# nekopanda/Amatsukaze

Hardware: NVIDIA H100
Metric: 1920x1080i YV12 frames/sec (logo-eval + combing) (higher is better)
Workload: dtype u8+f32

## Files before the change

__graft_entry__.py:

```python
import os
import sys

ROOT = os.path.dirname(os.path.abspath(__file__))
if ROOT not in sys.path:
    sys.path.insert(0, ROOT)


def build():
    from amatsukaze_b200 import _build
    _build.build()
    _build.build_host_test()
    _build.build_pipeline_test()
    _build.build_host_only_test()
    _build.build_tnr_filter_test()
    _build.build_tnr_widen_test()
    _build.build_tnr_filter_stream_test()
    from oracle import pyoracle
    pyoracle.build_oracle()
    pyoracle.build_ref()
    from oracle import pytnr
    pytnr.build_oracle()
    pytnr.build_ref()
    from oracle import pytnr_stream
    pytnr_stream.build_ref()
    import amatsukaze_b200 as ab
    ab.lib()


def smoke():
    import numpy as np
    import torch
    import amatsukaze_b200 as ab
    from amatsukaze_b200 import synth
    from oracle import pyoracle as po

    assert torch.cuda.is_available(), "smoke() needs a GPU: there is no CPU fallback"
    torch.cuda.set_device(0)
    W, H, n, imgx, imgy = 512, 256, 12, 400, 40
    lg = synth.make_logo(64, 64)
    frames = synth.make_frames(45, n, W, H, device="cuda:0", logo=lg, imgx=imgx, imgy=imgy, logo_period=20)
    ctx = ab.Context(0, torch.cuda.current_stream().cuda_stream)
    logo = ab.Logo.create(lg["data"], 64, 64, W, H, imgx, imgy).deint().create_mask(0.35)
    prm = ab.default_comb_params()
    scores, counts = ctx.scan_comb_frames(ab.yv12_clip(frames, W, H, n, True), [logo], prm)
    torch.cuda.synchronize()
    scores, counts = scores.cpu().numpy(), counts.cpu().numpy()
    Y, U, V = synth.split_planes(frames, W, H)
    if po.ref_available():
        rlog = po.RefLogo.create(lg["data"], 64, 64, W, H, imgx, imgy).deint().create_mask(0.35)
        ref_s = np.stack([po.ref_scan_frame(rlog, Y[i]) for i in range(n)])
        checker = "reference code (oracle/_ref)"
    else:
        olog = po.OracleLogo.create(lg["data"], 64, 64, W, H, imgx, imgy).deint().create_mask(0.35)
        ref_s = np.stack([olog.scan_frame(Y[i]) for i in range(n)])
        checker = "C port (oracle/amtk_oracle.c)"
    ref_c = po.or_comb_clip(Y, U, V, prm.as_list())
    assert np.array_equal(scores[:, 0].view(np.uint32), ref_s.view(np.uint32)), "logo scores differ from the oracle"
    assert np.array_equal(counts, ref_c), "combing counters differ from the oracle"
    launches = ctx.launches
    assert launches >= 2
    ctx.close()
    del logo
    print("smoke ok: %d frames bit-exact vs %s, corr0 range [%.3f, %.3f], launches=%d"
          % (n, checker, ref_s[:, 0].min(), ref_s[:, 0].max(), launches))


if __name__ == "__main__":
    build()
    print("build ok")
```

amatsukaze_b200/csrc/amtk_b200.cu:

```cuda
#include "amtk_internal.h"
#include "logo_kernels.cuh"
#include "comb_kernels.cuh"
#include "comb_stream.cuh"
#include "comb_mma.cuh"
#include "scan_kernels.cuh"
#include "tnr_kernels.cuh"
#include <algorithm>
#include <cfloat>
#include <cmath>
#include <cstdlib>
#include <cstring>
#include <deque>
#include <mutex>

extern "C" { static int logo_ensure_device(const amtk_logo* cl, amtk_ctx* ctx, bool need_tables); }

namespace amtk {

static thread_local std::string g_error;
static constexpr size_t kEvalSmemLimit = 226 * 1024;
void set_error(const std::string& msg) { g_error = msg; }
bool cuda_ok(cudaError_t e, const char* what) {
  if (e == cudaSuccess) return true;
  set_error(std::string("CUDA error: ") + cudaGetErrorString(e) + " in " + what);
// ... 52 lines not shown
  if (ctx->stage_bytes < need) {
    for (int b = 0; b < 2; ++b) { if (ctx->stage[b]) cudaFree(ctx->stage[b]); ctx->stage[b] = nullptr; }
    ctx->stage_bytes = 0;
    for (int b = 0; b < 2; ++b) AMTK_CUDA(cudaMalloc(&ctx->stage[b], need));
    ctx->stage_bytes = need;
  }
  int chunk = 0;
  long long h2d = 0;
  for (int lo = frame0; lo < frame0 + nframes; lo += per, ++chunk) {
    const int hi = std::min(frame0 + nframes, lo + per);
    const int b = chunk & 1;
    const int first = (need_prev && lo > 0) ? lo - 1 : lo;
    AMTK_CUDA(cudaStreamWaitEvent(ctx->copy_stream, ctx->ev_done[b], 0));
    AMTK_CUDA(cudaMemcpyAsync(ctx->stage[b], reinterpret_cast<const uint8_t*>(clip->base) + (size_t)first * fs,
                              (size_t)(hi - first) * fs, cudaMemcpyHostToDevice, ctx->copy_stream));
    AMTK_CUDA(cudaEventRecord(ctx->ev_copy[b], ctx->copy_stream));
    AMTK_CUDA(cudaStreamWaitEvent(ctx->stream, ctx->ev_copy[b], 0));
    Window w{ reinterpret_cast<const uint8_t*>(ctx->stage[b]), first, hi - first };
    if (!fn(w, lo, hi)) return 0;
    AMTK_CUDA(cudaEventRecord(ctx->ev_done[b], ctx->stream));
    h2d += (long long)(hi - first) * (long long)fs;
  }
  ctx->h2d_bytes_last = h2d;
  return 1;
}

template <typename Fn>
static int for_each_roi_window(amtk_ctx* ctx, const amtk_clip* clip, int frame0, int nframes, int rx, int ry, int rw, int rh,
                               bool with_chroma, bool write_back, Fn fn) {
  if (frame0 < 0 || nframes < 0 || frame0 + nframes > clip->num_frames) AMTK_FAIL("frame range outside the clip");
  if (nframes == 0) return 1;
  if (clip->on_device) {
    Window w{ reinterpret_cast<const uint8_t*>(clip->base), 0, clip->num_frames };
    return fn(*clip, w, frame0, frame0 + nframes, 0, 0);
  }
  const int bps = clip->bytes_per_sample, lx = clip->log_uvx, ly = clip->log_uvy;
  const int A = 16 << lx;
  const int xb0 = ((rx * bps) / A) * A;
  const int xb1 = std::min(clip->pitch_y, (((rx + rw) * bps + A - 1) / A) * A);
  const int cp = ((xb1 - xb0 + A - 1) / A) * A;
  const int dy = ry & ~((1 << ly) - 1);
  const int y1 = std::min(clip->height, (ry + rh + (1 << ly) - 1) & ~((1 << ly) - 1));
  const int rowsY = y1 - dy, rowsC = with_chroma ? (rowsY >> ly) : 0;
  const int cpc = cp >> lx, spanY = xb1 - xb0;
  const int xc0 = xb0 >> lx, spanC = std::min(clip->pitch_uv - xc0, spanY >> lx);
  const int rows_u = rowsY, rows_c_as_y = (int)(((long long)cpc * rowsC + cp - 1) / cp);
  const long long offU = (long long)cp * rows_u, offV = offU + (long long)cp * rows_c_as_y;
  const long long fs = with_chroma ? offV + (long long)cp * rows_c_as_y : (long long)cp * rowsY;
  if (cp <= 0 || rowsY <= 0 || (with_chroma && spanC <= 0)) AMTK_FAIL("ROI staging: empty rectangle");
  size_t budget = (size_t)256 << 20;
  if (const char* e = getenv("AMTK_STAGE_MB")) budget = (size_t)std::max(1, atoi(e)) << 20;
  const int per = (int)std::max<size_t>(1, std::min<size_t>((size_t)nframes, budget / (size_t)fs));
  const size_t need = (size_t)per * (size_t)fs;
  if (ctx->stage_bytes < need) {
    for (int b = 0; b < 2; ++b) { if (ctx->stage[b]) cudaFree(ctx->stage[b]); ctx->stage[b] = nullptr; }
    ctx->stage_bytes = 0;
    for (int b = 0; b < 2; ++b) AMTK_CUDA(cudaMalloc(&ctx->stage[b], std::max(need, (size_t)1 << 20)));
    ctx->stage_bytes = std::max(need, (size_t)1 << 20);
  }
  amtk_clip v = *clip;
  v.frame_stride = fs; v.off_u = offU; v.off_v = offV;
  v.width = cp / bps; v.height = rowsY; v.pitch_y = cp; v.pitch_uv = cpc; v.on_device = 1;
  const uint8_t* hbase = reinterpret_cast<const uint8_t*>(clip->base);
  auto copy_plane = [&](int pl, uint8_t* dev, int first, int count, bool to_host, cudaStream_t st) -> bool {
    const long long hoff = pl == 0 ? 0 : (pl == 1 ? clip->off_u : clip->off_v);
    const int hp = pl ? clip->pitch_uv : clip->pitch_y, dp = pl ? cpc : cp;
    const int span = pl ? spanC : spanY, rows = pl ? rowsC : rowsY;
    const long long doff = pl == 0 ? 0 : (pl == 1 ? offU : offV);
    uint8_t* h = const_cast<uint8_t*>(hbase) + (long long)first * clip->frame_stride + hoff + (long long)(pl ? (dy >> ly) : dy) * hp + (pl ? xc0 : xb0);
    uint8_t* d = dev + doff;
    if (clip->frame_stride % hp == 0 && fs % dp == 0) {
      cudaMemcpy3DParms p3; memset(&p3, 0, sizeof(p3));
      const cudaPitchedPtr hptr = make_cudaPitchedPtr(h, (size_t)hp, (size_t)hp, (size_t)(clip->frame_stride / hp));
      const cudaPitchedPtr dptr = make_cudaPitchedPtr(d, (size_t)dp, (size_t)dp, (size_t)(fs / dp));
      p3.srcPtr = to_host ? dptr : hptr; p3.dstPtr = to_host ? hptr : dptr;
      p3.extent = make_cudaExtent((size_t)span, (size_t)rows, (size_t)count);
      p3.kind = to_host ? cudaMemcpyDeviceToHost : cudaMemcpyHostToDevice;
      return cuda_ok(cudaMemcpy3DAsync(&p3, st), "cudaMemcpy3DAsync(roi)");
    }
    for (int f = 0; f < count; ++f) {
      uint8_t* hf = h + (long long)f * clip->frame_stride; uint8_t* df = d + (long long)f * fs;
      if (!cuda_ok(to_host ? cudaMemcpy2DAsync(hf, hp, df, dp, span, rows, cudaMemcpyDeviceToHost, st)
                           : cudaMemcpy2DAsync(df, dp, hf, hp, span, rows, cudaMemcpyHostToDevice, st), "cudaMemcpy2DAsync(roi)")) return false;
    }
    return true;
  };
  int chunk = 0;
  for (int lo = frame0; lo < frame0 + nframes; lo += per, ++chunk) {
    const int hi = std::min(frame0 + nframes, lo + per);
    const int b = chunk & 1;
    uint8_t* dev = reinterpret_cast<uint8_t*>(ctx->stage[b]);
    AMTK_CUDA(cudaStreamWaitEvent(ctx->copy_stream, ctx->ev_done[b], 0));
    for (int pl = 0; pl < (with_chroma ? 3 : 1); ++pl) if (!copy_plane(pl, dev, lo, hi - lo, false, ctx->copy_stream)) return 0;
    AMTK_CUDA(cudaEventRecord(ctx->ev_copy[b], ctx->copy_stream));
    AMTK_CUDA(cudaStreamWaitEvent(ctx->stream, ctx->ev_copy[b], 0));
    v.base = dev; v.num_frames = hi - lo;
    Window w{ dev, lo, hi - lo };
    if (!fn(v, w, lo, hi, xb0 / bps, dy)) return 0;
    if (write_back)
      for (int pl = 0; pl < (with_chroma ? 3 : 1); ++pl) if (!copy_plane(pl, dev, lo, hi - lo, true, ctx->stream)) return 0;
    AMTK_CUDA(cudaEventRecord(ctx->ev_done[b], ctx->stream));
  }
  ctx->h2d_bytes_last = (long long)nframes * ((long long)spanY * rowsY + (with_chroma ? 2LL * spanC * rowsC : 0));
  return 1;
}

struct EvalSpec {
  const amtk_logo* logo;
  int roi_x, roi_y;
  int roi_w, roi_h;
  int src_mode, src_off, src_stride;
  int nfades; const float* fades;
  int take_abs;
  int out_off, out_fade_stride;
};

static bool want_smem(amtk_ctx* ctx, const void* fn, int bytes) {
  static std::mutex mu;
  static std::vector<std::pair<std::pair<int, const void*>, int>> table;
  std::lock_guard<std::mutex> lock(mu);
  for (auto& e : table) if (e.first.first == ctx->device && e.first.second == fn) {
    if (e.second >= bytes) return true;
    if (!cuda_ok(cudaFuncSetAttribute(fn, cudaFuncAttributeMaxDynamicSharedMemorySize, bytes), "cudaFuncSetAttribute")) return false;
    e.second = bytes; return true;
  }
  if (!cuda_ok(cudaFuncSetAttribute(fn, cudaFuncAttributeMaxDynamicSharedMemorySize, bytes), "cudaFuncSetAttribute")) return false;
  table.emplace_back(std::make_pair(ctx->device, fn), bytes);
  return true;
}

static int launch_eval(amtk_ctx* ctx, const amtk_clip* clip, const Window& win, int lo, int hi, int pitch_elems,
                       const EvalSpec& sp, float* dout, int out_frame_stride, int out_row0) {
  const amtk::HostLogo& hl = sp.logo->host;
  if (!logo_ensure_device(sp.logo, ctx, true)) return 0;
  if (sp.nfades < 1 || sp.nfades > kMaxFades) AMTK_FAIL("too many fade levels");
  const int count = hl.count();
  const int bits = clip->bits_per_sample;
  const float maxv = (float)((1 << bits) - 1);
  if (count == 0) {
    AMTK_FAIL("logo has no feature pixels");
  }
  const int countPad = sp.logo->countPad;
  const int bps = clip->bytes_per_sample;
  const int box_x = ((sp.roi_x * bps) & ~15) / bps;
  const int box_w = ((((sp.roi_x - box_x) + sp.roi_w) * bps + 15) & ~15) / bps;
  const long long pitch_bytes = (long long)pitch_elems * bps;
  const long long plane_rows = ((long long)clip->pitch_y * clip->height) / pitch_bytes;
  const bool tma_ok = ctx->encode_tiled && box_w <= 256 && sp.roi_h <= 256 && (pitch_bytes & 15) == 0 &&
                      (clip->frame_stride & 15) == 0 && (reinterpret_cast<uintptr_t>(win.dev_base) & 15) == 0;
  int ab_smem = 1, pair_fades = 1;
  size_t smem = logo_scores_smem_bytes(sp.roi_w * sp.roi_h, hl.w * hl.h, box_w * sp.roi_h * bps, ab_smem, pair_fades);
  if (smem > kEvalSmemLimit) { ab_smem = 0; smem = logo_scores_smem_bytes(sp.roi_w * sp.roi_h, hl.w * hl.h, box_w * sp.roi_h * bps, ab_smem, pair_fades); }
  if (smem > kEvalSmemLimit) { pair_fades = 0; smem = logo_scores_smem_bytes(sp.roi_w * sp.roi_h, hl.w * hl.h, box_w * sp.roi_h * bps, ab_smem, pair_fades); }
  if (smem > kEvalSmemLimit) AMTK_FAIL("logo too large for the shared-memory evaluation path (more than ~24k pixels)");
  CUtensorMap roi_map;
  memset(&roi_map, 0, sizeof(roi_map));
  if (tma_ok) {
    cuuint64_t gdim[3] = { (cuuint64_t)pitch_elems, (cuuint64_t)plane_rows, (cuuint64_t)win.count };
    cuuint64_t gstr[2] = { (cuuint64_t)pitch_bytes, (cuuint64_t)clip->frame_stride };
    cuuint32_t box[3] = { (cuuint32_t)box_w, (cuuint32_t)sp.roi_h, 1u };
    cuuint32_t estr[3] = { 1u, 1u, 1u };
    CUresult r = ctx->encode_tiled(&roi_map, bps == 1 ? CU_TENSOR_MAP_DATA_TYPE_UINT8 : CU_TENSOR_MAP_DATA_TYPE_UINT16, 3,
                                   const_cast<uint8_t*>(win.dev_base), gdim, gstr, box, estr, CU_TENSOR_MAP_INTERLEAVE_NONE,
                                   CU_TENSOR_MAP_SWIZZLE_NONE, CU_TENSOR_MAP_L2_PROMOTION_NONE, CU_TENSOR_MAP_FLOAT_OOB_FILL_NONE);
    if (r != CUDA_SUCCESS) AMTK_FAIL("cuTensorMapEncodeTiled(roi) failed (" + std::to_string((int)r) + ")");
  }
  const size_t per_frame = (size_t)sp.nfades * countPad * sizeof(float);
  const int batch = (int)std::max<size_t>(1, std::min<size_t>((size_t)(hi - lo), ((size_t)96 << 20) / per_frame));
  if (!ensure(&ctx->scratch, &ctx->scratch_bytes, ctx->scratch_off + per_frame * batch)) return 0;
  for (int f0 = lo; f0 < hi; f0 += batch) {
    const int n = std::min(batch, hi - f0);
    EvalJob job;
    job.ybase = win.dev_base; job.frame_stride = clip->frame_stride; job.pitch = pitch_elems;
    job.frame0 = f0 - win.first; job.nframes = n;
    job.imgx = sp.roi_x; job.imgy = sp.roi_y;
    job.roi_w = sp.roi_w; job.roi_h = sp.roi_h;
    job.src_mode = sp.src_mode; job.src_off = sp.src_off; job.src_stride = sp.src_stride;
    job.logo = logo_dev(sp.logo); job.maxv = maxv; job.nfades = sp.nfades;
    for (int i = 0; i < sp.nfades; ++i) job.fades[i] = sp.fades[i];
    job.scores = reinterpret_cast<float*>(reinterpret_cast<uint8_t*>(ctx->scratch) + ctx->scratch_off);
    job.use_tma = tma_ok ? 1 : 0; job.roi_box_w = box_w; job.roi_box_x = box_x; job.roi_map = roi_map;
    job.ab_smem = ab_smem; job.pair_fades = pair_fades;
    const int slices3 = (count + kEvalThreads * 3 - 1) / (kEvalThreads * 3);
    int pxt = 3, slices = slices3;
    if (count <= kEvalThreads) { pxt = 1; slices = 1; }
    else if (count <= kEvalThreads * 2) { pxt = 2; slices = 1; }
    const int lanes = std::max(1, std::min(n, (ctx->sm_count * ctx->knobs.eval_waves) / slices));
    dim3 grid(slices, lanes);
    const bool u16 = clip->bytes_per_sample == 2;
    const bool w64 = hl.w == 64 && sp.roi_w == 64 && ctx->knobs.eval_cw;
    const bool wh64 = w64 && hl.h == 64 && sp.roi_h == 64;
#define AMTK_LAUNCH_SCORES(T, P)                                                                              \
  do {                                                                                                        \
    void (*kfn)(const EvalJob) = wh64 ? logo_scores_kernel<T, P, 64, 64> : w64 ? logo_scores_kernel<T, P, 64, 0> : logo_scores_kernel<T, P, 0, 0>; \
    if (!want_smem(ctx, (const void*)kfn, (int)smem)) return 0;                                                \
    kfn<<<grid, kEvalThreads, smem, ctx->stream>>>(job);                                                      \
  } while (0)
    if (!u16) { if (pxt == 1) AMTK_LAUNCH_SCORES(uint8_t, 1); else if (pxt == 2) AMTK_LAUNCH_SCORES(uint8_t, 2); else AMTK_LAUNCH_SCORES(uint8_t, 3); }
    else      { if (pxt == 1) AMTK_LAUNCH_SCORES(uint16_t, 1); else if (pxt == 2) AMTK_LAUNCH_SCORES(uint16_t, 2); else AMTK_LAUNCH_SCORES(uint16_t, 3); }
#undef AMTK_LAUNCH_SCORES
    AMTK_CUDA(cudaGetLastError());
    const int total = n * sp.nfades;
    float* sum_out = dout + (size_t)(f0 - out_row0) * out_frame_stride;
    const size_t sum_smem = (size_t)32 * (countPad + 4) * sizeof(float);
    if (sum_smem <= 200 * 1024) {
      if (!want_smem(ctx, (const void*)logo_sum_bulk_kernel, (int)sum_smem)) return 0;
      logo_sum_bulk_kernel<<<(total + 31) / 32, 32, sum_smem, ctx->stream>>>(
          job.scores, count, countPad, n, sp.nfades, hl.blackScore, sp.take_abs, sum_out, out_frame_stride, sp.out_off, sp.out_fade_stride);
    } else {
      logo_sum_kernel<<<(total + kSumThreads - 1) / kSumThreads, kSumThreads, 0, ctx->stream>>>(
          job.scores, count, countPad, n, sp.nfades, hl.blackScore, sp.take_abs, sum_out, out_frame_stride, sp.out_off, sp.out_fade_stride);
    }
    AMTK_CUDA(cudaGetLastError());
    ctx->launches += 2;
  }
  return 1;
}

static bool roi_inside(const amtk::HostLogo& full, const amtk_clip* clip, int pitch_elems) {
  if (full.imgx < 0 || full.imgy < 0) return false;
  const long long last = (long long)full.imgx + full.w - 1 + (long long)(full.imgy + full.h - 1) * pitch_elems;
  const long long plane_elems = (long long)clip->pitch_y / clip->bytes_per_sample * clip->height;
  return full.imgx + full.w <= pitch_elems && last < plane_elems;
}

static int comb_thresholds_ok(const amtk_comb_params* p, int bytes_per_sample) {
  if (bytes_per_sample == 2) {
    const int all[6] = { p->th_move_y, p->th_shima_y, p->th_lshima_y, p->th_move_c, p->th_shima_c, p->th_lshima_c };
    for (int v : all) if (v < 1) { set_error("comb: thresholds must be >= 1"); return 0; }
    if (p->th_move_y > 32768 || p->th_move_c > 32768) { set_error("comb: th_move must be in [1,32768] for 16-bit samples"); return 0; }
    return 1;
  }
  const int m[2] = { p->th_move_y, p->th_move_c };
  const int s[4] = { p->th_shima_y, p->th_lshima_y, p->th_shima_c, p->th_lshima_c };
  for (int v : m) if (v < 1 || v > 128) { set_error("comb: th_move must be in [1,128]"); return 0; }
  for (int v : s) if (v < 1 || v > 2047) { set_error("comb: th_shima/th_lshima must be in [1,2047]"); return 0; }
  return 1;
}

struct CombVariant {
  int R, strip, stages, sync, TH, boxH, threads, smem;
  void (*kernel)(const CombArgs);
  void (*kernel16)(const CombArgs);
};
template <typename Cfg> static CombVariant make_variant() {
  return CombVariant{ Cfg::R, Cfg::STRIP, Cfg::STAGES, Cfg::SYNC, Cfg::TH, Cfg::BOXH, Cfg::THREADS, Cfg::SMEM, comb_tma_kernel<Cfg, 1>, nullptr };
}
template <typename Cfg> static CombVariant make_variant16() {
  return CombVariant{ Cfg::R, Cfg::STRIP, Cfg::STAGES, Cfg::SYNC, Cfg::TH, Cfg::BOXH, Cfg::THREADS, Cfg::SMEM, comb_tma_kernel<Cfg, 1>, comb_tma_kernel<Cfg, 2> };
}
static const CombVariant* comb_variants(int* n) {
  static const CombVariant v[] = {
    make_variant16<CombCfg<15, 8, 3, 0>>(), make_variant16<CombCfg<16, 8, 3, 0>>(), make_variant16<CombCfg<17, 8, 3, 0>>(),
    make_variant<CombCfg<17, 8, 2, 0>>(), make_variant<CombCfg<17, 8, 4, 0>>(), make_variant<CombCfg<17, 8, 3, 1>>(),
  };
  *n = (int)(sizeof(v) / sizeof(v[0]));
  return v;
}

static int pick_comb_R(int hY, int hC) {
  int best = 16; long long best_waste = -1;
  for (int R = 17; R >= 15; --R) {
    const int th = 8 * R;
    const long long waste = (long long)((hY + th - 1) / th) * th - hY + 2LL * (((hC + th - 1) / th) * th - hC) / 2;
    if (best_waste < 0 || waste < best_waste) { best_waste = waste; best = R; }
  }
  return best;
}

struct WsVariant { int R, stages, warps, bps, TH, boxH, smem; bool band; void (*kernel)(const WsArgs); };
template <typename Cfg> static WsVariant make_ws() { return WsVariant{ Cfg::R, Cfg::STAGES, Cfg::WARPS, Cfg::BPS, Cfg::TH, Cfg::BOXH, Cfg::SMEM, Cfg::BAND, comb_ws_kernel<Cfg> }; }
static const WsVariant* ws_variants(int* n) {
  static const WsVariant v[] = { make_ws<WsCfg<17, 2>>(), make_ws<WsCfg<15, 2>>(), make_ws<WsCfg<16, 2>>(), make_ws<WsCfg<9, 2>>(), make_ws<WsCfg<15, 3>>(), make_ws<WsCfg<12, 2>>(), make_ws<WsCfg<10, 2>>(),
                                 make_ws<WsCfg<15, 2, 7>>(), make_ws<WsCfg<13, 2, 5>>(), make_ws<WsCfg<15, 2, 2>>(), make_ws<WsCfg<15, 3, 3>>(),
                                 make_ws<WsCfg<15, 2, 4, 2>>(), make_ws<WsCfg<16, 2, 4, 2>>(), make_ws<WsCfg<17, 2, 4, 2>>(),
                                 make_ws<WbCfg<15, 2>>(), make_ws<WbCfg<16, 2>>(), make_ws<WbCfg<17, 2>>(), make_ws<WbCfg<15, 3>>() };
  *n = (int)(sizeof(v) / sizeof(v[0]));
  return v;
}
static int pick_ws_R(int hY, int hC) {
  int best = 17; long long best_waste = -1;
  for (int R : { 17, 16, 15 }) {
    const int th = 4 * R;
    const long long waste = 2LL * ((long long)((hY + th - 1) / th) * th - hY) + 2LL * ((long long)((hC + th - 1) / th) * th - hC);
    if (best_waste < 0 || waste < best_waste) { best_waste = waste; best = R; }
  }
  return best;
}

static int ws_watchdog_ok(amtk_ctx* ctx) {
  if (!ctx->watch_pending) return 1;
  AMTK_CUDA(cudaEventSynchronize(ctx->ev_watch));
  ctx->watch_pending = false;
  const int* d = ctx->ws_watch;
  if (d[0]) {
    char msg[256];
    snprintf(msg, sizeof(msg), "comb_ws (band form): a device-side wait of the previous launch timed out (wait %d, step %d, CTA %d, thread %d, parity %d); its counters are not valid",
             d[1], d[2], d[3], d[4], d[5]);
    AMTK_FAIL(msg);
  }
  return 1;
}

static int launch_comb_ws(amtk_ctx* ctx, const amtk_clip* clip, const Window& win, int lo, int hi,
                          const amtk_comb_params* prm, int* dcounts, int out_row0) {
  const int hY = clip->height, hC = clip->height >> clip->log_uvy;
  const int wY = clip->width, wC = clip->width >> clip->log_uvx;
  const int R = ctx->knobs.comb_R ? ctx->knobs.comb_R : pick_ws_R(hY, hC);
  int nvar = 0; const WsVariant* vars = ws_variants(&nvar); const WsVariant* V = nullptr;
  const int bps = clip->bytes_per_sample;
  const bool band = bps == 1 && ctx->knobs.comb_ws_band && ctx->knobs.comb_ws_warps == kWsWarps;
  for (int i = 0; i < nvar; ++i)
    if (vars[i].R == R && vars[i].stages == ctx->knobs.comb_ws_stages && vars[i].warps == ctx->knobs.comb_ws_warps && vars[i].bps == bps && vars[i].band == band) V = &vars[i];
  if (!V) AMTK_FAIL("comb: no warp-stream kernel variant for the requested AMTK_COMB_* settings");
  const int WW = V->warps;
  if (!ws_watchdog_ok(ctx)) return 0;
  WsArgs args;
  memset(&args, 0, sizeof(args));
  const CUtensorMapL2promotion promo = ctx->knobs.comb_l2 == 0 ? CU_TENSOR_MAP_L2_PROMOTION_NONE : ctx->knobs.comb_l2 == 64 ? CU_TENSOR_MAP_L2_PROMOTION_L2_64B :
                                       ctx->knobs.comb_l2 == 256 ? CU_TENSOR_MAP_L2_PROMOTION_L2_256B : CU_TENSOR_MAP_L2_PROMOTION_L2_128B;
  for (int pl = 0; pl < 3; ++pl) {
    const long long off = pl == 0 ? 0 : (pl == 1 ? clip->off_u : clip->off_v);
    cuuint64_t gdim[3] = { (cuuint64_t)(pl ? wC : wY) * bps, (cuuint64_t)(pl ? hC : hY), (cuuint64_t)win.count };
    cuuint64_t gstr[2] = { (cuuint64_t)(pl ? clip->pitch_uv : clip->pitch_y), (cuuint64_t)clip->frame_stride };
    cuuint32_t box[3] = { (cuuint32_t)(band ? kWbHalf : kWsTW), (cuuint32_t)V->boxH, 1u };
    cuuint32_t estr[3] = { 1u, 1u, 1u };
    if (ctx->encode_tiled(&args.map[pl], CU_TENSOR_MAP_DATA_TYPE_UINT8, 3, const_cast<uint8_t*>(win.dev_base) + off, gdim, gstr, box, estr,
                          CU_TENSOR_MAP_INTERLEAVE_NONE, CU_TENSOR_MAP_SWIZZLE_NONE, promo, CU_TENSOR_MAP_FLOAT_OOB_FILL_NONE) != CUDA_SUCCESS)
      AMTK_FAIL("cuTensorMapEncodeTiled failed");
  }
  const int remC = (wC * bps) % kWsTW;
  const long long uv_dist = clip->off_v - clip->off_u;
  const bool pair_uv = !band && ctx->knobs.comb_merge_uv && remC > 0 && remC <= kWsTW / 2 && uv_dist > 0 && (uv_dist & 15) == 0;
  if (pair_uv) {
    cuuint64_t gdim[4] = { (cuuint64_t)wC * bps, 2u, (cuuint64_t)hC, (cuuint64_t)win.count };
    cuuint64_t gstr[3] = { (cuuint64_t)uv_dist, (cuuint64_t)clip->pitch_uv, (cuuint64_t)clip->frame_stride };
    cuuint32_t box[4] = { (cuuint32_t)(kWsTW / 2), 2u, (cuuint32_t)V->boxH, 1u };
    cuuint32_t estr[4] = { 1u, 1u, 1u, 1u };
    if (ctx->encode_tiled(&args.map_uv, CU_TENSOR_MAP_DATA_TYPE_UINT8, 4, const_cast<uint8_t*>(win.dev_base) + clip->off_u, gdim, gstr, box, estr,
                          CU_TENSOR_MAP_INTERLEAVE_NONE, CU_TENSOR_MAP_SWIZZLE_NONE, promo, CU_TENSOR_MAP_FLOAT_OOB_FILL_NONE) != CUDA_SUCCESS)
      AMTK_FAIL("cuTensorMapEncodeTiled(uv pair) failed");
  }
  const int tyY = (hY + V->TH - 1) / V->TH, tyC = (hC + V->TH - 1) / V->TH;
  int tile0 = 0, nc = 0;
  auto thresholds = [&](WsClass& C, bool chroma) {
    C.cls = chroma ? 1 : 0; C.H = chroma ? hC : hY;
    const int tM = chroma ? prm->th_move_c : prm->th_move_y, tS = chroma ? prm->th_shima_c : prm->th_shima_y, tL = chroma ? prm->th_lshima_c : prm->th_lshima_y;
    if (bps == 1) {
      C.thM = (unsigned)(0x80 - tM) * 0x01010101u;
      C.thS = (unsigned)tS * 0x00010001u;
      C.thL = (unsigned)tL * 0x00010001u;
    } else {
      C.thM = (unsigned)std::min(tM, 2047) * 0x00010001u;
      C.thS = (unsigned)(8192 + std::min(tS, 8191)) * 0x00010001u;
      C.thL = (unsigned)(8192 + std::min(tL, 8191)) * 0x00010001u;
    }
  };
  for (int pl = 0; pl < 3; ++pl) {
    WsClass& C = args.cl[nc];
    const int w = (pl ? wC : wY) * bps;
    C.kind = 0; C.map = pl; C.W = w; thresholds(C, pl != 0);
    C.tilesX = band ? (w + kWbW - 1) / kWbW : (pl && pair_uv) ? w / kWsTW : (w + kWsTW - 1) / kWsTW;
    C.tile0 = tile0; C.ntiles = C.tilesX * (pl ? tyC : tyY);
    if (C.ntiles == 0) continue;
    tile0 += C.ntiles; ++nc;
  }
  if (pair_uv) {
    WsClass& C = args.cl[nc];
    C.kind = 1; C.x0 = wC * bps - remC; C.tilesX = 1; thresholds(C, true);
    C.tile0 = tile0; C.ntiles = tyC; tile0 += C.ntiles; ++nc;
  }
  args.nclasses = nc;
  const int ntiles = tile0, nf = hi - lo;
  amtk_ctx::CombPlan& plan = ctx->plan;
  if (plan.occ_kernel != (const void*)V->kernel) {
    int occ = 0;
    AMTK_CUDA(cudaFuncSetAttribute(V->kernel, cudaFuncAttributeMaxDynamicSharedMemorySize, V->smem));
    AMTK_CUDA(cudaOccupancyMaxActiveBlocksPerMultiprocessor(&occ, V->kernel, 32 * WW, V->smem));
    if (occ < 1) AMTK_FAIL("comb kernel does not fit on an SM");
    plan.occ = occ; plan.occ_kernel = (const void*)V->kernel; plan.valid = false;
  }
  int occ = plan.occ;
  if (ctx->knobs.comb_ctas > 0) occ = std::min(occ, ctx->knobs.comb_ctas);
  const long long total = (long long)ntiles * nf;
  const int per_cta = band ? 1 : WW;
  const int nwarps = ctx->sm_count * occ * per_cta;
  const int grid = (int)std::min<long long>((long long)ctx->sm_count * occ, (total + per_cta - 1) / per_cta);
  const int f0 = lo - win.first;
  if (!(plan.valid && plan.wY == wY && plan.hY == hY && plan.wC == wC && plan.hC == hC && plan.ntiles == ntiles && plan.nf == nf && plan.f0 == f0 &&
        plan.R == V->R + 100 * bps + 1000 * band && plan.item == ctx->knobs.comb_item + 1000 * ctx->knobs.comb_tail && plan.ctas == occ * WW)) {
    int big = ctx->knobs.comb_item > 0 ? ctx->knobs.comb_item : 64, small = std::max(4, big / 4);
    while (big > 8 && (long long)ntiles * (nf / big) < 6LL * nwarps) { big /= 2; small = std::max(4, big / 4); }
    const int tail_frames = std::min(nf, std::max(small, (int)(nf * 0.15)));
    const int head_frames = nf - tail_frames;
    const int tiny = ctx->knobs.comb_tail;
    const int end_frames = (tiny > 0 && tiny < small) ? std::min(tail_frames, std::max(tiny, (int)(nf * 0.04))) : 0;
    const int mid_end = nf - end_frames;
    std::vector<CombSegment> segs;
    segs.reserve((size_t)ntiles * (head_frames / big + tail_frames / small + (tiny > 0 ? end_frames / tiny : 0) + 3));
    auto tier = [&](int fa, int fz, int step) {
      if (band) {
        for (int f = fa; f < fz; f += step)
          for (int t = 0; t < ntiles; ++t) segs.push_back(CombSegment{ t, f0 + f, f0 + std::min(fz, f + step) });
      } else {
        for (int t = 0; t < ntiles; ++t)
          for (int f = fa; f < fz; f += step) segs.push_back(CombSegment{ t, f0 + f, f0 + std::min(fz, f + step) });
      }
    };
    tier(0, head_frames, big);
    tier(head_frames, mid_end, small);
    if (tiny > 0) tier(mid_end, nf, tiny);
    const size_t seg_bytes = segs.size() * sizeof(CombSegment);
    plan.q_off = (seg_bytes + 255) & ~(size_t)255;
    plan.valid = false;
    if (!ensure(&plan.dev, &plan.cap, plan.q_off + 256)) return 0;
    AMTK_CUDA(cudaMemcpyAsync(plan.dev, segs.data(), seg_bytes, cudaMemcpyHostToDevice, ctx->stream));
    AMTK_CUDA(cudaStreamSynchronize(ctx->stream));
    plan.nitems = (int)segs.size();
    plan.wY = wY; plan.hY = hY; plan.wC = wC; plan.hC = hC; plan.ntiles = ntiles; plan.nf = nf; plan.f0 = f0; plan.R = V->R + 100 * bps + 1000 * band;
    plan.item = ctx->knobs.comb_item + 1000 * ctx->knobs.comb_tail; plan.ctas = occ * WW; plan.valid = true;
  }
  AMTK_CUDA(cudaMemsetAsync(reinterpret_cast<uint8_t*>(plan.dev) + plan.q_off, 0, 256, ctx->stream));
  args.segs = reinterpret_cast<const CombSegment*>(plan.dev);
  args.nitems = plan.nitems;
  args.queue = reinterpret_cast<int*>(reinterpret_cast<uint8_t*>(plan.dev) + plan.q_off);
  args.counts = dcounts;
  args.out_frame0 = out_row0 - win.first;
  AMTK_CUDA(cudaMemsetAsync(dcounts + (size_t)(lo - out_row0) * 12, 0, (size_t)nf * 12 * sizeof(int), ctx->stream));
  std::pair<cudaEvent_t, cudaEvent_t> ev{ nullptr, nullptr };
  if (ctx->timing) {
    if (!ctx->timing_pool.empty()) { ev = ctx->timing_pool.back(); ctx->timing_pool.pop_back(); }
    else { AMTK_CUDA(cudaEventCreate(&ev.first)); AMTK_CUDA(cudaEventCreate(&ev.second)); }
    AMTK_CUDA(cudaEventRecord(ev.first, ctx->stream));
  }
  args.prefetch = ctx->knobs.comb_ws_prefetch;
  if (ctx->want_side_mark) {
    AMTK_CUDA(cudaEventRecord(ctx->ev_side, ctx->stream));
    ctx->want_side_mark = false;
  }
  V->kernel<<<grid, 32 * WW, V->smem, ctx->stream>>>(args);
  AMTK_CUDA(cudaGetLastError());
  if (ctx->timing) { AMTK_CUDA(cudaEventRecord(ev.second, ctx->stream)); ctx->timing_events.push_back(ev); }
  ctx->launches += 1;
  if (band) {
    if (!ctx->ws_watch) {
      AMTK_CUDA(cudaHostAlloc(&ctx->ws_watch, 8 * sizeof(int), cudaHostAllocDefault));
      AMTK_CUDA(cudaEventCreateWithFlags(&ctx->ev_watch, cudaEventDisableTiming));
    }
    AMTK_CUDA(cudaMemcpyAsync(ctx->ws_watch, args.queue + 16, 8 * sizeof(int), cudaMemcpyDeviceToHost, ctx->stream));
    AMTK_CUDA(cudaEventRecord(ctx->ev_watch, ctx->stream));
    ctx->watch_pending = true;
  }
  return 1;
}

static int launch_comb_mma(amtk_ctx* ctx, const amtk_clip* clip, const Window& win, int lo, int hi,
                           const amtk_comb_params* prm, int* dcounts, int out_row0) {
  const int hY = clip->height, hC = clip->height >> clip->log_uvy;
  const int wY = clip->width, wC = clip->width >> clip->log_uvx;
  WsArgs args;
  memset(&args, 0, sizeof(args));
  const CUtensorMapL2promotion promo = ctx->knobs.comb_l2 == 0 ? CU_TENSOR_MAP_L2_PROMOTION_NONE : ctx->knobs.comb_l2 == 64 ? CU_TENSOR_MAP_L2_PROMOTION_L2_64B :
                                       ctx->knobs.comb_l2 == 256 ? CU_TENSOR_MAP_L2_PROMOTION_L2_256B : CU_TENSOR_MAP_L2_PROMOTION_L2_128B;
  for (int pl = 0; pl < 3; ++pl) {
    const long long off = pl == 0 ? 0 : (pl == 1 ? clip->off_u : clip->off_v);
    cuuint64_t gdim[3] = { (cuuint64_t)(pl ? wC : wY), (cuuint64_t)(pl ? hC : hY), (cuuint64_t)win.count };
    cuuint64_t gstr[2] = { (cuuint64_t)(pl ? clip->pitch_uv : clip->pitch_y), (cuuint64_t)clip->frame_stride };
    cuuint32_t box[3] = { (cuuint32_t)kMmTW, (cuuint32_t)kMmBoxH, 1u };
    cuuint32_t estr[3] = { 1u, 1u, 1u };
    if (ctx->encode_tiled(&args.map[pl], CU_TENSOR_MAP_DATA_TYPE_UINT8, 3, const_cast<uint8_t*>(win.dev_base) + off, gdim, gstr, box, estr,
                          CU_TENSOR_MAP_INTERLEAVE_NONE, CU_TENSOR_MAP_SWIZZLE_128B, promo, CU_TENSOR_MAP_FLOAT_OOB_FILL_NONE) != CUDA_SUCCESS)
      AMTK_FAIL("cuTensorMapEncodeTiled failed");
  }
  const int tyY = (hY + kMmTH - 1) / kMmTH, tyC = (hC + kMmTH - 1) / kMmTH;
  int tile0 = 0, nc = 0;
  for (int pl = 0; pl < 3; ++pl) {
    WsClass& C = args.cl[nc];
    const bool chroma = pl != 0;
    C.kind = 0; C.map = pl; C.cls = chroma ? 1 : 0; C.H = chroma ? hC : hY;
    C.thM = (unsigned)(0x80 - (chroma ? prm->th_move_c : prm->th_move_y)) * 0x01010101u;
    C.thS = (unsigned)(chroma ? prm->th_shima_c : prm->th_shima_y) * 0x00010001u;
    C.thL = (unsigned)(chroma ? prm->th_lshima_c : prm->th_lshima_y) * 0x00010001u;
    C.tilesX = ((chroma ? wC : wY) + kMmTW - 1) / kMmTW;
    C.tile0 = tile0; C.ntiles = C.tilesX * (chroma ? tyC : tyY);
    if (C.ntiles == 0) continue;
    tile0 += C.ntiles; ++nc;
  }
  args.nclasses = nc;
  const int ntiles = tile0, nf = hi - lo;
  amtk_ctx::CombPlan& plan = ctx->plan;
  const int NS = ctx->knobs.comb_mma == 2 ? 2 : 1;
  void (*kern)(const WsArgs) = NS == 2 ? comb_mma_kernel<2> : comb_mma_kernel<1>;
  const int smem = NS * kMmSmemPerStream + kMmBandBytes + 1024;
  if (plan.occ_kernel != (const void*)kern) {
    AMTK_CUDA(cudaFuncSetAttribute(kern, cudaFuncAttributeMaxDynamicSharedMemorySize, smem));
    int occ_q = 0;
    AMTK_CUDA(cudaOccupancyMaxActiveBlocksPerMultiprocessor(&occ_q, kern, kMmThreads, smem));
    if (occ_q < 1) AMTK_FAIL("comb_mma: kernel does not fit on an SM");
    plan.occ = occ_q; plan.occ_kernel = (const void*)kern; plan.valid = false;
  }
  int occ = plan.occ;
  if (ctx->knobs.comb_ctas > 0) occ = std::min(occ, ctx->knobs.comb_ctas);
  const int npairs_t = (ntiles + NS - 1) / NS;
  const long long total = (long long)npairs_t * nf;
  const int nstreams = ctx->sm_count * occ;
  const int grid = (int)std::min<long long>(nstreams, total);
  const int f0 = lo - win.first;
  if (!(plan.valid && plan.wY == wY && plan.hY == hY && plan.wC == wC && plan.hC == hC && plan.ntiles == ntiles && plan.nf == nf && plan.f0 == f0 &&
        plan.R == 1000 * NS + kMmTH && plan.item == ctx->knobs.comb_item && plan.ctas == occ)) {
    int big = ctx->knobs.comb_item > 0 ? ctx->knobs.comb_item : 64, small = std::max(4, big / 4);
    while (big > 8 && (long long)npairs_t * (nf / big) < 6LL * nstreams) { big /= 2; small = std::max(4, big / 4); }
    const int tail_frames = std::min(nf, std::max(small, (int)(nf * 0.15)));
    const int head_frames = nf - tail_frames;
    std::vector<CombSegment> segs;
    segs.reserve((size_t)NS * npairs_t * (head_frames / big + tail_frames / small + 2));
    auto push_block = [&](int fa, int fz) {
      for (int t = 0; t < ntiles; t += NS) {
        segs.push_back(CombSegment{ t, fa, fz });
        if (NS == 2) segs.push_back(CombSegment{ t + 1 < ntiles ? t + 1 : ~t, fa, fz });
      }
    };
    for (int f = 0; f < head_frames; f += big) push_block(f0 + f, f0 + std::min(head_frames, f + big));
    for (int f = head_frames; f < nf; f += small) push_block(f0 + f, f0 + std::min(nf, f + small));
    const size_t seg_bytes = segs.size() * sizeof(CombSegment);
    plan.q_off = (seg_bytes + 255) & ~(size_t)255;
    plan.valid = false;
    if (!ensure(&plan.dev, &plan.cap, plan.q_off + 256)) return 0;
    AMTK_CUDA(cudaMemcpyAsync(plan.dev, segs.data(), seg_bytes, cudaMemcpyHostToDevice, ctx->stream));
    AMTK_CUDA(cudaStreamSynchronize(ctx->stream));
    plan.nitems = (int)segs.size();
    plan.wY = wY; plan.hY = hY; plan.wC = wC; plan.hC = hC; plan.ntiles = ntiles; plan.nf = nf; plan.f0 = f0; plan.R = 1000 * NS + kMmTH;
    plan.item = ctx->knobs.comb_item; plan.ctas = occ; plan.valid = true;
  }
  AMTK_CUDA(cudaMemsetAsync(reinterpret_cast<uint8_t*>(plan.dev) + plan.q_off, 0, 256, ctx->stream));
  args.segs = reinterpret_cast<const CombSegment*>(plan.dev);
  args.nitems = plan.nitems;
  args.queue = reinterpret_cast<int*>(reinterpret_cast<uint8_t*>(plan.dev) + plan.q_off);
  args.counts = dcounts;
  args.out_frame0 = out_row0 - win.first;
  AMTK_CUDA(cudaMemsetAsync(dcounts + (size_t)(lo - out_row0) * 12, 0, (size_t)nf * 12 * sizeof(int), ctx->stream));
  std::pair<cudaEvent_t, cudaEvent_t> ev{ nullptr, nullptr };
  if (ctx->timing) {
    if (!ctx->timing_pool.empty()) { ev = ctx->timing_pool.back(); ctx->timing_pool.pop_back(); }
    else { AMTK_CUDA(cudaEventCreate(&ev.first)); AMTK_CUDA(cudaEventCreate(&ev.second)); }
    AMTK_CUDA(cudaEventRecord(ev.first, ctx->stream));
  }
  kern<<<grid, kMmThreads, smem, ctx->stream>>>(args);
  AMTK_CUDA(cudaGetLastError());
  if (ctx->timing) { AMTK_CUDA(cudaEventRecord(ev.second, ctx->stream)); ctx->timing_events.push_back(ev); }
  ctx->launches += 1;
  int dbg[8] = { 0, 0, 0, 0, 0, 0, 0, 0 };
  AMTK_CUDA(cudaMemcpyAsync(dbg, args.queue + 16, sizeof(dbg), cudaMemcpyDeviceToHost, ctx->stream));
  AMTK_CUDA(cudaStreamSynchronize(ctx->stream));
  if (dbg[0]) {
    char msg[256];
    snprintf(msg, sizeof(msg), "comb_mma<%d>: a device-side wait timed out (wait %d, step %d, CTA %d, thread %d, parity %d); results discarded",
             NS, dbg[1], dbg[2], dbg[3], dbg[4], dbg[5]);
    AMTK_FAIL(msg);
  }
  return 1;
}

static int launch_comb(amtk_ctx* ctx, const amtk_clip* clip, const Window& win, int lo, int hi,
                       const amtk_comb_params* prm, int* dcounts, int out_row0) {
  const bool tma_layout = !((clip->frame_stride & 15) || (clip->pitch_y & 15) || (clip->pitch_uv & 15) || (clip->off_u & 15) ||
                            (clip->off_v & 15) || (reinterpret_cast<uintptr_t>(win.dev_base) & 15));
  if (!tma_layout || !ctx->encode_tiled || ctx->knobs.comb_generic) {
    CombGenericArgs g;
    g.base = win.dev_base; g.frame_stride = clip->frame_stride;
    g.off[0] = 0; g.off[1] = clip->off_u; g.off[2] = clip->off_v;
    const int bps = clip->bytes_per_sample;
    for (int pl = 0; pl < 3; ++pl) {
      g.pitch[pl] = (pl ? clip->pitch_uv : clip->pitch_y) / bps;
      g.W[pl] = pl ? (clip->width >> clip->log_uvx) : clip->width;
      g.H[pl] = pl ? (clip->height >> clip->log_uvy) : clip->height;
      g.thM[pl] = pl ? prm->th_move_c : prm->th_move_y;
      g.thS[pl] = pl ? prm->th_shima_c : prm->th_shima_y;
      g.thL[pl] = pl ? prm->th_lshima_c : prm->th_lshima_y;
    }
    g.first_frame = lo - win.first; g.prev_of_first = lo > 0 ? lo - 1 - win.first : lo - win.first;
    g.nframes = hi - lo; g.counts = dcounts + (size_t)(lo - out_row0) * 12;
    AMTK_CUDA(cudaMemsetAsync(g.counts, 0, (size_t)(hi - lo) * 12 * sizeof(int), ctx->stream));
    for (int f0 = 0; f0 < hi - lo; f0 += 16384) {
      CombGenericArgs gg = g;
      gg.first_frame = g.first_frame + f0; gg.prev_of_first = f0 ? gg.first_frame - 1 : g.prev_of_first;
      gg.nframes = std::min(16384, hi - lo - f0); gg.counts = g.counts + (size_t)f0 * 12;
      dim3 grid((g.W[0] + kGenTW - 1) / kGenTW, (g.H[0] + kGenTH - 1) / kGenTH, gg.nframes * 3);
      if (bps == 1) comb_generic_kernel<uint8_t><<<grid, 256, 0, ctx->stream>>>(gg);
      else comb_generic_kernel<uint16_t><<<grid, 256, 0, ctx->stream>>>(gg);
      AMTK_CUDA(cudaGetLastError());
      ctx->launches += 1;
    }
    return 1;
  }
  if (clip->bytes_per_sample == 1 && ctx->knobs.comb_mma) return launch_comb_mma(ctx, clip, win, lo, hi, prm, dcounts, out_row0);
  if (ctx->knobs.comb_ws && (clip->bytes_per_sample == 1 || (clip->bits_per_sample <= 10 && ctx->knobs.comb_ws10)))
    return launch_comb_ws(ctx, clip, win, lo, hi, prm, dcounts, out_row0);
  const int hY = clip->height, hC = clip->height >> clip->log_uvy;
  const int R = ctx->knobs.comb_R ? ctx->knobs.comb_R : pick_comb_R(hY, hC);
  int nvar = 0; const CombVariant* vars = comb_variants(&nvar); const CombVariant* V = nullptr;
  for (int i = 0; i < nvar; ++i) if (vars[i].R == R && vars[i].strip == ctx->knobs.comb_strip && vars[i].stages == ctx->knobs.comb_stages && vars[i].sync == ctx->knobs.comb_sync) V = &vars[i];
  if (!V) AMTK_FAIL("comb: no kernel variant for the requested AMTK_COMB_* settings");
  const int bps = clip->bytes_per_sample;
  if (bps == 2 && !V->kernel16) AMTK_FAIL("comb: the selected AMTK_COMB_* variant has no 16-bit kernel");
  const int twe = kCombTW / bps;
  CombArgs args;
  memset(&args, 0, sizeof(args));
  const int wC = clip->width >> clip->log_uvx;
  const int rem = wC % twe;
  const bool merge_uv = ctx->knobs.comb_merge_uv && rem > 0 && rem <= twe / 2 && (V->boxH * (kCombTW / 2)) % 128 == 0;
  int tile0 = 0;
  for (int pl = 0; pl < 4; ++pl) {
    CombPlane& P = args.plane[pl];
    const bool chroma = pl != 0;
    P.W = chroma ? wC : clip->width;
    P.H = chroma ? hC : hY;
    P.tilesX = (P.W + twe - 1) / twe; P.tilesY = (P.H + V->TH - 1) / V->TH;
    if (merge_uv && (pl == 1 || pl == 2)) P.tilesX -= 1;
    if (pl == 3) { P.tilesX = merge_uv ? 1 : 0; if (!merge_uv) P.tilesY = 0; }
    P.tile0 = tile0; tile0 += P.tilesX * P.tilesY;
    P.cls = chroma ? 1 : 0;
    const int thM = chroma ? prm->th_move_c : prm->th_move_y;
    const int thS = chroma ? prm->th_shima_c : prm->th_shima_y, thL = chroma ? prm->th_lshima_c : prm->th_lshima_y;
    if (bps == 1) {
      P.thM = (unsigned)(0x80 - thM) * 0x01010101u;
      P.thS = (unsigned)thS * 0x00010001u;
      P.thL = (unsigned)thL * 0x00010001u;
    } else {
      P.thM = (unsigned)(0x8000 - thM) * 0x00010001u;
      const float fs = (float)thS, fl = (float)thL;
      memcpy(&P.thS, &fs, 4); memcpy(&P.thL, &fl, 4);
    }
    if (pl == 3) break;
    const long long off = pl == 0 ? 0 : (pl == 1 ? clip->off_u : clip->off_v);
    const int pitch = pl ? clip->pitch_uv : clip->pitch_y;
    cuuint64_t gdim[3] = { (cuuint64_t)P.W, (cuuint64_t)P.H, (cuuint64_t)win.count };
    cuuint64_t gstr[2] = { (cuuint64_t)pitch, (cuuint64_t)clip->frame_stride };
    cuuint32_t estr[3] = { 1u, 1u, 1u };
    const CUtensorMapL2promotion promo = ctx->knobs.comb_l2 == 0 ? CU_TENSOR_MAP_L2_PROMOTION_NONE : ctx->knobs.comb_l2 == 64 ? CU_TENSOR_MAP_L2_PROMOTION_L2_64B :
                                         ctx->knobs.comb_l2 == 256 ? CU_TENSOR_MAP_L2_PROMOTION_L2_256B : CU_TENSOR_MAP_L2_PROMOTION_L2_128B;
    for (int half = 0; half < (pl && merge_uv ? 2 : 1); ++half) {
      cuuint32_t box[3] = { (cuuint32_t)(half ? twe / 2 : twe), (cuuint32_t)V->boxH, 1u };
      CUtensorMap* m = half ? &args.map_half[pl - 1] : &args.map[pl];
      CUresult r = ctx->encode_tiled(m, bps == 1 ? CU_TENSOR_MAP_DATA_TYPE_UINT8 : CU_TENSOR_MAP_DATA_TYPE_UINT16, 3, const_cast<uint8_t*>(win.dev_base) + off, gdim, gstr, box, estr,
                                     CU_TENSOR_MAP_INTERLEAVE_NONE, CU_TENSOR_MAP_SWIZZLE_NONE, promo, CU_TENSOR_MAP_FLOAT_OOB_FILL_NONE);
      if (r != CUDA_SUCCESS) AMTK_FAIL("cuTensorMapEncodeTiled failed (" + std::to_string((int)r) + ")");
    }
  }
  args.half_x = wC - rem;
  const int ntiles = tile0;
  const int nf = hi - lo;
  int occ = 0;
  void (*kern)(const CombArgs) = bps == 1 ? V->kernel : V->kernel16;
  AMTK_CUDA(cudaFuncSetAttribute(kern, cudaFuncAttributeMaxDynamicSharedMemorySize, V->smem));
  AMTK_CUDA(cudaOccupancyMaxActiveBlocksPerMultiprocessor(&occ, kern, V->threads, V->smem));
  if (occ < 1) AMTK_FAIL("comb kernel does not fit on an SM");
  if (ctx->knobs.comb_ctas > 0) occ = std::min(occ, ctx->knobs.comb_ctas);
  const long long total = (long long)ntiles * nf;
  int grid = (int)std::min<long long>((long long)ctx->sm_count * occ, total);
  std::vector<CombSegment> segs;
  const int chunks = std::max(1, std::min(nf, grid / std::max(1, ntiles)));
  const bool lockstep = ctx->knobs.comb_part == 1;
  if (lockstep) grid = chunks * ntiles;
  std::vector<int> seg_start((size_t)grid + 1, 0);
  if (lockstep) {
    for (int b = 0; b < grid; ++b) {
      const int c = b / ntiles, t = b % ntiles;
      const int f0 = (int)((long long)nf * c / chunks), f1 = (int)((long long)nf * (c + 1) / chunks);
      seg_start[b] = (int)segs.size();
      if (f1 > f0) segs.push_back(CombSegment{ t, lo - win.first + f0, lo - win.first + f1 });
    }
  } else
  for (int b = 0; b < grid; ++b) {
    const long long lo_i = total * b / grid, hi_i = total * (b + 1) / grid;
    seg_start[b] = (int)segs.size();
    long long i = lo_i;
    while (i < hi_i) {
      const int t = (int)(i / nf), f = (int)(i % nf);
      const int take = (int)std::min<long long>(nf - f, hi_i - i);
      segs.push_back(CombSegment{ t, lo - win.first + f, lo - win.first + f + take });
      i += take;
    }
  }
  seg_start[grid] = (int)segs.size();
  const size_t seg_bytes = segs.size() * sizeof(CombSegment), st_bytes = seg_start.size() * sizeof(int);
  const size_t st_off = (seg_bytes + 255) & ~(size_t)255;
  if (!ensure(&ctx->small, &ctx->small_bytes, st_off + st_bytes)) return 0;
  AMTK_CUDA(cudaMemcpyAsync(ctx->small, segs.data(), seg_bytes, cudaMemcpyHostToDevice, ctx->stream));
  AMTK_CUDA(cudaMemcpyAsync(reinterpret_cast<uint8_t*>(ctx->small) + st_off, seg_start.data(), st_bytes, cudaMemcpyHostToDevice, ctx->stream));
  args.segs = reinterpret_cast<const CombSegment*>(ctx->small);
  args.seg_start = reinterpret_cast<const int*>(reinterpret_cast<uint8_t*>(ctx->small) + st_off);
  args.counts = dcounts;
  args.out_frame0 = out_row0 - win.first;
  AMTK_CUDA(cudaMemsetAsync(dcounts + (size_t)(lo - out_row0) * 12, 0, (size_t)nf * 12 * sizeof(int), ctx->stream));
  std::pair<cudaEvent_t, cudaEvent_t> ev{ nullptr, nullptr };
  if (ctx->timing) {
    if (!ctx->timing_pool.empty()) { ev = ctx->timing_pool.back(); ctx->timing_pool.pop_back(); }
    else { AMTK_CUDA(cudaEventCreate(&ev.first)); AMTK_CUDA(cudaEventCreate(&ev.second)); }
    AMTK_CUDA(cudaEventRecord(ev.first, ctx->stream));
  }
  kern<<<grid, V->threads, V->smem, ctx->stream>>>(args);
  AMTK_CUDA(cudaGetLastError());
  if (ctx->timing) { AMTK_CUDA(cudaEventRecord(ev.second, ctx->stream)); ctx->timing_events.push_back(ev); }
  ctx->launches += 1;
  return 1;
}

static void clip_span(const amtk_clip* c, uintptr_t* lo, uintptr_t* hi) {
  const int hc = c->height >> c->log_uvy, rowc = (c->width >> c->log_uvx) * c->bytes_per_sample;
  const long long ends[3] = { (long long)c->pitch_y * (c->height - 1) + (long long)c->width * c->bytes_per_sample,
                              c->off_u + (long long)c->pitch_uv * (hc - 1) + rowc, c->off_v + (long long)c->pitch_uv * (hc - 1) + rowc };
  const long long first = std::min<long long>(0, std::min(c->off_u, c->off_v));
  const long long last = std::max(ends[0], std::max(ends[1], ends[2])) + (long long)(c->num_frames - 1) * c->frame_stride;
  *lo = reinterpret_cast<uintptr_t>(c->base) + first; *hi = reinterpret_cast<uintptr_t>(c->base) + last;
}

static int launch_tnr(amtk_ctx* ctx, const amtk_clip* src, const Window& win, const amtk_clip* dl, uint8_t* dbase,
                      int lo, int hi, const amtk_tnr_params* p, bool ring = false) {
  TnrArgs a;
  a.src = win.dev_base; a.src_stride = src->frame_stride; a.s_offu = src->off_u; a.s_offv = src->off_v;
  a.s_pitchY = src->pitch_y; a.s_pitchUV = src->pitch_uv; a.src_first = win.first; a.src_count = win.count;
  a.dst = dbase; a.dst_stride = dl->frame_stride; a.d_offu = dl->off_u; a.d_offv = dl->off_v;
  a.d_pitchY = dl->pitch_y; a.d_pitchUV = dl->pitch_uv;
  a.W = src->width; a.H = src->height; a.N = src->num_frames;
  a.lo = lo; a.hi = hi;
  a.thresh = p->threshold << (src->bits_per_sample - 8);
  a.interlaced = p->interlaced;
  const int bps = src->bytes_per_sample, obps = dl->bytes_per_sample, nl = 16 / obps;
  const int shift = dl->bits_per_sample - src->bits_per_sample;
  const TnrWiden wd{ ldexpf(0.5f, -shift), ldexpf(1.0f, shift) };
  const int sa = 16 * bps / obps;
  auto al = [](long long v, int m) { return (v & (m - 1)) == 0; };
  a.vec = al((long long)reinterpret_cast<uintptr_t>(win.dev_base), sa) && al(a.src_stride, sa) && al(a.s_pitchY, sa) &&
          al(a.s_offu, sa / 2) && al(a.s_offv, sa / 2) && al(a.s_pitchUV, sa / 2) &&
          al((long long)reinterpret_cast<uintptr_t>(dbase), 16) && al(a.dst_stride, 16) && al(a.d_pitchY, 16) &&
          al(a.d_offu, 8) && al(a.d_offv, 8) && al(a.d_pitchUV, 8);
  const long long groups = (long long)((a.W + nl - 1) / nl) * (a.H >> 1);
  const long long want = (long long)ctx->sm_count * 2048 * 2;
  const int n = hi - lo;
  int nruns = (int)std::max<long long>(1, std::min<long long>({ (long long)n, (want + groups - 1) / groups, 65535LL }));
  a.run = (n + nruns - 1) / nruns;
  nruns = (n + a.run - 1) / a.run;
  const dim3 grid((unsigned)((groups + kTnrThreads - 1) / kTnrThreads), (unsigned)nruns);
  const int d = p->temporal_distance;
#define AMTK_TNR_CASE(TI, TO, RING, WIDEN)                                                                    \
  switch (d) {                                                                                                \
    case 0: tnr_kernel<TI, TO, 0, RING, WIDEN><<<grid, kTnrThreads, 0, ctx->stream>>>(a, wd); break;         \
    case 1: tnr_kernel<TI, TO, 1, RING, WIDEN><<<grid, kTnrThreads, 0, ctx->stream>>>(a, wd); break;         \
    case 2: tnr_kernel<TI, TO, 2, RING, WIDEN><<<grid, kTnrThreads, 0, ctx->stream>>>(a, wd); break;         \
    case 3: tnr_kernel<TI, TO, 3, RING, WIDEN><<<grid, kTnrThreads, 0, ctx->stream>>>(a, wd); break;         \
    case 4: tnr_kernel<TI, TO, 4, RING, WIDEN><<<grid, kTnrThreads, 0, ctx->stream>>>(a, wd); break;         \
    case 5: tnr_kernel<TI, TO, 5, RING, WIDEN><<<grid, kTnrThreads, 0, ctx->stream>>>(a, wd); break;         \
    case 6: tnr_kernel<TI, TO, 6, RING, WIDEN><<<grid, kTnrThreads, 0, ctx->stream>>>(a, wd); break;         \
    case 7: tnr_kernel<TI, TO, 7, RING, WIDEN><<<grid, kTnrThreads, 0, ctx->stream>>>(a, wd); break;         \
    default: tnr_general_kernel<TI, TO, RING, WIDEN><<<grid, kTnrThreads, 0, ctx->stream>>>(a, d, wd); break;     \
  }
  static_assert(kTnrMaxTemplD == 7, "the switch above lists every register-window kernel");
  if (shift == 0) {
    if (bps == 1) { if (ring) { AMTK_TNR_CASE(uint8_t, uint8_t, true, false) } else { AMTK_TNR_CASE(uint8_t, uint8_t, false, false) } }
    else { if (ring) { AMTK_TNR_CASE(uint16_t, uint16_t, true, false) } else { AMTK_TNR_CASE(uint16_t, uint16_t, false, false) } }
  } else {
    if (bps == 1) { if (ring) { AMTK_TNR_CASE(uint8_t, uint16_t, true, true) } else { AMTK_TNR_CASE(uint8_t, uint16_t, false, true) } }
    else { if (ring) { AMTK_TNR_CASE(uint16_t, uint16_t, true, true) } else { AMTK_TNR_CASE(uint16_t, uint16_t, false, true) } }
  }
#undef AMTK_TNR_CASE
  AMTK_CUDA(cudaGetLastError());
  ctx->launches += 1;
  return 1;
}

static std::once_flag g_driver_once;
static amtk_encode_tiled_fn g_encode = nullptr;

}

using namespace amtk;

extern "C" {

const char* amtk_last_error(void) { return g_error.c_str(); }
int amtk_version(void) { return 100; }

int amtk_device_count(void) {
  int n = 0;
  if (cudaGetDeviceCount(&n) != cudaSuccess) { cudaGetLastError(); return 0; }
  return n;
}

int amtk_ctx_create(int device, void* cuda_stream, amtk_ctx** out) {
  if (!out) AMTK_FAIL("amtk_ctx_create: out is null");
  *out = nullptr;
  int n = 0;
  if (cudaGetDeviceCount(&n) != cudaSuccess || n == 0) { cudaGetLastError(); AMTK_FAIL("no CUDA device: this library has no CPU fallback"); }
  if (device < 0 || device >= n) AMTK_FAIL("amtk_ctx_create: bad device ordinal");
  int prev = 0; AMTK_CUDA(cudaGetDevice(&prev));
  AMTK_CUDA(cudaSetDevice(device));
  cudaDeviceProp prop; AMTK_CUDA(cudaGetDeviceProperties(&prop, device));
  if (prop.major != 9 || prop.minor != 0) { cudaSetDevice(prev); AMTK_FAIL("this build targets sm_90a (Hopper H100) only"); }
  amtk_ctx* c = new amtk_ctx();
  c->device = device; c->sm_count = prop.multiProcessorCount;
  c->stream = reinterpret_cast<cudaStream_t>(cuda_stream); c->own_stream = false;
  bool ok = cuda_ok(cudaStreamCreateWithFlags(&c->copy_stream, cudaStreamNonBlocking), "cudaStreamCreate(copy)") &&
            cuda_ok(cudaStreamCreateWithFlags(&c->side_stream, cudaStreamNonBlocking), "cudaStreamCreate(side)") &&
            cuda_ok(cudaEventCreateWithFlags(&c->ev_side, cudaEventDisableTiming), "cudaEventCreate") &&
            cuda_ok(cudaEventCreateWithFlags(&c->ev_side_done, cudaEventDisableTiming), "cudaEventCreate") &&
            cuda_ok(cudaStreamCreateWithFlags(&c->side_stream2, cudaStreamNonBlocking), "cudaStreamCreate(side2)") &&
            cuda_ok(cudaEventCreateWithFlags(&c->ev_fork, cudaEventDisableTiming), "cudaEventCreate") &&
            cuda_ok(cudaEventCreateWithFlags(&c->ev_join1, cudaEventDisableTiming), "cudaEventCreate") &&
            cuda_ok(cudaEventCreateWithFlags(&c->ev_join2, cudaEventDisableTiming), "cudaEventCreate");
  for (int b = 0; b < 2 && ok; ++b) {
    ok = cuda_ok(cudaEventCreateWithFlags(&c->ev_copy[b], cudaEventDisableTiming), "cudaEventCreate") &&
         cuda_ok(cudaEventCreateWithFlags(&c->ev_done[b], cudaEventDisableTiming), "cudaEventCreate");
  }
  std::call_once(g_driver_once, [] {
    void* fn = nullptr; cudaDriverEntryPointQueryResult q;
    if (cudaGetDriverEntryPoint("cuTensorMapEncodeTiled", &fn, cudaEnableDefault, &q) == cudaSuccess && q == cudaDriverEntryPointSuccess)
      g_encode = reinterpret_cast<amtk_encode_tiled_fn>(fn);
    else cudaGetLastError();
  });
  c->encode_tiled = g_encode;
  if (const char* e = getenv("AMTK_COMB_STRIP")) c->knobs.comb_strip = atoi(e);
  if (const char* e = getenv("AMTK_COMB_STAGES")) c->knobs.comb_stages = atoi(e);
  if (const char* e = getenv("AMTK_COMB_R")) c->knobs.comb_R = atoi(e);
  if (const char* e = getenv("AMTK_COMB_CTAS")) c->knobs.comb_ctas = atoi(e);
  if (const char* e = getenv("AMTK_COMB_SYNC")) c->knobs.comb_sync = atoi(e);
  if (const char* e = getenv("AMTK_COMB_GENERIC")) c->knobs.comb_generic = atoi(e);
  if (const char* e = getenv("AMTK_COMB_MERGE_UV")) c->knobs.comb_merge_uv = atoi(e);
  if (const char* e = getenv("AMTK_COMB_PART")) c->knobs.comb_part = atoi(e);
  if (const char* e = getenv("AMTK_EVAL_WAVES")) c->knobs.eval_waves = std::max(1, atoi(e));
  if (const char* e = getenv("AMTK_COMB_L2")) c->knobs.comb_l2 = atoi(e);
  if (const char* e = getenv("AMTK_COMB_WS")) c->knobs.comb_ws = atoi(e);
  if (const char* e = getenv("AMTK_SCAN_LITE")) c->knobs.scan_lite = atoi(e);
  if (const char* e = getenv("AMTK_LITE_CTAS")) c->knobs.lite_ctas = std::max(1, atoi(e));
  if (const char* e = getenv("AMTK_COMB_WS_STAGES")) c->knobs.comb_ws_stages = atoi(e);
  if (const char* e = getenv("AMTK_COMB_ITEM")) c->knobs.comb_item = atoi(e);
  if (const char* e = getenv("AMTK_COMB_TAIL")) c->knobs.comb_tail = atoi(e);
  if (const char* e = getenv("AMTK_COMB_MMA")) c->knobs.comb_mma = atoi(e);
  if (const char* e = getenv("AMTK_COMB_WS10")) c->knobs.comb_ws10 = atoi(e);
  if (const char* e = getenv("AMTK_EVAL_CW")) c->knobs.eval_cw = atoi(e);
  if (const char* e = getenv("AMTK_EVAL_PAR")) c->knobs.eval_par = atoi(e);
  if (const char* e = getenv("AMTK_SCAN_OVERLAP")) c->knobs.scan_overlap = atoi(e);
  if (const char* e = getenv("AMTK_COMB_WS_WARPS")) c->knobs.comb_ws_warps = atoi(e);
  if (const char* e = getenv("AMTK_COMB_WS_PF")) c->knobs.comb_ws_prefetch = atoi(e);
  if (const char* e = getenv("AMTK_COMB_WS_BAND")) c->knobs.comb_ws_band = atoi(e);
  cudaSetDevice(prev);
  if (!ok) { amtk_ctx_destroy(c); return 0; }
  *out = c;
  return 1;
}

void amtk_ctx_destroy(amtk_ctx* c) {
  if (!c) return;
  int prev = 0; cudaGetDevice(&prev); cudaSetDevice(c->device);
  if (c->stream) cudaStreamSynchronize(c->stream);
  if (c->copy_stream) { cudaStreamSynchronize(c->copy_stream); cudaStreamDestroy(c->copy_stream); }
  if (c->side_stream) { cudaStreamSynchronize(c->side_stream); cudaStreamDestroy(c->side_stream); }
  if (c->ev_side) cudaEventDestroy(c->ev_side);
  if (c->ev_side_done) cudaEventDestroy(c->ev_side_done);
  if (c->side_stream2) { cudaStreamSynchronize(c->side_stream2); cudaStreamDestroy(c->side_stream2); }
  for (cudaEvent_t e : { c->ev_fork, c->ev_join1, c->ev_join2 }) if (e) cudaEventDestroy(e);
  for (int b = 0; b < 2; ++b) { if (c->ev_copy[b]) cudaEventDestroy(c->ev_copy[b]); if (c->ev_done[b]) cudaEventDestroy(c->ev_done[b]); if (c->stage[b]) cudaFree(c->stage[b]); }
  if (c->scratch) cudaFree(c->scratch);
  if (c->small) cudaFree(c->small);
  if (c->dout) cudaFree(c->dout);
  if (c->dout2) cudaFree(c->dout2);
  if (c->hout) cudaFreeHost(c->hout);
  if (c->ws_watch) cudaFreeHost(c->ws_watch);
  if (c->ev_watch) cudaEventDestroy(c->ev_watch);
  if (c->plan.dev) cudaFree(c->plan.dev);
  for (auto* v : { &c->timing_events, &c->timing_pool }) for (auto& ev : *v) { cudaEventDestroy(ev.first); cudaEventDestroy(ev.second); }
  if (c->own_stream && c->stream) cudaStreamDestroy(c->stream);
  cudaSetDevice(prev);
  delete c;
}

int amtk_ctx_synchronize(amtk_ctx* c) {
  if (!c) AMTK_FAIL("null context");
  DevSelect ds(c); if (!ds.ok) return 0;
  AMTK_CUDA(cudaStreamSynchronize(c->stream));
  return 1;
}
int64_t amtk_ctx_launch_count(const amtk_ctx* c) { return c ? c->launches : 0; }
int64_t amtk_ctx_last_h2d_bytes(const amtk_ctx* c) { return c ? c->h2d_bytes_last : 0; }

int amtk_ctx_set_kernel_timing(amtk_ctx* c, int enable) {
  if (!c) AMTK_FAIL("null context");
  c->timing = enable != 0;
  return 1;
}

int amtk_ctx_get_kernel_timing(amtk_ctx* c, double* ms_total, int64_t* launches, int reset) {
  if (!c) AMTK_FAIL("null context");
  DevSelect ds(c); if (!ds.ok) return 0;
  AMTK_CUDA(cudaStreamSynchronize(c->stream));
  for (auto& ev : c->timing_events) {
    float ms = 0.0f;
    AMTK_CUDA(cudaEventElapsedTime(&ms, ev.first, ev.second));
    c->timing_ms += ms; c->timing_count += 1;
    c->timing_pool.push_back(ev);
  }
  c->timing_events.clear();
  if (ms_total) *ms_total = c->timing_ms;
  if (launches) *launches = c->timing_count;
  if (reset) { c->timing_ms = 0.0; c->timing_count = 0; }
  return 1;
}

int amtk_probe_read_ms(amtk_ctx* c, const void* ptr, size_t bytes, int reps, double* ms_out) {
  if (!c || !ptr || !ms_out || reps < 1) AMTK_FAIL("amtk_probe_read_ms: bad argument");
  if (reinterpret_cast<uintptr_t>(ptr) & 15) AMTK_FAIL("amtk_probe_read_ms: pointer must be 16-byte aligned");
  DevSelect ds(c); if (!ds.ok) return 0;
  if (!ensure(&c->small, &c->small_bytes, 256)) return 0;
  cudaEvent_t e0, e1;
  AMTK_CUDA(cudaEventCreate(&e0)); AMTK_CUDA(cudaEventCreate(&e1));
  const int grid = c->sm_count * 8;
  unsigned* sink = reinterpret_cast<unsigned*>(c->small);
  read_probe_kernel<<<grid, 256, 0, c->stream>>>(reinterpret_cast<const uint4*>(ptr), bytes / 16, sink);
  AMTK_CUDA(cudaEventRecord(e0, c->stream));
  for (int i = 0; i < reps; ++i) read_probe_kernel<<<grid, 256, 0, c->stream>>>(reinterpret_cast<const uint4*>(ptr), bytes / 16, sink);
  AMTK_CUDA(cudaEventRecord(e1, c->stream));
  AMTK_CUDA(cudaEventSynchronize(e1));
  float ms = 0; AMTK_CUDA(cudaEventElapsedTime(&ms, e0, e1));
  cudaEventDestroy(e0); cudaEventDestroy(e1);
  AMTK_CUDA(cudaGetLastError());
  *ms_out = ms / reps;
  return 1;
}

int amtk_host_alloc(size_t bytes, void** out) {
  if (!out) AMTK_FAIL("amtk_host_alloc: out is null");
  AMTK_CUDA(cudaHostAlloc(out, bytes, cudaHostAllocDefault));
  return 1;
}
void amtk_host_free(void* p) { if (p) cudaFreeHost(p); }

int amtk_device_alloc(amtk_ctx* c, size_t bytes, void** out) {
  if (!c || !out) AMTK_FAIL("amtk_device_alloc: null argument");
  DevSelect ds(c); if (!ds.ok) return 0;
  AMTK_CUDA(cudaMalloc(out, bytes));
  return 1;
}
void amtk_device_free(amtk_ctx* c, void* p) {
  if (!c || !p) return;
  DevSelect ds(c);
  cudaStreamSynchronize(c->stream);
  cudaFree(p);
}
int amtk_memcpy_h2d(amtk_ctx* c, void* dst, const void* src, size_t bytes) {
  if (!c || !dst || !src) AMTK_FAIL("amtk_memcpy_h2d: null argument");
  DevSelect ds(c); if (!ds.ok) return 0;
  AMTK_CUDA(cudaMemcpyAsync(dst, src, bytes, cudaMemcpyHostToDevice, c->stream));
  AMTK_CUDA(cudaStreamSynchronize(c->stream));
  return 1;
}
int amtk_memcpy_d2d(amtk_ctx* c, void* dst, const void* src, size_t bytes) {
  if (!c || !dst || !src) AMTK_FAIL("amtk_memcpy_d2d: null argument");
  DevSelect ds(c); if (!ds.ok) return 0;
  AMTK_CUDA(cudaMemcpyAsync(dst, src, bytes, cudaMemcpyDeviceToDevice, c->stream));
  AMTK_CUDA(cudaStreamSynchronize(c->stream));
  return 1;
}
int amtk_memcpy_d2h(amtk_ctx* c, void* dst, const void* src, size_t bytes) {
  if (!c || !dst || !src) AMTK_FAIL("amtk_memcpy_d2h: null argument");
  DevSelect ds(c); if (!ds.ok) return 0;
  AMTK_CUDA(cudaMemcpyAsync(dst, src, bytes, cudaMemcpyDeviceToHost, c->stream));
  AMTK_CUDA(cudaStreamSynchronize(c->stream));
  return 1;
}

static void logo_free_device(amtk_logo* l) {
  float* fp[] = { l->dA, l->dB, l->dAU, l->dBU, l->dAV, l->dBV, l->dTapsT };
  for (float* p : fp) if (p) cudaFree(p);
  if (l->dPix) cudaFree(l->dPix);
  if (l->dScales) cudaFree(l->dScales);
  l->dA = l->dB = l->dAU = l->dBU = l->dAV = l->dBV = l->dTapsT = nullptr; l->dPix = nullptr; l->dScales = nullptr;
}

static int logo_upload_planes(amtk_logo* l) {
  amtk::HostLogo& h = l->host;
  const size_t ny = h.ySize() * sizeof(float), nc = h.cSize() * sizeof(float);
  float** dst[6] = { &l->dA, &l->dB, &l->dAU, &l->dBU, &l->dAV, &l->dBV };
  const float* src[6] = { h.aY(), h.bY(), h.aU(), h.bU(), h.aV(), h.bV() };
  for (int i = 0; i < 6; ++i) {
    const size_t n = i < 2 ? ny : nc;
    AMTK_CUDA(cudaMalloc(dst[i], std::max<size_t>(n, 16)));
    AMTK_CUDA(cudaMemcpy(*dst[i], src[i], n, cudaMemcpyHostToDevice));
  }
  return 1;
}

static int logo_upload_tables(amtk_logo* l) {
  amtk::HostLogo& h = l->host;
  if (l->dPix) { cudaFree(l->dPix); l->dPix = nullptr; }
  if (l->dTapsT) { cudaFree(l->dTapsT); l->dTapsT = nullptr; }
  if (l->dScales) { cudaFree(l->dScales); l->dScales = nullptr; }
  const int count = h.count();
  if (count > 0) {
    std::vector<float> tapsT((size_t)25 * l->countPad, 0.0f);
    for (int c = 0; c < count; ++c) for (int t = 0; t < 25; ++t) tapsT[(size_t)t * l->countPad + c] = h.kernels[(size_t)c * 25 + t];
    AMTK_CUDA(cudaMalloc(&l->dPix, (size_t)count * sizeof(uint32_t)));
    AMTK_CUDA(cudaMalloc(&l->dTapsT, tapsT.size() * sizeof(float)));
    AMTK_CUDA(cudaMalloc(&l->dScales, (size_t)count * 32 * sizeof(float2)));
    AMTK_CUDA(cudaMemcpy(l->dPix, h.pix.data(), (size_t)count * sizeof(uint32_t), cudaMemcpyHostToDevice));
    AMTK_CUDA(cudaMemcpy(l->dTapsT, tapsT.data(), tapsT.size() * sizeof(float), cudaMemcpyHostToDevice));
    AMTK_CUDA(cudaMemcpy(l->dScales, h.scales.data(), (size_t)count * 32 * sizeof(float2), cudaMemcpyHostToDevice));
  }
  l->tables_uploaded = true;
  return 1;
}

static int logo_ensure_device(const amtk_logo* cl, amtk_ctx* ctx, bool need_tables) {
  amtk_logo* l = const_cast<amtk_logo*>(cl);
  std::lock_guard<std::mutex> lock(l->mu);
  if (l->device >= 0 && l->dA && l->device != ctx->device) AMTK_FAIL("logo already resident on another device");
  l->device = ctx->device;
  if (!l->dA && !logo_upload_planes(l)) return 0;
  if (need_tables) {
    if (!l->has_mask) AMTK_FAIL("logo has no mask: call amtk_logo_create_mask first");
    if (!l->tables_uploaded && !logo_upload_tables(l)) return 0;
  }
  return 1;
}

static int logo_adopt(amtk_ctx* , amtk::HostLogo&& h, amtk_logo** out) {
  amtk_logo* l = new amtk_logo();
  l->host = std::move(h);
  *out = l;
  return 1;
}

int amtk_logo_create(amtk_ctx* ctx, const float* data, int w, int h, int lx, int ly, int imgw, int imgh, int imgx, int imgy, amtk_logo** out) {
  if (!data || !out) AMTK_FAIL("amtk_logo_create: null argument");
  if (w < 5 || h < 5 || w > 4096 || h > 4096 || lx < 0 || lx > 2 || ly < 0 || ly > 2) AMTK_FAIL("amtk_logo_create: bad logo geometry");
  amtk::HostLogo hl; hl.init(w, h, lx, ly, imgw, imgh, imgx, imgy);
  memcpy(hl.data.data(), data, hl.dataSize() * sizeof(float));
  return logo_adopt(ctx, std::move(hl), out);
}

int amtk_logo_load(amtk_ctx* ctx, const char* path, amtk_logo** out, void* header540) {
  if (!path || !out) AMTK_FAIL("amtk_logo_load: null argument");
  amtk::HostLogo hl; amtk::LgdHeader hdr; std::string err;
  if (!amtk::lgd_load(path, hl, &hdr, err)) AMTK_FAIL(err);
  if (header540) memcpy(header540, &hdr, sizeof(hdr));
  return logo_adopt(ctx, std::move(hl), out);
}

int amtk_logo_save(const amtk_logo* l, const char* path, const char* name, int service_id) {
  if (!l || !path) AMTK_FAIL("amtk_logo_save: null argument");
  std::string err;
  if (!amtk::lgd_save(l->host, path, name ? name : "No Name", service_id, err)) AMTK_FAIL(err);
  return 1;
}

void amtk_logo_destroy(amtk_logo* l) {
  if (!l) return;
  if (l->device >= 0 && l->dA) { DevSelect ds(l->device); logo_free_device(l); }
  delete l;
}

int amtk_logo_deint(const amtk_logo* src, amtk_logo** out) {
  if (!src || !out) AMTK_FAIL("amtk_logo_deint: null argument");
  amtk::HostLogo d; amtk::logo_deint(src->host, d);
  return logo_adopt(nullptr, std::move(d), out);
}

int amtk_logo_field(const amtk_logo* src, int bottom, amtk_logo** out) {
  if (!src || !out) AMTK_FAIL("amtk_logo_field: null argument");
  if (src->host.h / 2 < 5) AMTK_FAIL("amtk_logo_field: logo too small");
  amtk::HostLogo f; amtk::logo_field(src->host, bottom != 0, f);
  return logo_adopt(nullptr, std::move(f), out);
}

int amtk_logo_create_mask(amtk_logo* l, float maskratio) {
  if (!l) AMTK_FAIL("amtk_logo_create_mask: null logo");
  if (!(maskratio > 0.0f) || maskratio > 1.0f) AMTK_FAIL("amtk_logo_create_mask: maskratio must be in (0,1]");
  std::lock_guard<std::mutex> lock(l->mu);
  amtk::logo_create_mask(l->host, maskratio);
  l->countPad = std::max(32, (l->host.count() + 31) & ~31);
  l->has_mask = true;
  l->tables_uploaded = false;
  return 1;
}

int amtk_logo_get_info(const amtk_logo* l, amtk_logo_info* o) {
  if (!l || !o) AMTK_FAIL("amtk_logo_get_info: null argument");
  const amtk::HostLogo& h = l->host;
  o->w = h.w; o->h = h.h; o->log_uvx = h.logUVx; o->log_uvy = h.logUVy;
  o->imgw = h.imgw; o->imgh = h.imgh; o->imgx = h.imgx; o->imgy = h.imgy;
  o->maskpixels = h.maskpixels; o->count = h.count(); o->black_score = h.blackScore;
  return 1;
}

int amtk_logo_get_tables(const amtk_logo* l, float* data, uint8_t* mask, float* kernels, float* scales) {
  if (!l) AMTK_FAIL("amtk_logo_get_tables: null logo");
  const amtk::HostLogo& h = l->host;
  if (data) memcpy(data, h.data.data(), h.dataSize() * sizeof(float));
  if ((mask || kernels || scales) && !l->has_mask) AMTK_FAIL("logo has no mask");
  if (mask) memcpy(mask, h.mask.data(), h.mask.size());
  if (kernels) memcpy(kernels, h.kernels.data(), h.kernels.size() * sizeof(float));
  if (scales) memcpy(scales, h.scales.data(), h.scales.size() * sizeof(float));
  return 1;
}

constexpr size_t kHostOutBytes = 64 << 10;
static float* host_out_alias(amtk_ctx* ctx, size_t bytes) {
  if (bytes > kHostOutBytes) return nullptr;
  if (!ctx->hout) {
    if (cudaHostAlloc(&ctx->hout, kHostOutBytes, cudaHostAllocMapped) != cudaSuccess) { cudaGetLastError(); ctx->hout = nullptr; return nullptr; }
    if (cudaHostGetDevicePointer(&ctx->hout_dev, ctx->hout, 0) != cudaSuccess) { cudaGetLastError(); cudaFreeHost(ctx->hout); ctx->hout = nullptr; return nullptr; }
  }
  return reinterpret_cast<float*>(ctx->hout_dev);
}
static float* host_out_buffer(amtk_ctx* ctx, size_t bytes) {
  if (float* a = host_out_alias(ctx, bytes)) return a;
  if (!ensure(&ctx->dout, &ctx->dout_bytes, bytes)) return nullptr;
  return reinterpret_cast<float*>(ctx->dout);
}

static int finish_output(amtk_ctx* ctx, void* host_dst, const void* dev_src, size_t bytes, int out_on_device) {
  if (out_on_device) return 1;
  if (ctx->hout && dev_src == ctx->hout_dev) {
    AMTK_CUDA(cudaStreamSynchronize(ctx->stream));
    memcpy(host_dst, ctx->hout, bytes);
    return 1;
  }
  AMTK_CUDA(cudaMemcpyAsync(host_dst, dev_src, bytes, cudaMemcpyDeviceToHost, ctx->stream));
  AMTK_CUDA(cudaStreamSynchronize(ctx->stream));
  return 1;
}

static int scan_frames_impl(amtk_ctx* ctx, const amtk_clip* real, const amtk_clip* clip, int dx, int dy, amtk_logo* const* logos, int nlogos,
                            const Window& win, int lo, int hi, int pitch_override, float* dscores, int row0) {
  static const float kFades01[2] = { 0.0f, 1.0f };
  const int pitch = pitch_override > 0 ? pitch_override : clip->pitch_y / clip->bytes_per_sample;
  const int real_pitch = pitch_override > 0 ? pitch_override : real->pitch_y / real->bytes_per_sample;
  for (int i = 0; i < nlogos; ++i) {
    const amtk_logo* lg = logos[i];
    float* o = dscores + (size_t)(lo - row0) * nlogos * 2;
    if (!lg || lg->host.imgw != real->width || lg->host.imgh != real->height) {
      fill_pairs_kernel<<<(hi - lo + 127) / 128, 128, 0, ctx->stream>>>(o, hi - lo, nlogos * 2, i * 2, 0.0f, -1.0f);
      AMTK_CUDA(cudaGetLastError()); ctx->launches += 1;
      continue;
    }
    if (!roi_inside(lg->host, real, real_pitch)) AMTK_FAIL("logo rectangle lies outside the frame");
    EvalSpec sp{ lg, lg->host.imgx - dx, lg->host.imgy - dy, lg->host.w, lg->host.h, 0, 0, lg->host.w, 2, kFades01, 0, i * 2, 1 };
    if (!launch_eval(ctx, clip, win, lo, hi, pitch, sp, dscores, nlogos * 2, row0)) return 0;
  }
  return 1;
}

static bool logos_bbox(const amtk_clip* clip, amtk_logo* const* logos, int nlogos, int* rx, int* ry, int* rw, int* rh) {
  int x0 = 1 << 30, y0 = 1 << 30, x1 = -1, y1 = -1;
  for (int i = 0; i < nlogos; ++i) {
    const amtk_logo* lg = logos[i];
    if (!lg || lg->host.imgw != clip->width || lg->host.imgh != clip->height) continue;
    x0 = std::min(x0, lg->host.imgx); y0 = std::min(y0, lg->host.imgy);
    x1 = std::max(x1, lg->host.imgx + lg->host.w); y1 = std::max(y1, lg->host.imgy + lg->host.h);
  }
  if (x1 < 0 || x0 < 0 || y0 < 0 || x1 > clip->width || y1 > clip->height) return false;
  *rx = x0; *ry = y0; *rw = x1 - x0; *rh = y1 - y0;
  return true;
}

int amtk_logo_scan_frames(amtk_ctx* ctx, const amtk_clip* clip, amtk_logo* const* logos, int nlogos,
                          int frame0, int nframes, int pitch_override, float* out, int out_on_device) {
  if (ctx && nframes == 0) return 1;
  if (!ctx || !logos || !out || nlogos < 1) AMTK_FAIL("amtk_logo_scan_frames: bad argument");
  if (!validate_clip(clip, false)) return 0;
  DevSelect ds(ctx); if (!ds.ok) return 0;
  const size_t bytes = (size_t)nframes * nlogos * 2 * sizeof(float);
  float* d = out;
  if (!out_on_device) { d = host_out_buffer(ctx, bytes); if (!d) return 0; }
  int rx, ry, rw, rh;
  if (!clip->on_device && pitch_override <= 0 && logos_bbox(clip, logos, nlogos, &rx, &ry, &rw, &rh)) {
    if (!for_each_roi_window(ctx, clip, frame0, nframes, rx, ry, rw, rh, false, false,
                             [&](const amtk_clip& v, const Window& w, int lo, int hi, int dx, int dy) {
          return scan_frames_impl(ctx, clip, &v, dx, dy, logos, nlogos, w, lo, hi, 0, d, frame0); }))
      return 0;
  } else if (!for_each_window(ctx, clip, frame0, nframes, false, [&](const Window& w, int lo, int hi) {
        return scan_frames_impl(ctx, clip, clip, 0, 0, logos, nlogos, w, lo, hi, pitch_override, d, frame0); }))
    return 0;
  return finish_output(ctx, out, d, bytes, out_on_device);
}

static int analyze_impl(amtk_ctx* ctx, const amtk_clip* clip, int dx, int dy, const amtk_logo* dl, const amtk_logo* ft, const amtk_logo* fb,
                        const Window& win, int lo, int hi, float* dout, int row0) {
  float fades[11];
  for (int f = 0; f <= 10; ++f) fades[f] = (float)f / 10.0f;
  const int pitch = clip->pitch_y / clip->bytes_per_sample;
  const int w = dl->host.w, h = dl->host.h;
  const int rx = dl->host.imgx - dx, ry = dl->host.imgy - dy;
  EvalSpec sp{ dl, rx, ry, w, h, 0, 0, w, 11, fades, 1, 0, 1 };
  EvalSpec st{ ft, rx, ry, w, h, 1, 0, 2 * w, 11, fades, 1, 11, 1 };
  EvalSpec sb{ fb, rx, ry, w, h, 1, w, 2 * w, 11, fades, 1, 22, 1 };
  const int n = hi - lo;
  if (!(ctx->knobs.eval_par && n <= 16 && ctx->side_stream && ctx->side_stream2))
    return launch_eval(ctx, clip, win, lo, hi, pitch, sp, dout, 33, row0) &&
           launch_eval(ctx, clip, win, lo, hi, pitch, st, dout, 33, row0) &&
           launch_eval(ctx, clip, win, lo, hi, pitch, sb, dout, 33, row0);
  const EvalSpec* specs[3] = { &sp, &st, &sb };
  size_t off[3], total = 0;
  for (int i = 0; i < 3; ++i) {
    if (!logo_ensure_device(specs[i]->logo, ctx, true)) return 0;
    off[i] = total;
    total += (((size_t)n * 11 * specs[i]->logo->countPad * sizeof(float)) + 255) & ~(size_t)255;
  }
  if (!ensure(&ctx->scratch, &ctx->scratch_bytes, total)) return 0;
  cudaStream_t main_stream = ctx->stream, streams[3] = { ctx->stream, ctx->side_stream, ctx->side_stream2 };
  cudaEvent_t joins[3] = { nullptr, ctx->ev_join1, ctx->ev_join2 };
  AMTK_CUDA(cudaEventRecord(ctx->ev_fork, main_stream));
  int ok = 1;
  for (int i = 0; i < 3 && ok; ++i) {
    if (i) ok = cuda_ok(cudaStreamWaitEvent(streams[i], ctx->ev_fork, 0), "cudaStreamWaitEvent");
    ctx->stream = streams[i]; ctx->scratch_off = off[i];
    ok = ok && launch_eval(ctx, clip, win, lo, hi, pitch, *specs[i], dout, 33, row0);
    ctx->stream = main_stream; ctx->scratch_off = 0;
    if (i && ok) ok = cuda_ok(cudaEventRecord(joins[i], streams[i]), "cudaEventRecord") &&
                      cuda_ok(cudaStreamWaitEvent(main_stream, joins[i], 0), "cudaStreamWaitEvent");
  }
  if (!ok) { cudaStreamSynchronize(ctx->side_stream); cudaStreamSynchronize(ctx->side_stream2); }
  return ok;
}

int amtk_logo_analyze_frames(amtk_ctx* ctx, const amtk_clip* clip, const amtk_logo* dl, const amtk_logo* ft, const amtk_logo* fb,
                             int frame0, int nframes, float* out, int out_on_device) {
  if (ctx && nframes == 0) return 1;
  if (!ctx || !dl || !ft || !fb || !out) AMTK_FAIL("amtk_logo_analyze_frames: bad argument");
  if (!validate_clip(clip, false)) return 0;
  if (ft->host.w != dl->host.w || fb->host.w != dl->host.w || ft->host.h != dl->host.h / 2 || fb->host.h != dl->host.h / 2)
    AMTK_FAIL("field logos do not match the deint logo");
  DevSelect ds(ctx); if (!ds.ok) return 0;
  const size_t bytes = (size_t)nframes * 33 * sizeof(float);
  float* d = out;
  if (!out_on_device) { d = host_out_buffer(ctx, bytes); if (!d) return 0; }
  if (!roi_inside(dl->host, clip, clip->pitch_y / clip->bytes_per_sample)) AMTK_FAIL("logo rectangle lies outside the frame");
  if (!for_each_roi_window(ctx, clip, frame0, nframes, dl->host.imgx, dl->host.imgy, dl->host.w, dl->host.h, false, false,
                           [&](const amtk_clip& v, const Window& w, int lo, int hi, int dx, int dy) {
        return analyze_impl(ctx, &v, dx, dy, dl, ft, fb, w, lo, hi, d, frame0); }))
    return 0;
  return finish_output(ctx, out, d, bytes, out_on_device);
}

int amtk_logo_eval_fades(amtk_ctx* ctx, const amtk_clip* clip, const amtk_logo* dl, const float* fades, int nfades,
                         int frame0, int nframes, float* out, int out_on_device) {
  if (ctx && nframes == 0) return 1;
  if (!ctx || !dl || !fades || !out) AMTK_FAIL("amtk_logo_eval_fades: bad argument");
  if (nfades < 1 || nfades > kMaxFades) AMTK_FAIL("amtk_logo_eval_fades: 1..24 fade levels");
  if (!validate_clip(clip, false)) return 0;
  DevSelect ds(ctx); if (!ds.ok) return 0;
  const size_t bytes = (size_t)nframes * nfades * sizeof(float);
  float* d = out;
  if (!out_on_device) { d = host_out_buffer(ctx, bytes); if (!d) return 0; }
  const int pitch = clip->pitch_y / clip->bytes_per_sample;
  if (!roi_inside(dl->host, clip, pitch)) AMTK_FAIL("logo rectangle lies outside the frame");
  if (!for_each_roi_window(ctx, clip, frame0, nframes, dl->host.imgx, dl->host.imgy, dl->host.w, dl->host.h, false, false,
                           [&](const amtk_clip& v, const Window& w, int lo, int hi, int dx, int dy) {
        EvalSpec sp{ dl, dl->host.imgx - dx, dl->host.imgy - dy, dl->host.w, dl->host.h, 0, 0, dl->host.w, nfades, fades, 0, 0, 1 };
        return launch_eval(ctx, &v, w, lo, hi, v.pitch_y / v.bytes_per_sample, sp, d, nfades, frame0); }))
    return 0;
  return finish_output(ctx, out, d, bytes, out_on_device);
}

void amtk_comb_default_params(amtk_comb_params* p) {
  if (!p) return;
  p->th_move_y = 20; p->th_shima_y = 12; p->th_lshima_y = 36;
  p->th_move_c = 24; p->th_shima_c = 16; p->th_lshima_c = 48;
}

int amtk_comb_frames(amtk_ctx* ctx, const amtk_clip* clip, const amtk_comb_params* prm, int frame0, int nframes,
                     int32_t* counts, int out_on_device) {
  if (ctx && nframes == 0) return 1;
  if (!ctx || !prm || !counts) AMTK_FAIL("amtk_comb_frames: bad argument");
  if (!validate_clip(clip, true) || !comb_thresholds_ok(prm, clip->bytes_per_sample)) return 0;
  DevSelect ds(ctx); if (!ds.ok) return 0;
  const size_t bytes = (size_t)nframes * 12 * sizeof(int32_t);
  int* d = counts;
  if (!out_on_device) { if (!ensure(&ctx->dout2, &ctx->dout2_bytes, bytes)) return 0; d = reinterpret_cast<int*>(ctx->dout2); }
  if (!for_each_window(ctx, clip, frame0, nframes, true, [&](const Window& w, int lo, int hi) {
        return launch_comb(ctx, clip, w, lo, hi, prm, d, frame0); }))
    return 0;
  return finish_output(ctx, counts, d, bytes, out_on_device);
}

static int launch_scan_lite(amtk_ctx* ctx, const amtk_clip* clip, const Window& win, int lo, int hi, const amtk_logo* lg,
                            float* dscores, int nlogos, int logo_index, int row0, bool side) {
  cudaStream_t st = side ? ctx->side_stream : ctx->stream;
  if (!logo_ensure_device(lg, ctx, true)) return 0;
  const amtk::HostLogo& hl = lg->host;
  const int count = hl.count(), countPad = lg->countPad, n = hi - lo;
  if (!ensure(&ctx->scratch, &ctx->scratch_bytes, (size_t)n * 2 * countPad * sizeof(float))) return 0;
  LiteJob job;
  job.ybase = win.dev_base; job.frame_stride = clip->frame_stride; job.pitch = clip->pitch_y / clip->bytes_per_sample;
  job.frame0 = lo - win.first; job.nframes = n; job.imgx = hl.imgx; job.imgy = hl.imgy;
  job.logo = logo_dev(lg); job.maxv = (float)((1 << clip->bits_per_sample) - 1);
  job.nfades = 2; job.fades[0] = 0.0f; job.fades[1] = 1.0f;
  job.scores = reinterpret_cast<float*>(ctx->scratch);
  const size_t smem = logo_lite_smem_bytes(hl.w, hl.h, clip->bytes_per_sample);
  if (side) AMTK_CUDA(cudaStreamWaitEvent(ctx->side_stream, ctx->ev_side, 0));
  const int grid = side ? std::min(n, ctx->sm_count) : std::min(n, ctx->sm_count * ctx->knobs.lite_ctas);
  static bool carveout_set = false;
  if (!carveout_set) {
    AMTK_CUDA(cudaFuncSetAttribute(logo_lite_kernel<uint8_t>, cudaFuncAttributePreferredSharedMemoryCarveout, cudaSharedmemCarveoutMaxShared));
    AMTK_CUDA(cudaFuncSetAttribute(logo_lite_kernel<uint16_t>, cudaFuncAttributePreferredSharedMemoryCarveout, cudaSharedmemCarveoutMaxShared));
    AMTK_CUDA(cudaFuncSetAttribute(logo_sum_bulk_kernel, cudaFuncAttributePreferredSharedMemoryCarveout, cudaSharedmemCarveoutMaxShared));
    carveout_set = true;
  }
  if (clip->bytes_per_sample == 1) logo_lite_kernel<uint8_t><<<grid, kLiteThreads, smem, st>>>(job);
  else logo_lite_kernel<uint16_t><<<grid, kLiteThreads, smem, st>>>(job);
  AMTK_CUDA(cudaGetLastError());
  const int total = n * 2;
  float* sum_out = dscores + (size_t)(lo - row0) * nlogos * 2;
  const size_t sum_smem = (size_t)32 * (countPad + 4) * sizeof(float);
  if (sum_smem <= 200 * 1024) {
    if (!want_smem(ctx, (const void*)logo_sum_bulk_kernel, (int)sum_smem)) return 0;
    logo_sum_bulk_kernel<<<(total + 31) / 32, 32, sum_smem, st>>>(job.scores, count, countPad, n, 2, hl.blackScore, 0, sum_out, nlogos * 2, logo_index * 2, 1);
  } else {
    logo_sum_kernel<<<(total + kSumThreads - 1) / kSumThreads, kSumThreads, 0, st>>>(job.scores, count, countPad, n, 2, hl.blackScore, 0, sum_out, nlogos * 2, logo_index * 2, 1);
  }
  AMTK_CUDA(cudaGetLastError());
  if (side) AMTK_CUDA(cudaEventRecord(ctx->ev_side_done, ctx->side_stream));
  ctx->launches += 2;
  return 1;
}

int amtk_scan_comb_frames(amtk_ctx* ctx, const amtk_clip* clip, amtk_logo* const* logos, int nlogos,
                          const amtk_comb_params* prm, int frame0, int nframes, float* scores, int32_t* counts, int out_on_device) {
  if (ctx && nframes == 0) return 1;
  if (!ctx || !prm || !counts || !scores || !logos || nlogos < 1) AMTK_FAIL("amtk_scan_comb_frames: bad argument");
  if (!validate_clip(clip, true) || !comb_thresholds_ok(prm, clip->bytes_per_sample)) return 0;
  DevSelect ds(ctx); if (!ds.ok) return 0;
  const size_t sbytes = (size_t)nframes * nlogos * 2 * sizeof(float), cbytes = (size_t)nframes * 12 * sizeof(int32_t);
  float* ds_ = scores; int* dc = counts;
  if (!out_on_device) {
    if (!ensure(&ctx->dout, &ctx->dout_bytes, sbytes) || !ensure(&ctx->dout2, &ctx->dout2_bytes, cbytes)) return 0;
    ds_ = reinterpret_cast<float*>(ctx->dout); dc = reinterpret_cast<int*>(ctx->dout2);
  }
  const amtk_logo* lg0 = logos[0];
  const bool lite = ctx->knobs.scan_lite && nlogos == 1 && lg0 && lg0->has_mask && lg0->host.count() > 0 &&
                    lg0->host.imgw == clip->width && lg0->host.imgh == clip->height &&
                    roi_inside(lg0->host, clip, clip->pitch_y / clip->bytes_per_sample) &&
                    logo_lite_smem_bytes(lg0->host.w, lg0->host.h, clip->bytes_per_sample) <= 29 * 1024;
  if (!for_each_window(ctx, clip, frame0, nframes, true, [&](const Window& w, int lo, int hi) -> int {
        if (lite && ctx->knobs.scan_lite == 2) {
          return launch_comb(ctx, clip, w, lo, hi, prm, dc, frame0) && launch_scan_lite(ctx, clip, w, lo, hi, lg0, ds_, nlogos, 0, frame0, false);
        }
        if (lite) {
          AMTK_CUDA(cudaEventRecord(ctx->ev_side, ctx->stream));
          if (!launch_comb(ctx, clip, w, lo, hi, prm, dc, frame0)) return 0;
          if (!launch_scan_lite(ctx, clip, w, lo, hi, lg0, ds_, nlogos, 0, frame0, true)) return 0;
          return cuda_ok(cudaStreamWaitEvent(ctx->stream, ctx->ev_side_done, 0), "cudaStreamWaitEvent") ? 1 : 0;
        }
        if (ctx->knobs.scan_overlap && clip->on_device) {
          ctx->want_side_mark = true;
          if (!launch_comb(ctx, clip, w, lo, hi, prm, dc, frame0)) { ctx->want_side_mark = false; return 0; }
          const bool marked = !ctx->want_side_mark;
          ctx->want_side_mark = false;
          if (marked) {
            AMTK_CUDA(cudaStreamWaitEvent(ctx->side_stream, ctx->ev_side, 0));
            cudaStream_t main_stream = ctx->stream;
            ctx->stream = ctx->side_stream;
            const int ok = scan_frames_impl(ctx, clip, clip, 0, 0, logos, nlogos, w, lo, hi, 0, ds_, frame0);
            ctx->stream = main_stream;
            if (!ok) return 0;
            AMTK_CUDA(cudaEventRecord(ctx->ev_side_done, ctx->side_stream));
            return cuda_ok(cudaStreamWaitEvent(ctx->stream, ctx->ev_side_done, 0), "cudaStreamWaitEvent") ? 1 : 0;
          }
          return scan_frames_impl(ctx, clip, clip, 0, 0, logos, nlogos, w, lo, hi, 0, ds_, frame0);
        }
        return launch_comb(ctx, clip, w, lo, hi, prm, dc, frame0) &&
               scan_frames_impl(ctx, clip, clip, 0, 0, logos, nlogos, w, lo, hi, 0, ds_, frame0); }))
    return 0;
  if (out_on_device) return 1;
  AMTK_CUDA(cudaMemcpyAsync(scores, ds_, sbytes, cudaMemcpyDeviceToHost, ctx->stream));
  AMTK_CUDA(cudaMemcpyAsync(counts, dc, cbytes, cudaMemcpyDeviceToHost, ctx->stream));
  AMTK_CUDA(cudaStreamSynchronize(ctx->stream));
  return 1;
}

int amtk_scan_create(amtk_ctx* ctx, int scanw, int scanh, int lx, int ly, int thy, amtk_scan** out) {
  if (!ctx || !out) AMTK_FAIL("amtk_scan_create: null argument");
  if (scanw < 4 || scanh < 4 || scanw > 4096 || scanh > 4096 || lx < 0 || lx > 2 || ly < 0 || ly > 2) AMTK_FAIL("amtk_scan_create: bad geometry");
  DevSelect ds(ctx); if (!ds.ok) return 0;
  amtk_scan* s = new amtk_scan();
  s->ctx = ctx; s->device = ctx->device; s->scanw = scanw; s->scanh = scanh; s->logUVx = lx; s->logUVy = ly; s->thy = thy;
  s->npix = (size_t)scanw * scanh + 2 * (size_t)(scanw >> lx) * (scanh >> ly);
  if (!cuda_ok(cudaMalloc(&s->dSums, s->npix * 3 * sizeof(unsigned long long)), "cudaMalloc") ||
      !cuda_ok(cudaMalloc(&s->dBg, 8 * sizeof(unsigned long long)), "cudaMalloc")) { amtk_scan_destroy(s); return 0; }
  cudaMemset(s->dSums, 0, s->npix * 3 * sizeof(unsigned long long));
  cudaMemset(s->dBg, 0, 8 * sizeof(unsigned long long));
  *out = s;
  return 1;
}

void amtk_scan_destroy(amtk_scan* s) {
  if (!s) return;
  { DevSelect ds(s->device); if (s->dSums) cudaFree(s->dSums); if (s->dBg) cudaFree(s->dBg); }
  delete s;
}

int amtk_scan_add_frames(amtk_scan* s, const amtk_clip* clip, int scanx, int scany, int frame0, int nframes,
                         const uint8_t* frame_select, uint8_t* valid_out) {
  if (!s) AMTK_FAIL("amtk_scan_add_frames: null scan");
  amtk_ctx* ctx = s->ctx;
  if (!validate_clip(clip, true)) return 0;
  if (clip->bytes_per_sample != 1) AMTK_FAIL("LogoScan supports 8-bit clips only (as the reference, LogoScan.hpp:812)");
  if (clip->log_uvx != s->logUVx || clip->log_uvy != s->logUVy) AMTK_FAIL("chroma subsampling mismatch");
  if (scanx < 0 || scany < 0 || scanx + s->scanw > clip->width || scany + s->scanh > clip->height) AMTK_FAIL("scan rectangle outside the frame");
  DevSelect ds(ctx); if (!ds.ok) return 0;
  const size_t bg_bytes = (size_t)nframes * sizeof(int4), off_sel = (bg_bytes + 255) & ~(size_t)255;
  const size_t off_val = off_sel + (((size_t)nframes + 255) & ~(size_t)255);
  if (!ensure(&ctx->dout, &ctx->dout_bytes, off_val + (size_t)nframes + 256)) return 0;
  uint8_t* base = reinterpret_cast<uint8_t*>(ctx->dout);
  int4* dbg = reinterpret_cast<int4*>(base); uint8_t* dsel = base + off_sel; uint8_t* dval = base + off_val;
  if (frame_select) AMTK_CUDA(cudaMemcpyAsync(dsel, frame_select, (size_t)nframes, cudaMemcpyHostToDevice, ctx->stream));
  const int ok = for_each_roi_window(ctx, clip, frame0, nframes, scanx, scany, s->scanw, s->scanh, true, false,
                                     [&](const amtk_clip& v, const Window& w, int lo, int hi, int dx, int dy) {
    ScanClip c;
    c.base = w.dev_base; c.frame_stride = v.frame_stride; c.offU = v.off_u; c.offV = v.off_v;
    c.pitchY = v.pitch_y; c.pitchUV = v.pitch_uv;
    c.scanx = scanx - dx; c.scany = scany - dy; c.scanw = s->scanw; c.scanh = s->scanh; c.logUVx = s->logUVx; c.logUVy = s->logUVy; c.thy = s->thy;
    c.frame0 = lo - w.first; c.nframes = hi - lo;
    const int rel = lo - frame0;
    scan_border_kernel<<<hi - lo, 256, 0, ctx->stream>>>(c, frame_select ? dsel + rel : nullptr, dbg + rel);
    AMTK_CUDA(cudaGetLastError());
    const int pixblocks = (int)((s->npix + 255) / 256);
    const int splits = std::max(1, std::min(hi - lo, (ctx->sm_count * 8) / pixblocks));
    scan_accumulate_kernel<<<dim3(pixblocks, splits), 256, 0, ctx->stream>>>(c, dbg + rel, s->dSums, s->dBg, dval + rel);
    AMTK_CUDA(cudaGetLastError());
    ctx->launches += 2;
    return 1;
  });
  if (!ok) return 0;
  std::vector<uint8_t> tmp;
  unsigned long long nv = 0;
  if (valid_out) AMTK_CUDA(cudaMemcpyAsync(valid_out, dval, (size_t)nframes, cudaMemcpyDeviceToHost, ctx->stream));
  AMTK_CUDA(cudaMemcpyAsync(&nv, s->dBg + 6, sizeof(nv), cudaMemcpyDeviceToHost, ctx->stream));
  AMTK_CUDA(cudaStreamSynchronize(ctx->stream));
  s->nvalid = (int)nv;
  return 1;
}

int amtk_scan_num_valid(const amtk_scan* s) { return s ? s->nvalid : 0; }

int amtk_scan_get_sums(amtk_scan* s, double* out) {
  if (!s || !out) AMTK_FAIL("amtk_scan_get_sums: null argument");
  DevSelect ds(s->ctx); if (!ds.ok) return 0;
  std::vector<unsigned long long> h(s->npix * 3), bg(8);
  AMTK_CUDA(cudaStreamSynchronize(s->ctx->stream));
  AMTK_CUDA(cudaMemcpy(h.data(), s->dSums, h.size() * sizeof(unsigned long long), cudaMemcpyDeviceToHost));
  AMTK_CUDA(cudaMemcpy(bg.data(), s->dBg, bg.size() * sizeof(unsigned long long), cudaMemcpyDeviceToHost));
  const size_t ny = (size_t)s->scanw * s->scanh, nc = (size_t)(s->scanw >> s->logUVx) * (s->scanh >> s->logUVy);
  for (size_t i = 0; i < s->npix; ++i) {
    const int pl = i < ny ? 0 : (i < ny + nc ? 1 : 2);
    out[i * 5 + 0] = (double)h[i * 3 + 0];
    out[i * 5 + 1] = (double)bg[pl * 2 + 0];
    out[i * 5 + 2] = (double)h[i * 3 + 1];
    out[i * 5 + 3] = (double)bg[pl * 2 + 1];
    out[i * 5 + 4] = (double)h[i * 3 + 2];
  }
  s->nvalid = (int)bg[6];
  return 1;
}

int amtk_scan_get_logo(amtk_scan* s, int maxv, int clean, float* data) {
  if (!s || !data) AMTK_FAIL("amtk_scan_get_logo: null argument");
  std::vector<double> sums(s->npix * 5);
  if (!amtk_scan_get_sums(s, sums.data())) return 0;
  if (!amtk::scan_finalize(sums.data(), s->nvalid, s->scanw, s->scanh, s->logUVx, s->logUVy, maxv, clean != 0, data))
    AMTK_FAIL("Insufficient logo frames");
  return 1;
}

namespace {
struct ScanGuard { amtk_scan* s = nullptr; ~ScanGuard() { if (s) amtk_scan_destroy(s); } };
struct LogoGuard { amtk_logo* l = nullptr; ~LogoGuard() { if (l) amtk_logo_destroy(l); } };
}

int amtk_scan_logo(amtk_ctx* ctx, const amtk_clip* clip, int service_id, const char* dstpath,
                   int imgx, int imgy, int w, int h, int thy, int max_frames, amtk_logo_analyze_cb cb) {
  if (!ctx || !dstpath) AMTK_FAIL("amtk_scan_logo: null argument");
  if (!validate_clip(clip, true)) return 0;
  if (clip->bytes_per_sample != 1) AMTK_FAIL("LogoScan supports 8-bit clips only (as the reference, LogoScan.hpp:812)");
  const int n = clip->num_frames;
  std::vector<uint8_t> valid((size_t)n), select((size_t)n, 0);
  int numFrames = 0, nread = 0;
  {
    ScanGuard probe;
    if (!amtk_scan_create(ctx, w, h, clip->log_uvx, clip->log_uvy, thy, &probe.s)) return 0;
    while (nread < n && numFrames < max_frames) {
      const int blk = std::min(200, n - nread);
      if (!amtk_scan_add_frames(probe.s, clip, imgx, imgy, nread, blk, nullptr, valid.data() + nread)) return 0;
      int i = nread;
      for (; i < nread + blk && numFrames < max_frames; ++i) if (valid[i]) { select[i] = 1; ++numFrames; }
      nread = (numFrames >= max_frames) ? i : nread + blk;
      if ((nread % 200) == 0 && cb && !cb(50.0f * (float)nread / (float)std::max(1, n), nread, 0, numFrames)) AMTK_FAIL("Cancel requested");
    }
  }
  const size_t ndata = ((size_t)w * h + 2 * (size_t)(w >> clip->log_uvx) * (h >> clip->log_uvy)) * 2;
  std::vector<float> logodata(ndata);
  {
    ScanGuard init;
    if (!amtk_scan_create(ctx, w, h, clip->log_uvx, clip->log_uvy, thy, &init.s)) return 0;
    if (!amtk_scan_add_frames(init.s, clip, imgx, imgy, 0, nread, select.data(), nullptr)) return 0;
    if (!amtk_scan_get_logo(init.s, 255, 0, logodata.data())) return 0;
  }
  float fades[20];
  for (int fi = 0; fi < 20; ++fi) fades[fi] = 0.1f * fi;
  const int kBlock = 128;
  std::vector<float> sweep((size_t)kBlock * 20);
  for (int round = 0; round < 2; ++round) {
    const float progressbase = 50.0f + 25.0f * round;
    LogoGuard raw, deint;
    if (!amtk_logo_create(ctx, logodata.data(), w, h, clip->log_uvx, clip->log_uvy, w, h, imgx, imgy, &raw.l)) return 0;
    if (!amtk_logo_deint(raw.l, &deint.l) || !amtk_logo_create_mask(deint.l, 0.1f)) return 0;
    std::vector<uint8_t> sel2((size_t)n, 0);
    int stored = 0;
    for (int f0 = 0; f0 < nread; f0 += kBlock) {
      const int blk = std::min(kBlock, nread - f0);
      bool any = false;
      for (int i = f0; i < f0 + blk; ++i) any = any || select[i];
      if (!any) continue;
      if (!amtk_logo_eval_fades(ctx, clip, deint.l, fades, 20, f0, blk, sweep.data(), 0)) return 0;
      for (int i = f0; i < f0 + blk; ++i) {
        if (!select[i]) continue;
        float best = FLT_MAX; int bi = 0;
        for (int fi = 0; fi < 20; ++fi) { const float r = std::fabs(sweep[(size_t)(i - f0) * 20 + fi]); if (r < best) { best = r; bi = fi; } }
        sel2[i] = bi > 8;
        if ((stored % 100) == 0 && cb && !cb((float)stored / (float)numFrames * 25.0f + progressbase, stored, numFrames, numFrames))
          AMTK_FAIL("Cancel requested");
        ++stored;
      }
    }
    ScanGuard acc;
    if (!amtk_scan_create(ctx, w, h, clip->log_uvx, clip->log_uvy, thy, &acc.s)) return 0;
    if (!amtk_scan_add_frames(acc.s, clip, imgx, imgy, 0, nread, sel2.data(), nullptr)) return 0;
    if (!amtk_scan_get_logo(acc.s, 255, 1, logodata.data())) return 0;
  }
  if (cb && !cb(1.0f, numFrames, numFrames, numFrames)) AMTK_FAIL("Cancel requested");
  LogoGuard fin;
  if (!amtk_logo_create(nullptr, logodata.data(), w, h, clip->log_uvx, clip->log_uvy, clip->width, clip->height, imgx, imgy, &fin.l)) return 0;
  return amtk_logo_save(fin.l, dstpath, "No Name", service_id);
}

int amtk_erase_logo_frames(amtk_ctx* ctx, const amtk_clip* clip, const amtk_logo* logo, int frame0, int nframes, const float* fades) {
  if (!ctx || !logo || !fades) AMTK_FAIL("amtk_erase_logo_frames: bad argument");
  if (!validate_clip(clip, true)) return 0;
  const amtk::HostLogo& h = logo->host;
  if (h.imgx < 0 || h.imgy < 0 || h.imgx + h.w > clip->width || h.imgy + h.h > clip->height) AMTK_FAIL("logo rectangle lies outside the frame");
  if (frame0 < 0 || nframes < 0 || frame0 + nframes > clip->num_frames) AMTK_FAIL("frame range outside the clip");
  if (nframes == 0) return 1;
  DevSelect ds(ctx); if (!ds.ok) return 0;
  if (!logo_ensure_device(logo, ctx, false)) return 0;
  if (!ensure(&ctx->dout, &ctx->dout_bytes, (size_t)nframes * 2 * sizeof(float))) return 0;
  AMTK_CUDA(cudaMemcpyAsync(ctx->dout, fades, (size_t)nframes * 2 * sizeof(float), cudaMemcpyHostToDevice, ctx->stream));
  const int ok = for_each_roi_window(ctx, clip, frame0, nframes, h.imgx, h.imgy, h.w, h.h, true, true,
                                     [&](const amtk_clip& v, const Window& w, int lo, int hi, int dx, int dy) {
    EraseJob j;
    j.base = const_cast<uint8_t*>(w.dev_base); j.frame_stride = v.frame_stride;
    j.offU = v.off_u; j.offV = v.off_v;
    j.pitchY = v.pitch_y / v.bytes_per_sample; j.pitchUV = v.pitch_uv / v.bytes_per_sample;
    j.frame0 = lo - w.first; j.nframes = hi - lo;
    j.w = h.w; j.h = h.h; j.logUVx = h.logUVx; j.logUVy = h.logUVy; j.imgx = h.imgx - dx; j.imgy = h.imgy - dy;
    j.uvparity = (h.imgy / 2) % 2;
    j.aY = logo->dA; j.bY = logo->dB; j.aU = logo->dAU; j.bU = logo->dBU; j.aV = logo->dAV; j.bV = logo->dBV;
    j.fades = reinterpret_cast<const float*>(ctx->dout) + (size_t)(lo - frame0) * 2;
    j.maxv = (float)((1 << v.bits_per_sample) - 1);
    if (v.bytes_per_sample == 1) erase_logo_kernel<uint8_t><<<hi - lo, 256, 0, ctx->stream>>>(j);
    else erase_logo_kernel<uint16_t><<<hi - lo, 256, 0, ctx->stream>>>(j);
    AMTK_CUDA(cudaGetLastError());
    ctx->launches += 1;
    return 1;
  });
  if (!ok) return 0;
  AMTK_CUDA(cudaStreamSynchronize(ctx->stream));
  return 1;
}

int amtk_weave_frames(amtk_ctx* ctx, const amtk_clip* src, const amtk_clip* dst, int dst_frame0,
                      const int32_t* top_idx, const int32_t* bottom_idx, int n, int src_is_nv12) {
  if (!ctx || !top_idx || !bottom_idx) AMTK_FAIL("amtk_weave_frames: null argument");
  if (!validate_clip(src, true) || !validate_clip(dst, true)) return 0;
  if (!src->on_device || !dst->on_device) AMTK_FAIL("amtk_weave_frames: clips must be device resident");
  if (src->width != dst->width || src->height != dst->height || src->bytes_per_sample != dst->bytes_per_sample ||
      src->log_uvx != dst->log_uvx || src->log_uvy != dst->log_uvy)
    AMTK_FAIL("amtk_weave_frames: source and destination formats differ");
  if (n < 0 || dst_frame0 < 0 || dst_frame0 + n > dst->num_frames) AMTK_FAIL("frame range outside the clip");
  for (int k = 0; k < n; ++k)
    if (top_idx[k] < 0 || top_idx[k] >= src->num_frames || bottom_idx[k] < 0 || bottom_idx[k] >= src->num_frames)
      AMTK_FAIL("amtk_weave_frames: source frame index outside the clip");
  if (n == 0) return 1;
  DevSelect ds(ctx); if (!ds.ok) return 0;
  if (!ensure(&ctx->dout, &ctx->dout_bytes, (size_t)n * 2 * sizeof(int))) return 0;
  int* didx = reinterpret_cast<int*>(ctx->dout);
  AMTK_CUDA(cudaMemcpyAsync(didx, top_idx, (size_t)n * sizeof(int), cudaMemcpyHostToDevice, ctx->stream));
  AMTK_CUDA(cudaMemcpyAsync(didx + n, bottom_idx, (size_t)n * sizeof(int), cudaMemcpyHostToDevice, ctx->stream));
  WeaveJob j;
  j.src = reinterpret_cast<const uint8_t*>(src->base); j.dst = const_cast<uint8_t*>(reinterpret_cast<const uint8_t*>(dst->base));
  j.sstride = src->frame_stride; j.dstride = dst->frame_stride;
  j.s_offu = src->off_u; j.s_offv = src->off_v; j.d_offu = dst->off_u; j.d_offv = dst->off_v;
  j.s_pitchY = src->pitch_y; j.s_pitchUV = src->pitch_uv; j.d_pitchY = dst->pitch_y; j.d_pitchUV = dst->pitch_uv;
  j.bps = src->bytes_per_sample; j.nv12 = src_is_nv12 ? 1 : 0;
  j.H = src->height; j.HC = src->height >> src->log_uvy;
  j.row_bytes_y = src->width * j.bps; j.row_bytes_c = (src->width >> src->log_uvx) * j.bps;
  j.top_idx = didx; j.bot_idx = didx + n; j.dst_frame0 = dst_frame0;
  for (int k0 = 0; k0 < n; k0 += 32768) {
    WeaveJob jj = j; jj.top_idx += k0; jj.bot_idx += k0; jj.dst_frame0 += k0;
    const int nn = std::min(32768, n - k0);
    const long long work = (long long)j.H * ((j.row_bytes_y + 15) / 16);
    dim3 grid((unsigned)std::min<long long>((work + 255) / 256, 4096), 3, nn);
    weave_kernel<<<grid, 256, 0, ctx->stream>>>(jj);
    AMTK_CUDA(cudaGetLastError());
    ctx->launches += 1;
  }
  AMTK_CUDA(cudaStreamSynchronize(ctx->stream));
  return 1;
}

void amtk_tnr_default_params(amtk_tnr_params* p) {
  if (!p) return;
  p->temporal_distance = 3; p->threshold = 1; p->interlaced = 0;
}

int amtk_tnr_frames(amtk_ctx* ctx, const amtk_clip* src, const amtk_clip* dst, int dst_frame0,
                    const amtk_tnr_params* p, int frame0, int nframes) {
  if (!ctx || !src || !dst || !p) AMTK_FAIL("amtk_tnr_frames: null argument");
  if (p->temporal_distance < 0 || p->temporal_distance > kTnrMaxD) AMTK_FAIL("tnr: temporal_distance must be in [0,63]");
  if (p->threshold < 0 || p->threshold > 65535) AMTK_FAIL("tnr: threshold must be in [0,65535]");
  if (p->interlaced != 0 && p->interlaced != 1) AMTK_FAIL("tnr: interlaced must be 0 or 1");
  if (!validate_clip(src, true) || !validate_clip(dst, true)) return 0;
  if (src->log_uvx != 1 || src->log_uvy != 1) AMTK_FAIL("tnr: only 4:2:0 clips are supported");
  const int bits = src->bits_per_sample;
  if (!(src->bytes_per_sample == 1 ? bits == 8 : (bits == 10 || bits == 12 || bits == 14 || bits == 16)))
    AMTK_FAIL("tnr: bits_per_sample must be 8 (1-byte samples) or 10, 12, 14, 16 (2-byte samples)");
  if ((src->width & 1) || (src->height & 1)) AMTK_FAIL("tnr: width and height must be even");
  if (p->interlaced && (src->height & 3)) AMTK_FAIL("tnr: interlaced clips need a height that is a multiple of 4");
  if (dst->width != src->width || dst->height != src->height || dst->log_uvx != 1 || dst->log_uvy != 1)
    AMTK_FAIL("tnr: source and destination formats differ");
  if (dst->bytes_per_sample != src->bytes_per_sample || dst->bits_per_sample != bits) {
    if (dst->bytes_per_sample == 1 && src->bytes_per_sample == 2)
      AMTK_FAIL("tnr: a 1-byte destination cannot hold a 2-byte source");
    if (dst->bytes_per_sample != 2 || dst->bits_per_sample == 8)
      AMTK_FAIL("tnr: source and destination formats differ (a 2-byte destination must be at 10, 12, 14 or 16 bits)");
    if (dst->bits_per_sample < bits)
      AMTK_FAIL("tnr: the destination has fewer bits than the source; only widening is provided (narrowing is dither arithmetic)");
    if (!(dst->bits_per_sample == 10 || dst->bits_per_sample == 12 || dst->bits_per_sample == 14 || dst->bits_per_sample == 16))
      AMTK_FAIL("tnr: bits_per_sample must be 8 (1-byte samples) or 10, 12, 14, 16 (2-byte samples)");
  }
  if (frame0 < 0 || nframes < 0 || frame0 + nframes > src->num_frames) AMTK_FAIL("frame range outside the clip");
  if (dst_frame0 < 0 || dst_frame0 + nframes > dst->num_frames) AMTK_FAIL("tnr: destination frame range outside the clip");
  if (src->on_device == dst->on_device) {
    uintptr_t s0, s1, d0, d1;
    clip_span(src, &s0, &s1); clip_span(dst, &d0, &d1);
    if (s0 < d1 && d0 < s1) AMTK_FAIL("tnr: source and destination overlap");
  }
  if (nframes == 0) return 1;
  DevSelect ds(ctx); if (!ds.ok) return 0;
  const int d = p->temporal_distance, N = src->num_frames;
  const size_t sfs = (size_t)src->frame_stride, dfs = (size_t)dst->frame_stride;
  size_t budget = (size_t)256 << 20;
  if (const char* e = getenv("AMTK_STAGE_MB")) budget = (size_t)std::max(1, atoi(e)) << 20;
  int per = nframes;
  if (!src->on_device) per = (int)std::max<long long>(1, std::min<long long>(per, (long long)(budget / sfs) - 2LL * d));
  if (!dst->on_device) per = (int)std::max<size_t>(1, std::min<size_t>((size_t)per, budget / dfs));
  if (!src->on_device) {
    const size_t need = (size_t)(per + 2 * d) * sfs;
    if (ctx->stage_bytes < need) {
      for (int b = 0; b < 2; ++b) { if (ctx->stage[b]) cudaFree(ctx->stage[b]); ctx->stage[b] = nullptr; }
      ctx->stage_bytes = 0;
      for (int b = 0; b < 2; ++b) AMTK_CUDA(cudaMalloc(&ctx->stage[b], need));
      ctx->stage_bytes = need;
// ... 275 lines not shown
```

amatsukaze_b200/csrc/amtk_internal.h:

```cpp
#pragma once
#include <cuda.h>
#include <cuda_runtime.h>
#include <cstdint>
#include <cstdio>
#include <mutex>
#include <string>
#include <vector>
#include "../../include/amtk_b200.h"
#include "logo_host.h"

typedef CUresult (*amtk_encode_tiled_fn)(CUtensorMap*, CUtensorMapDataType, cuuint32_t, void*, const cuuint64_t*,
                                         const cuuint64_t*, const cuuint32_t*, const cuuint32_t*, CUtensorMapInterleave,
                                         CUtensorMapSwizzle, CUtensorMapL2promotion, CUtensorMapFloatOOBfill);

namespace amtk {

void set_error(const std::string& msg);
bool cuda_ok(cudaError_t e, const char* what);

#define AMTK_CUDA(call)                                          \
  do {                                                           \
    if (!::amtk::cuda_ok((call), #call)) return 0;               \
  } while (0)
#define AMTK_FAIL(msg)                                           \
  do {                                                           \
    ::amtk::set_error(msg);                                      \
    return 0;                                                    \
  } while (0)

struct LogoDev {
  int w, h, count, countPad;
  float blackScore;
  const float* A;
  const float* B;
  const uint32_t* pix;
  const float* tapsT;
  const float2* scales;
};

}

struct amtk_ctx {
  mutable std::recursive_mutex mu;
  int device = 0;
  cudaStream_t stream = nullptr;
  bool own_stream = false;
  cudaStream_t copy_stream = nullptr;
  cudaStream_t side_stream = nullptr;
  cudaEvent_t ev_side = nullptr, ev_side_done = nullptr;
  cudaStream_t side_stream2 = nullptr;
  cudaEvent_t ev_fork = nullptr, ev_join1 = nullptr, ev_join2 = nullptr;
  size_t scratch_off = 0;
  cudaEvent_t ev_copy[2] = { nullptr, nullptr };
  cudaEvent_t ev_done[2] = { nullptr, nullptr };
  int sm_count = 0;
  int64_t launches = 0;
  long long h2d_bytes_last = 0;
  void* scratch = nullptr; size_t scratch_bytes = 0;
  void* stage[2] = { nullptr, nullptr }; size_t stage_bytes = 0;
  void* small = nullptr; size_t small_bytes = 0;
  void* dout = nullptr; size_t dout_bytes = 0;
  void* dout2 = nullptr; size_t dout2_bytes = 0;
  void* hout = nullptr; void* hout_dev = nullptr;
  amtk_encode_tiled_fn encode_tiled = nullptr;
  bool want_side_mark = false;
  struct Knobs {
    int eval_waves = 1;
    int eval_cw = 1;
    int eval_par = 1;
    int scan_overlap = 0;
    int comb_generic = 0;
    int comb_merge_uv = 1;
    int comb_part = -1;
    int comb_strip = 8, comb_stages = 3, comb_R = 0, comb_ctas = 0, comb_sync = 0, comb_l2 = 64;
    int comb_item = 0;
    int comb_tail = 4;
    int comb_ws_stages = 2;
    int comb_mma = 0;
    int comb_ws10 = 0;
    int comb_ws_warps = 4;
    int comb_ws_prefetch = 0;
    int comb_ws_band = 1;
    int lite_ctas = 5;
    int scan_lite = 0;
    int comb_ws = 1;
  } knobs;
  struct CombPlan {
    bool valid = false;
    int wY = 0, hY = 0, wC = 0, hC = 0, ntiles = 0, nf = 0, f0 = 0, R = 0, item = 0, ctas = 0;
    void* dev = nullptr; size_t cap = 0;
    int nitems = 0; size_t q_off = 0;
    int occ = 0; const void* occ_kernel = nullptr;
  } plan;
  int* ws_watch = nullptr;
  cudaEvent_t ev_watch = nullptr;
  bool watch_pending = false;
  bool timing = false;
  std::vector<std::pair<cudaEvent_t, cudaEvent_t>> timing_events;
  std::vector<std::pair<cudaEvent_t, cudaEvent_t>> timing_pool;
  double timing_ms = 0.0; int64_t timing_count = 0;
};

struct amtk_logo {
  int device = -1;
  amtk::HostLogo host;
  float* dA = nullptr; float* dB = nullptr;
  float* dAU = nullptr; float* dBU = nullptr; float* dAV = nullptr; float* dBV = nullptr;
  uint32_t* dPix = nullptr; float* dTapsT = nullptr; float2* dScales = nullptr;
  int countPad = 0;
  bool has_mask = false;
  bool tables_uploaded = false;
  std::mutex mu;
};

struct amtk_scan {
  amtk_ctx* ctx = nullptr;
  int device = 0;
  int scanw = 0, scanh = 0, logUVx = 1, logUVy = 1, thy = 0;
  int nvalid = 0;
  unsigned long long* dSums = nullptr;
  unsigned long long* dBg = nullptr;
  size_t npix = 0;
};
```

amatsukaze_b200/csrc/comb_stream.cuh:

```cuda
#pragma once
#include <cuda_fp16.h>
#include "amtk_internal.h"
#include "tma_utils.cuh"
#include "comb_kernels.cuh"

namespace amtk {

constexpr int kWsTW = 128;
constexpr int kWsRuns = 4;
constexpr int kWsWarps = 4;

template <int R_, int STAGES_, int WARPS_ = kWsWarps, int BPS_ = 1>
struct WsCfg {
  static constexpr int R = R_, STAGES = STAGES_, WARPS = WARPS_;
  static constexpr int BPS = BPS_;
  static constexpr int TH = kWsRuns * R;
  static constexpr int BOXH = TH + 4;
  static constexpr int STAGE_BYTES = kWsTW * BOXH;
  static constexpr int RING_BYTES = STAGES * STAGE_BYTES;
  static constexpr int SMEM = WARPS * RING_BYTES + 128;
  static constexpr int FIT = (227 * 1024) / (SMEM + 1024 + 8 * WARPS * STAGES + 8);
  static constexpr int MIN_CTAS = FIT >= 4 ? 4 : FIT >= 3 ? 3 : FIT >= 2 ? 2 : 1;
  static constexpr bool BAND = false;
};

constexpr int kWbW = 512;
constexpr int kWbHalf = 256;
template <int R_, int STAGES_>
struct WbCfg {
  static constexpr int R = R_, STAGES = STAGES_, WARPS = kWbW / kWsTW, BPS = 1;
  static constexpr int TH = kWsRuns * R;
  static constexpr int BOXH = TH + 4;
  static constexpr int HALF_BYTES = kWbHalf * BOXH;
  static constexpr int STAGE_BYTES = 2 * HALF_BYTES;
  static constexpr int SMEM = STAGES * STAGE_BYTES + 128;
  static constexpr int FIT = (227 * 1024) / (SMEM + 1024 + 12 * STAGES + 16);
  static constexpr int MIN_CTAS = FIT >= 4 ? 4 : FIT >= 3 ? 3 : FIT >= 2 ? 2 : 1;
  static constexpr bool BAND = true;
};

struct WsClass {
  int tile0, ntiles;
  int kind;
  int tilesX;
  int map;
  int x0;
  int W;
  int H;
  int cls;
  unsigned thM, thS, thL;
};
constexpr int kWsMaxClasses = 4;
struct WsArgs {
  CUtensorMap map[3];
  CUtensorMap map_uv;
  WsClass cl[kWsMaxClasses];
  int nclasses;
  const CombSegment* segs;
  int nitems;
  int* queue;
  int* counts;
  int out_frame0;
  int prefetch;
};

__device__ __forceinline__ void tma_load_4d(void* smem_dst, const CUtensorMap* map, uint64_t* bar, int c0, int c1, int c2, int c3) {
  asm volatile(
      "cp.async.bulk.tensor.4d.shared::cluster.global.mbarrier::complete_tx::bytes [%0], [%1, {%3, %4, %5, %6}], [%2];"
      ::"r"(smem_u32(smem_dst)), "l"(map), "r"(smem_u32(bar)), "r"(c0), "r"(c1), "r"(c2), "r"(c3)
      : "memory");
}

__device__ __forceinline__ void tma_prefetch_3d(const CUtensorMap* map, int c0, int c1, int c2) {
  asm volatile("cp.async.bulk.prefetch.tensor.3d.L2.global.tile [%0, {%1, %2, %3}];" ::"l"(map), "r"(c0), "r"(c1), "r"(c2) : "memory");
}
__device__ __forceinline__ void tma_prefetch_4d(const CUtensorMap* map, int c0, int c1, int c2, int c3) {
  asm volatile("cp.async.bulk.prefetch.tensor.4d.L2.global.tile [%0, {%1, %2, %3, %4}];" ::"l"(map), "r"(c0), "r"(c1), "r"(c2), "r"(c3) : "memory");
}

#ifndef AMTK_WS_RELOAD_PREV
#define AMTK_WS_RELOAD_PREV 1
#endif
constexpr bool kWsReloadPrev = AMTK_WS_RELOAD_PREV != 0;
#ifndef AMTK_WS_L_VIA_IDP
#define AMTK_WS_L_VIA_IDP 0
#endif
constexpr bool kWsLviaIdp = AMTK_WS_L_VIA_IDP != 0;
__device__ __forceinline__ uint4 lds128(const uint8_t* p) {
  uint4 v;
  asm("ld.shared.v4.u32 {%0, %1, %2, %3}, [%4];" : "=r"(v.x), "=r"(v.y), "=r"(v.z), "=r"(v.w) : "r"(smem_u32(p)));
  return v;
}

struct H8 { __half2 v[8]; };

__device__ __forceinline__ H8 bytes16_to_half(const uint4 raw) {
  H8 r;
  const uint32_t w[4] = { raw.x, raw.y, raw.z, raw.w };
#pragma unroll
  for (int i = 0; i < 4; ++i) {
    uint32_t a = __byte_perm(w[i], 0, 0x4140), b = __byte_perm(w[i], 0, 0x4342);
    r.v[2 * i] = *reinterpret_cast<__half2*>(&a); r.v[2 * i + 1] = *reinterpret_cast<__half2*>(&b);
  }
  return r;
}

struct WsCounts { uint32_t S[2], L[2], M[2]; };

__device__ __forceinline__ void ws_row_masks(const H8& h0, const H8& h1, const H8& h2, const H8& h3, const H8& h4,
                                             const __half2 thS, const __half2 thL, uint32_t& accS, uint32_t& accL) {
  const __half2 k4 = __float2half2_rn(4.0f), km3 = __float2half2_rn(-3.0f);
  uint32_t mS[8], mL[8];
#pragma unroll
  for (int q = 0; q < 8; ++q) {
    __half2 t = __hadd2(h0.v[q], h4.v[q]);
    t = __hfma2(k4, h2.v[q], t);
    const __half2 u = __hadd2(h1.v[q], h3.v[q]);
    const __half2 r = __habs2(__hfma2(km3, u, t));
    mS[q] = __hge2_mask(r, thS);
    mL[q] = __hge2_mask(r, thL);
  }
  accS = accS - (mS[0] + mS[1]) - (mS[2] + mS[3] + mS[4]) - (mS[5] + mS[6] + mS[7]);
  if (kWsLviaIdp) {
#pragma unroll
    for (int q = 0; q < 8; ++q) accL = __dp4a(mL[q], 0x01010101u, accL);
  } else {
    accL = accL - (mL[0] + mL[1]) - (mL[2] + mL[3] + mL[4]) - (mL[5] + mL[6] + mL[7]);
  }
}

template <int R, int PITCH>
__device__ __forceinline__ WsCounts ws_rows(const uint8_t* __restrict__ cur, uint4 (&P)[R],
                                            const uint32_t kM, const uint32_t thS_bits, const uint32_t thL_bits) {
  const __half2 thS = *reinterpret_cast<const __half2*>(&thS_bits);
  const __half2 thL = *reinterpret_cast<const __half2*>(&thL_bits);
  WsCounts c = { { 0u, 0u }, { 0u, 0u }, { 0u, 0u } };
  H8 h0 = bytes16_to_half(*reinterpret_cast<const uint4*>(cur));
  H8 h1 = bytes16_to_half(*reinterpret_cast<const uint4*>(cur + PITCH));
  uint4 raw_c = *reinterpret_cast<const uint4*>(cur + 2 * PITCH);
  uint4 raw_n = *reinterpret_cast<const uint4*>(cur + 3 * PITCH);
  H8 h2 = bytes16_to_half(raw_c);
  H8 h3 = bytes16_to_half(raw_n);
#pragma unroll
  for (int j = 0; j < R; ++j) {
    const uint4 raw_nn = *reinterpret_cast<const uint4*>(cur + (j + 4) * PITCH);
    const uint4 pv = P[j];
    const int f = j & 1;
    const H8 h4 = bytes16_to_half(raw_nn);
    c.M[f] = __dp4a(bytes_ge(__vabsdiffu4(raw_c.x, pv.x), kM), 0x01010101u, c.M[f]);
    c.M[f] = __dp4a(bytes_ge(__vabsdiffu4(raw_c.y, pv.y), kM), 0x01010101u, c.M[f]);
    c.M[f] = __dp4a(bytes_ge(__vabsdiffu4(raw_c.z, pv.z), kM), 0x01010101u, c.M[f]);
    c.M[f] = __dp4a(bytes_ge(__vabsdiffu4(raw_c.w, pv.w), kM), 0x01010101u, c.M[f]);
    if (kWsReloadPrev) P[j] = lds128(cur + (j + 2) * PITCH); else P[j] = raw_c;
    ws_row_masks(h0, h1, h2, h3, h4, thS, thL, c.S[f], c.L[f]);
    h0 = h1; h1 = h2; h2 = h3; h3 = h4; raw_c = raw_n; raw_n = raw_nn;
  }
  return c;
}


__device__ __forceinline__ void ws_masks_q(const __half2 r, const __half2 thS, const __half2 thL, uint32_t& mS, uint32_t& mL) {
  mS = __hge2_mask(__habs2(r), thS);
  mL = __hge2_mask(__habs2(r), thL);
}
template <int R, int PITCH>
__device__ __forceinline__ WsCounts ws_rows_sp(const uint8_t* __restrict__ cur, uint4 (&P)[R],
                                               const uint32_t kM, const uint32_t thS_bits, const uint32_t thL_bits) {
  const __half2 thS = *reinterpret_cast<const __half2*>(&thS_bits);
  const __half2 thL = *reinterpret_cast<const __half2*>(&thL_bits);
  const __half2 k4 = __float2half2_rn(4.0f), km3 = __float2half2_rn(-3.0f);
  WsCounts c = { { 0u, 0u }, { 0u, 0u }, { 0u, 0u } };
  H8 h0 = bytes16_to_half(*reinterpret_cast<const uint4*>(cur));
  H8 h1 = bytes16_to_half(*reinterpret_cast<const uint4*>(cur + PITCH));
  uint4 raw_c = *reinterpret_cast<const uint4*>(cur + 2 * PITCH);
  uint4 raw_n = *reinterpret_cast<const uint4*>(cur + 3 * PITCH);
  H8 h2 = bytes16_to_half(raw_c);
  H8 h3 = bytes16_to_half(raw_n);
  __half2 rp[8];
#pragma unroll
  for (int j = 0; j <= R; ++j) {
    uint4 raw_nn = make_uint4(0u, 0u, 0u, 0u);
    H8 h4;
    if (j < R) {
      raw_nn = *reinterpret_cast<const uint4*>(cur + (j + 4) * PITCH);
      const uint4 pv = P[j];
      const int f = j & 1;
      h4 = bytes16_to_half(raw_nn);
      c.M[f] = __dp4a(bytes_ge(__vabsdiffu4(raw_c.x, pv.x), kM), 0x01010101u, c.M[f]);
      c.M[f] = __dp4a(bytes_ge(__vabsdiffu4(raw_c.y, pv.y), kM), 0x01010101u, c.M[f]);
      c.M[f] = __dp4a(bytes_ge(__vabsdiffu4(raw_c.z, pv.z), kM), 0x01010101u, c.M[f]);
      c.M[f] = __dp4a(bytes_ge(__vabsdiffu4(raw_c.w, pv.w), kM), 0x01010101u, c.M[f]);
      if (kWsReloadPrev) P[j] = lds128(cur + (j + 2) * PITCH); else P[j] = raw_c;
    }
    uint32_t mS[8], mL[8];
    __half2 rn[8];
#pragma unroll
    for (int q = 0; q < 8; ++q) {
      if (j < R) {
        __half2 t = __hadd2(h0.v[q], h4.v[q]);
        t = __hfma2(k4, h2.v[q], t);
        const __half2 u = __hadd2(h1.v[q], h3.v[q]);
        rn[q] = __hfma2(km3, u, t);
      }
      if (j > 0) ws_masks_q(rp[q], thS, thL, mS[q], mL[q]);
    }
    if (j > 0) {
      const int fp = (j - 1) & 1;
      c.S[fp] = c.S[fp] - (mS[0] + mS[1]) - (mS[2] + mS[3] + mS[4]) - (mS[5] + mS[6] + mS[7]);
      c.L[fp] = c.L[fp] - (mL[0] + mL[1]) - (mL[2] + mL[3] + mL[4]) - (mL[5] + mL[6] + mL[7]);
    }
    if (j < R) {
#pragma unroll
      for (int q = 0; q < 8; ++q) rp[q] = rn[q];
      h0 = h1; h1 = h2; h2 = h3; h3 = h4; raw_c = raw_n; raw_n = raw_nn;
    }
  }
  return c;
}

#ifndef AMTK_WS_SP
#define AMTK_WS_SP 0
#endif
struct W4 { uint32_t v[4]; };
__device__ __forceinline__ W4 w4(const uint4 r) { W4 x; x.v[0] = r.x; x.v[1] = r.y; x.v[2] = r.z; x.v[3] = r.w; return x; }
constexpr uint32_t kWs10Bias = 8192u * 0x00010001u;

__device__ __forceinline__ void ws_row_masks10(const W4& h0, const W4& h1, const W4& h2, const W4& h3, const W4& h4,
                                               const __half2 thS, const __half2 thL, uint32_t& accS, uint32_t& accL) {
  uint32_t mS[4], mL[4];
#pragma unroll
  for (int q = 0; q < 4; ++q) {
    uint32_t t = h2.v[q] * 4u + h0.v[q];
    t = t + h4.v[q] + kWs10Bias;
    const uint32_t u = h1.v[q] + h3.v[q];
    const uint32_t rp = t - 3u * u;
    const uint32_t m = __vmaxu2(rp, 2u * kWs10Bias - rp);
    const __half2 mh = *reinterpret_cast<const __half2*>(&m);
    mS[q] = __hge2_mask(mh, thS);
    mL[q] = __hge2_mask(mh, thL);
  }
  accS = accS - (mS[0] + mS[1]) - (mS[2] + mS[3]);
  accL = accL - (mL[0] + mL[1]) - (mL[2] + mL[3]);
}

template <int R, int PITCH>
__device__ __forceinline__ WsCounts ws_rows10(const uint8_t* __restrict__ cur, uint4 (&P)[R],
                                              const uint32_t kM, const uint32_t thS_bits, const uint32_t thL_bits) {
  const __half2 thS = *reinterpret_cast<const __half2*>(&thS_bits);
  const __half2 thL = *reinterpret_cast<const __half2*>(&thL_bits);
  const __half2 thM = *reinterpret_cast<const __half2*>(&kM);
  WsCounts c = { { 0u, 0u }, { 0u, 0u }, { 0u, 0u } };
  W4 h0 = w4(*reinterpret_cast<const uint4*>(cur));
  W4 h1 = w4(*reinterpret_cast<const uint4*>(cur + PITCH));
  W4 h2 = w4(*reinterpret_cast<const uint4*>(cur + 2 * PITCH));
  W4 h3 = w4(*reinterpret_cast<const uint4*>(cur + 3 * PITCH));
#pragma unroll
  for (int j = 0; j < R; ++j) {
    const W4 h4 = w4(*reinterpret_cast<const uint4*>(cur + (j + 4) * PITCH));
    const W4 pv = w4(P[j]);
    const int f = j & 1;
    uint32_t mM[4];
#pragma unroll
    for (int q = 0; q < 4; ++q)
      mM[q] = __hge2_mask(__habs2(__hsub2(*reinterpret_cast<const __half2*>(&h2.v[q]), *reinterpret_cast<const __half2*>(&pv.v[q]))), thM);
    c.M[f] = c.M[f] - (mM[0] + mM[1]) - (mM[2] + mM[3]);
    if (kWsReloadPrev) P[j] = lds128(cur + (j + 2) * PITCH); else P[j] = make_uint4(h2.v[0], h2.v[1], h2.v[2], h2.v[3]);
    ws_row_masks10(h0, h1, h2, h3, h4, thS, thL, c.S[f], c.L[f]);
    h0 = h1; h1 = h2; h2 = h3; h3 = h4;
  }
  return c;
}

template <int PITCH>
__device__ __noinline__ void ws_fixup10(const uint8_t* cur, uint32_t rows, uint32_t mine, uint32_t thS_bits, uint32_t thL_bits, WsCounts& c) {
  const __half2 thS = *reinterpret_cast<const __half2*>(&thS_bits);
  const __half2 thL = *reinterpret_cast<const __half2*>(&thL_bits);
  for (uint32_t m = rows; m; m &= m - 1) {
    const int j = __ffs(m) - 1;
    if (!((mine >> j) & 1u)) continue;
    const uint8_t* p = cur + j * PITCH;
    uint32_t dS = 0u, dL = 0u;
    ws_row_masks10(w4(*reinterpret_cast<const uint4*>(p)), w4(*reinterpret_cast<const uint4*>(p + PITCH)), w4(*reinterpret_cast<const uint4*>(p + 2 * PITCH)),
                   w4(*reinterpret_cast<const uint4*>(p + 3 * PITCH)), w4(*reinterpret_cast<const uint4*>(p + 4 * PITCH)), thS, thL, dS, dL);
    c.S[j & 1] -= dS; c.L[j & 1] -= dL;
  }
}

template <int PITCH>
__device__ __noinline__ void ws_fixup(const uint8_t* cur, uint32_t rows, uint32_t mine, uint32_t thS_bits, uint32_t thL_bits, WsCounts& c) {
  const __half2 thS = *reinterpret_cast<const __half2*>(&thS_bits);
  const __half2 thL = *reinterpret_cast<const __half2*>(&thL_bits);
  for (uint32_t m = rows; m; m &= m - 1) {
    const int j = __ffs(m) - 1;
    if (!((mine >> j) & 1u)) continue;
    const uint8_t* p = cur + j * PITCH;
    const H8 h0 = bytes16_to_half(*reinterpret_cast<const uint4*>(p));
    const H8 h1 = bytes16_to_half(*reinterpret_cast<const uint4*>(p + PITCH));
    const H8 h2 = bytes16_to_half(*reinterpret_cast<const uint4*>(p + 2 * PITCH));
    const H8 h3 = bytes16_to_half(*reinterpret_cast<const uint4*>(p + 3 * PITCH));
    const H8 h4 = bytes16_to_half(*reinterpret_cast<const uint4*>(p + 4 * PITCH));
    uint32_t dS = 0u, dL = 0u;
    ws_row_masks(h0, h1, h2, h3, h4, thS, thL, dS, dL);
    c.S[j & 1] -= dS; c.L[j & 1] -= dL;
  }
}

template <typename Cfg>
__device__ __forceinline__ void ws_warp_streams(const WsArgs& a) {
  constexpr int S = Cfg::STAGES, R = Cfg::R;
  extern __shared__ uint8_t smem_raw[];
  __shared__ __align__(8) uint64_t full_bars[Cfg::WARPS][S];
  const int lane = threadIdx.x & 31, warp = threadIdx.x >> 5;
  uint8_t* tiles = smem_raw + ((128u - (smem_u32(smem_raw) & 127u)) & 127u) + warp * Cfg::RING_BYTES;
  uint64_t* full_bar = full_bars[warp];
  if (lane == 0) {
#pragma unroll
    for (int s = 0; s < S; ++s) mbar_init(&full_bar[s], 1);
    asm volatile("fence.mbarrier_init.release.cluster;" ::: "memory");
  }
  __syncwarp();
  uint32_t gload = 0;
  const int strip = lane & 7, run = lane >> 3;
  const int lane_off = (run * R) * kWsTW + strip * 16;
  for (;;) {
    int item = 0;
    if (lane == 0) item = atomicAdd(a.queue, 1);
    item = __shfl_sync(0xFFFFFFFFu, item, 0);
    if (item >= a.nitems) break;
    const CombSegment seg = a.segs[item];
    int ci = 0;
#pragma unroll
    for (int k = 1; k < kWsMaxClasses; ++k) if (k < a.nclasses && seg.tile >= a.cl[k].tile0) ci = k;
    const WsClass& C = a.cl[ci];
    const int lt = seg.tile - C.tile0;
    const int ty = lt / C.tilesX, tx = lt - ty * C.tilesX;
    const int y0 = ty * Cfg::TH;
    const int y_first = y0 + run * R;
    const int nf = seg.fend - seg.fbegin;
    const int nloads = nf + 1;
    const int fprev = seg.fbegin > 0 ? seg.fbegin - 1 : seg.fbegin;

    auto issue_at = [&](int j, int st) {
      const int fr = (j == 0) ? fprev : seg.fbegin + j - 1;
      mbar_expect_tx(&full_bar[st], Cfg::STAGE_BYTES);
      uint8_t* dst = tiles + st * Cfg::STAGE_BYTES;
      if (C.kind == 0) tma_load_3d(dst, &a.map[C.map], &full_bar[st], tx * kWsTW, y0 - 2, fr);
      else tma_load_4d(dst, &a.map_uv, &full_bar[st], C.x0, 0, y0 - 2, fr);
    };
    auto prefetch_at = [&](int j) {
      const int fr = seg.fbegin + j - 1;
      if (C.kind == 0) tma_prefetch_3d(&a.map[C.map], tx * kWsTW, y0 - 2, fr);
      else tma_prefetch_4d(&a.map_uv, C.x0, 0, y0 - 2, fr);
    };
    const int pf = a.prefetch;
    if (lane == 0) {
      const int pro = nloads < S ? nloads : S;
      for (int j = 0; j < pro; ++j) issue_at(j, (int)((gload + (uint32_t)j) % S));
      for (int j = S; j < S + pf && j < nloads; ++j) prefetch_at(j);
    }
    uint32_t fix_mine = 0u;
    if (y_first < 2) fix_mine |= (1u << (2 - y_first)) - 1u;
    {
      const int lo_j = max(C.H - 2 - y_first, 0), hi_j = min(C.H + 2 - y_first, R);
      if (hi_j > lo_j) fix_mine |= ((1u << hi_j) - 1u) & ~((1u << lo_j) - 1u);
    }
    const uint32_t fix_rows = __reduce_or_sync(0xFFFFFFFFu, fix_mine);
    const int flip = y_first & 1;
    const uint32_t kM = C.thM, tS = C.thS, tL = C.thL;
    int* const crow = a.counts + C.cls * 6 + lane + ((long long)seg.fbegin - 1 - a.out_frame0) * 12;

    int st = (int)(gload % S);
    uint32_t ph = (gload / S) & 1u;
    mbar_wait(&full_bar[st], ph);
    uint4 P[R];
    {
      const uint8_t* l0 = tiles + st * Cfg::STAGE_BYTES + lane_off;
#pragma unroll
      for (int j = 0; j < R; ++j) P[j] = *reinterpret_cast<const uint4*>(l0 + (j + 2) * kWsTW);
      __syncwarp();
      if (lane == 0 && S < nloads) issue_at(S, st);
      if (lane == 0 && pf > 0 && S + pf < nloads) prefetch_at(S + pf);
    }
    for (int k = 1; k <= nf; ++k) {
      if (++st == S) { st = 0; ph ^= 1u; }
      mbar_wait(&full_bar[st], ph);
      const uint8_t* cur = tiles + st * Cfg::STAGE_BYTES + lane_off;
      WsCounts c = Cfg::BPS == 2 ? ws_rows10<R, kWsTW>(cur, P, kM, tS, tL)
                                 : (AMTK_WS_SP ? ws_rows_sp<R, kWsTW>(cur, P, kM, tS, tL) : ws_rows<R, kWsTW>(cur, P, kM, tS, tL));
      if (fix_rows) {
        if (Cfg::BPS == 2) ws_fixup10<kWsTW>(cur, fix_rows, fix_mine, tS, tL, c); else ws_fixup<kWsTW>(cur, fix_rows, fix_mine, tS, tL, c);
        __syncwarp();
      }
      const uint32_t s0 = flip ? c.S[1] : c.S[0], s1 = flip ? c.S[0] : c.S[1];
      const uint32_t l0 = flip ? c.L[1] : c.L[0], l1 = flip ? c.L[0] : c.L[1];
      const uint32_t m0 = flip ? c.M[1] : c.M[0], m1 = flip ? c.M[0] : c.M[1];
      const uint32_t rM0 = __reduce_add_sync(0xFFFFFFFFu, m0), rS0 = __reduce_add_sync(0xFFFFFFFFu, s0), rL0 = __reduce_add_sync(0xFFFFFFFFu, l0);
      const uint32_t rM1 = __reduce_add_sync(0xFFFFFFFFu, m1), rS1 = __reduce_add_sync(0xFFFFFFFFu, s1), rL1 = __reduce_add_sync(0xFFFFFFFFu, l1);
      __syncwarp();
      if (lane == 0 && (k + S) < nloads) issue_at(k + S, st);
      if (lane == 0 && pf > 0 && (k + S + pf) < nloads) prefetch_at(k + S + pf);
      if (lane < 6) {
        const int fld = lane >= 3, met = lane - 3 * fld;
        uint32_t v = met == 0 ? (fld ? rM1 : rM0) : met == 1 ? (fld ? rS1 : rS0) : (fld ? rL1 : rL0);
        v = (met == 0 && Cfg::BPS == 1) ? (v >> 7) : (met == 2 && kWsLviaIdp && Cfg::BPS == 1) ? v / 510u : decode_pair(v);
        if (v) atomicAdd(crow + (size_t)k * 12, (int)v);
      }
    }
    gload += (uint32_t)nloads;
  }
}

template <typename Cfg>
__device__ __forceinline__ void ws_bands(const WsArgs& a) {
  constexpr int S = Cfg::STAGES, R = Cfg::R, NW = Cfg::WARPS;
  extern __shared__ uint8_t smem_raw[];
  __shared__ __align__(8) uint64_t full_bar[S];
  __shared__ uint32_t released[S];
  __shared__ int item_s[2];
  const int tid = threadIdx.x, lane = tid & 31, warp = tid >> 5;
  uint8_t* slots = smem_raw + ((128u - (smem_u32(smem_raw) & 127u)) & 127u);
  if (tid == 0) {
#pragma unroll
    for (int s = 0; s < S; ++s) { mbar_init(&full_bar[s], 1); released[s] = 0u; }
    asm volatile("fence.mbarrier_init.release.cluster;" ::: "memory");
  }
  __syncthreads();
  int* const dbg = a.queue + 16;
  uint32_t gload = 0;
  const int strip = lane & 7, run = lane >> 3;
  const int col = warp * kWsTW;
  const int lane_off = (col / kWbHalf) * Cfg::HALF_BYTES + (run * R) * kWbHalf + (col % kWbHalf) + strip * 16;
  for (int it = 0;; it ^= 1) {
    if (tid == 0) item_s[it] = atomicAdd(a.queue, 1);
    __syncthreads();
    const int item = item_s[it];
    if (item >= a.nitems) break;
    const CombSegment seg = a.segs[item];
    int ci = 0;
#pragma unroll
    for (int k = 1; k < kWsMaxClasses; ++k) if (k < a.nclasses && seg.tile >= a.cl[k].tile0) ci = k;
    const WsClass& C = a.cl[ci];
    const int lt = seg.tile - C.tile0;
    const int ty = lt / C.tilesX, tx = lt - ty * C.tilesX;
    const int y0 = ty * Cfg::TH, x0 = tx * kWbW;
    const int y_first = y0 + run * R;
    const bool two = x0 + kWbHalf < C.W;
    const bool active = x0 + col < C.W;
    const int nf = seg.fend - seg.fbegin;
    const int nloads = nf + 1;
    const int fprev = seg.fbegin > 0 ? seg.fbegin - 1 : seg.fbegin;
    const CUtensorMap* map = &a.map[C.map];

    auto issue_at = [&](int j, int st) {
      const int fr = (j == 0) ? fprev : seg.fbegin + j - 1;
      uint8_t* dst = slots + st * Cfg::STAGE_BYTES;
      mbar_expect_tx(&full_bar[st], two ? 2 * Cfg::HALF_BYTES : Cfg::HALF_BYTES);
      tma_load_3d(dst, map, &full_bar[st], x0, y0 - 2, fr);
      if (two) tma_load_3d(dst + Cfg::HALF_BYTES, map, &full_bar[st], x0 + kWbHalf, y0 - 2, fr);
    };
    auto release = [&](int j, int st) {
      __syncwarp();
      if (lane == 0 && atomicAdd(&released[st], 1u) % NW == NW - 1 && j + S < nloads) issue_at(j + S, st);
    };
    if (tid == 0) {
      const int pro = nloads < S ? nloads : S;
      for (int j = 0; j < pro; ++j) issue_at(j, (int)((gload + (uint32_t)j) % S));
    }
    uint32_t fix_mine = 0u;
    if (y_first < 2) fix_mine |= (1u << (2 - y_first)) - 1u;
    {
      const int lo_j = max(C.H - 2 - y_first, 0), hi_j = min(C.H + 2 - y_first, R);
      if (hi_j > lo_j) fix_mine |= ((1u << hi_j) - 1u) & ~((1u << lo_j) - 1u);
    }
    const uint32_t fix_rows = __reduce_or_sync(0xFFFFFFFFu, fix_mine);
    const int flip = y_first & 1;
    const uint32_t kM = C.thM, tS = C.thS, tL = C.thL;
    int* const crow = a.counts + C.cls * 6 + lane + ((long long)seg.fbegin - 1 - a.out_frame0) * 12;

    int st = (int)(gload % S);
    uint32_t ph = (gload / S) & 1u;
    mm_wait(&full_bar[st], ph, dbg, 1, 0);
    uint4 P[R];
    if (active) {
      const uint8_t* l0 = slots + st * Cfg::STAGE_BYTES + lane_off;
#pragma unroll
      for (int j = 0; j < R; ++j) P[j] = *reinterpret_cast<const uint4*>(l0 + (j + 2) * kWbHalf);
    }
    release(0, st);
    for (int k = 1; k <= nf; ++k) {
      if (++st == S) { st = 0; ph ^= 1u; }
      mm_wait(&full_bar[st], ph, dbg, 2, k);
      if (!active) { release(k, st); continue; }
      const uint8_t* cur = slots + st * Cfg::STAGE_BYTES + lane_off;
      WsCounts c = ws_rows<R, kWbHalf>(cur, P, kM, tS, tL);
      if (fix_rows) {
        ws_fixup<kWbHalf>(cur, fix_rows, fix_mine, tS, tL, c);
        __syncwarp();
      }
      const uint32_t s0 = flip ? c.S[1] : c.S[0], s1 = flip ? c.S[0] : c.S[1];
      const uint32_t l0 = flip ? c.L[1] : c.L[0], l1 = flip ? c.L[0] : c.L[1];
      const uint32_t m0 = flip ? c.M[1] : c.M[0], m1 = flip ? c.M[0] : c.M[1];
      const uint32_t rM0 = __reduce_add_sync(0xFFFFFFFFu, m0), rS0 = __reduce_add_sync(0xFFFFFFFFu, s0), rL0 = __reduce_add_sync(0xFFFFFFFFu, l0);
      const uint32_t rM1 = __reduce_add_sync(0xFFFFFFFFu, m1), rS1 = __reduce_add_sync(0xFFFFFFFFu, s1), rL1 = __reduce_add_sync(0xFFFFFFFFu, l1);
      release(k, st);
      if (lane < 6) {
        const int fld = lane >= 3, met = lane - 3 * fld;
        uint32_t v = met == 0 ? (fld ? rM1 : rM0) : met == 1 ? (fld ? rS1 : rS0) : (fld ? rL1 : rL0);
        v = met == 0 ? (v >> 7) : (met == 2 && kWsLviaIdp) ? v / 510u : decode_pair(v);
        if (v) atomicAdd(crow + (size_t)k * 12, (int)v);
      }
    }
    gload += (uint32_t)nloads;
  }
}

template <typename Cfg>
__global__ void __launch_bounds__(32 * Cfg::WARPS, Cfg::MIN_CTAS) comb_ws_kernel(const __grid_constant__ WsArgs a) {
  if constexpr (Cfg::BAND) ws_bands<Cfg>(a); else ws_warp_streams<Cfg>(a);
}
}
```

amatsukaze_b200/csrc/logo_kernels.cuh:

```cuda
#pragma once
#include "amtk_internal.h"
#include "exact_math.h"
#include "tma_utils.cuh"

namespace amtk {

constexpr int kEvalThreads = 512;
constexpr int kMaxFades = 24;

struct EvalJob {
  const void* ybase;
  long long frame_stride;
  int pitch;
  int frame0, nframes;
  int imgx, imgy;
  int roi_w, roi_h;
  int src_mode;
  int src_off, src_stride;
  LogoDev logo;
  float maxv;
  int nfades;
  float fades[kMaxFades];
  float* scores;
  int use_tma;
  int roi_box_w;
  int roi_box_x;
  int ab_smem;
  int pair_fades;
  CUtensorMap roi_map;
};

__host__ __device__ inline size_t logo_scores_smem_bytes(int roi_n, int npx, int raw_bytes_one, int ab_smem, int pair_fades) {
  return ((size_t)(ab_smem ? 2 : 0) * ((npx + 3) & ~3) + ((roi_n + 3) & ~3) +
          (size_t)(pair_fades ? 2 : 1) * (((size_t)npx + 8 + 3) & ~(size_t)3)) * sizeof(float) +
         128 + 2 * (((size_t)raw_bytes_one + 127) & ~(size_t)127);
}

template <typename pixel_t, int PXT, int CW = 0, int CH = 0>
__global__ void __launch_bounds__(kEvalThreads, 1) logo_scores_kernel(const __grid_constant__ EvalJob job) {
  extern __shared__ float smem_f[];
  __shared__ __align__(8) uint64_t roi_bar[2];
  const int tid = threadIdx.x;
  const LogoDev& lg = job.logo;
  const int w = CW ? CW : lg.w, npx = w * (CH ? CH : lg.h);
  const int roi_w = CW ? CW : job.roi_w;
  const int roi_h = CH ? CH : job.roi_h;
  const int roi_n = roi_w * roi_h;
  float* src = smem_f + (job.ab_smem ? 2 * ((npx + 3) & ~3) : 0);
  const float* sA = job.ab_smem ? smem_f : lg.A;
  const float* sB = job.ab_smem ? smem_f + ((npx + 3) & ~3) : lg.B;
  float* work = src + ((roi_n + 3) & ~3);
  float* work2 = work + ((npx + 8 + 3) & ~3);
  uint8_t* raw_base = reinterpret_cast<uint8_t*>(work + (size_t)(job.pair_fades ? 2 : 1) * ((npx + 8 + 3) & ~3));
  raw_base += (128u - (smem_u32(raw_base) & 127u)) & 127u;
  const int raw_pitch = job.roi_box_w;
  const uint32_t raw_bytes = (uint32_t)raw_pitch * roi_h * sizeof(pixel_t);
  const uint32_t raw_stride = (raw_bytes + 127u) & ~127u;

  if (job.ab_smem)
    for (int i = tid; i < npx; i += kEvalThreads) { smem_f[i] = lg.A[i]; smem_f[((npx + 3) & ~3) + i] = lg.B[i]; }
  float taps[PXT][25];
  int pxy[PXT];
  int cidx[PXT];
#pragma unroll
  for (int p = 0; p < PXT; ++p) {
    const int c = (blockIdx.x * PXT + p) * kEvalThreads + tid;
    cidx[p] = c;
    if (c < lg.count) {
      const uint32_t v = lg.pix[c];
      pxy[p] = (int)((v & 0xFFFFu) - 2) + (int)((v >> 16) - 2) * w;
#pragma unroll
      for (int t = 0; t < 25; ++t) taps[p][t] = lg.tapsT[(size_t)t * lg.countPad + c];
    } else {
      pxy[p] = 0;
#pragma unroll
      for (int t = 0; t < 25; ++t) taps[p][t] = 0.0f;
    }
  }
  const int roi_dx = kEvalThreads % roi_w, roi_dy = kEvalThreads / roi_w;
  const int roi_y0 = tid / roi_w, roi_x0 = tid - roi_y0 * roi_w;
  const int lg_dx = kEvalThreads % w, lg_dy = kEvalThreads / w;
  const int lg_y0 = tid / w, lg_x0 = tid - lg_y0 * w;

  if (job.use_tma && tid == 0) {
    mbar_init(&roi_bar[0], 1); mbar_init(&roi_bar[1], 1);
    asm volatile("fence.mbarrier_init.release.cluster;" ::: "memory");
  }
  __syncthreads();
  auto issue_roi = [&](int f, int buf) {
    mbar_expect_tx(&roi_bar[buf], raw_bytes);
    tma_load_3d(raw_base + buf * raw_stride, &job.roi_map, &roi_bar[buf], job.roi_box_x, job.imgy, job.frame0 + f);
  };
  int f = blockIdx.y;
  if (job.use_tma && tid == 0 && f < job.nframes) issue_roi(f, 0);
  for (int it = 0; f < job.nframes; f += gridDim.y, ++it) {
    const pixel_t* raw;
    if (job.use_tma) {
      if (tid == 0 && f + (int)gridDim.y < job.nframes) issue_roi(f + gridDim.y, (it + 1) & 1);
      mbar_wait(&roi_bar[it & 1], (uint32_t)(it >> 1) & 1u);
      raw = reinterpret_cast<const pixel_t*>(raw_base + (it & 1) * raw_stride) + (job.imgx - job.roi_box_x);
    } else {
      const pixel_t* fr = reinterpret_cast<const pixel_t*>(
          reinterpret_cast<const uint8_t*>(job.ybase) + (long long)(job.frame0 + f) * job.frame_stride);
      const pixel_t* roi = fr + job.imgx + (long long)job.imgy * job.pitch;
      pixel_t* dst = reinterpret_cast<pixel_t*>(raw_base);
      int x = roi_x0, y = roi_y0;
      for (int i = tid; i < roi_n; i += kEvalThreads) {
        dst[x + y * raw_pitch] = roi[x + (long long)y * job.pitch];
        x += roi_dx; y += roi_dy; if (x >= roi_w) { x -= roi_w; ++y; }
      }
      __syncthreads();
      raw = dst;
    }
    {
      int x = roi_x0, y = roi_y0;
      for (int i = tid; i < roi_n; i += kEvalThreads) {
        const pixel_t* rp = raw + x + y * raw_pitch;
        float v;
        if (job.src_mode == 0 && y > 0 && y < roi_h - 1) {
          const int a = rp[-raw_pitch], b = rp[0], c = rp[raw_pitch];
          v = (float)(a + 2 * b + c + 2) / 4.0f;
        } else {
          v = (float)rp[0];
        }
        src[i] = v;
        x += roi_dx; y += roi_dy; if (x >= roi_w) { x -= roi_w; ++y; }
      }
    }
    __syncthreads();

    const int fstep = job.pair_fades ? 2 : 1;
    for (int fi = 0; fi < job.nfades; fi += fstep) {
      const int nf2 = min(fstep, job.nfades - fi);
      const float fade0 = job.fades[fi], fade1 = job.fades[fi + nf2 - 1];
      const float omf0 = AMTK_FSUB(1.0f, fade0), omf1 = AMTK_FSUB(1.0f, fade1);
      {
        int x = lg_x0, y = lg_y0;
        for (int i = tid; i < npx; i += kEvalThreads) {
          const float srcv = src[job.src_off + x + y * job.src_stride];
          const float av = sA[i], bv = sB[i];
          work[i] = remove_logo(srcv, av, bv, job.maxv, fade0, omf0);
          if (nf2 == 2) work2[i] = remove_logo(srcv, av, bv, job.maxv, fade1, omf1);
          x += lg_dx; y += lg_dy; if (x >= w) { x -= w; ++y; }
        }
      }
      __syncthreads();
      float* out0 = job.scores + ((size_t)f * job.nfades + fi) * lg.countPad;
      float sum[2][PXT]; int bin[2][PXT];
#pragma unroll
      for (int p = 0; p < PXT; ++p) {
        const float* wp = work + pxy[p];
        float avg;
        sum[0][p] = corr5x5_tree(taps[p], [&](int dy, int dx) { return wp[dy * w + dx]; }, &avg);
        bin[0][p] = scale_bin(avg);
        if (nf2 == 2) {
          const float* wq = work2 + pxy[p];
          sum[1][p] = corr5x5_tree(taps[p], [&](int dy, int dx) { return wq[dy * w + dx]; }, &avg);
          bin[1][p] = scale_bin(avg);
        }
      }
#pragma unroll
      for (int p = 0; p < PXT; ++p) {
        if (cidx[p] < lg.count) {
          const float2* sc = lg.scales + (size_t)cidx[p] * 32;
          const float2 s0 = __ldg(sc + bin[0][p]);
          out0[cidx[p]] = pixel_score(sum[0][p], s0.x, s0.y);
          if (nf2 == 2) {
            const float2 s1 = __ldg(sc + bin[1][p]);
            out0[lg.countPad + cidx[p]] = pixel_score(sum[1][p], s1.x, s1.y);
          }
        }
      }
      __syncthreads();
    }
  }
}

constexpr int kLiteThreads = 128;
struct LiteJob {
  const void* ybase; long long frame_stride; int pitch;
  int frame0, nframes;
  int imgx, imgy;
  LogoDev logo;
  float maxv;
  int nfades; float fades[4];
  float* scores;
};
__host__ __device__ inline size_t logo_lite_smem_bytes(int w, int h, int bps) {
  return (((size_t)w * h + 8 + 3) & ~(size_t)3) * sizeof(float) + (((size_t)w * h * bps + 15) & ~(size_t)15) + 16;
}

template <typename pixel_t>
__global__ void __launch_bounds__(kLiteThreads, 4) logo_lite_kernel(const LiteJob job) {
  extern __shared__ __align__(16) float lite_smem[];
  const LogoDev& lg = job.logo;
  const int w = lg.w, h = lg.h, npx = w * h, tid = threadIdx.x;
  float* work = lite_smem;
  pixel_t* raw = reinterpret_cast<pixel_t*>(lite_smem + ((npx + 8 + 3) & ~3));
  for (int f = blockIdx.x; f < job.nframes; f += gridDim.x) {
    const pixel_t* roi = reinterpret_cast<const pixel_t*>(reinterpret_cast<const uint8_t*>(job.ybase) + (long long)(job.frame0 + f) * job.frame_stride) +
                         job.imgx + (long long)job.imgy * job.pitch;
    for (int i = tid; i < npx; i += kLiteThreads) { const int y = i / w, x = i - y * w; raw[i] = roi[x + (long long)y * job.pitch]; }
    __syncthreads();
    for (int fi = 0; fi < job.nfades; ++fi) {
      const float fade = job.fades[fi], omf = AMTK_FSUB(1.0f, fade);
      for (int i = tid; i < npx; i += kLiteThreads) {
        const int y = i / w;
        float v;
        if (y > 0 && y < h - 1) { const int a = raw[i - w], b = raw[i], c = raw[i + w]; v = (float)(a + 2 * b + c + 2) / 4.0f; }
        else v = (float)raw[i];
        work[i] = remove_logo(v, __ldg(lg.A + i), __ldg(lg.B + i), job.maxv, fade, omf);
      }
      __syncthreads();
      float* out = job.scores + ((size_t)f * job.nfades + fi) * lg.countPad;
      for (int c = tid; c < lg.count; c += kLiteThreads) {
        const uint32_t pv = __ldg(lg.pix + c);
        const float* wp = work + (int)((pv & 0xFFFFu) - 2) + (int)((pv >> 16) - 2) * w;
        float taps[25];
#pragma unroll
        for (int t = 0; t < 25; ++t) taps[t] = __ldg(lg.tapsT + (size_t)t * lg.countPad + c);
        float avg;
        const float sum = corr5x5_tree(taps, [&](int dy, int dx) { return wp[dy * w + dx]; }, &avg);
        const float2 sc = __ldg(lg.scales + (size_t)c * 32 + scale_bin(avg));
        out[c] = pixel_score(sum, sc.x, sc.y);
      }
      __syncthreads();
    }
  }
}

constexpr int kSumThreads = 32;
__global__ void __launch_bounds__(kSumThreads) logo_sum_kernel(const float* __restrict__ scores, int count, int countPad,
                                                               int nframes, int nfades, float blackScore, int take_abs,
                                                               float* __restrict__ out, int out_frame_stride, int out_off,
                                                               int out_fade_stride) {
  const int t = blockIdx.x * blockDim.x + threadIdx.x;
  if (t >= nframes * nfades) return;
  const float4* row = reinterpret_cast<const float4*>(scores + (size_t)t * countPad);
  const int nlines = countPad >> 5;
  float4 cur[8], nxt[8];
#pragma unroll
  for (int k = 0; k < 8; ++k) cur[k] = row[k];
  float r = 0.0f;
  int c = 0;
  for (int l = 0; l < nlines; ++l) {
    if (l + 1 < nlines) {
#pragma unroll
      for (int k = 0; k < 8; ++k) nxt[k] = row[(l + 1) * 8 + k];
    }
    if (c + 32 <= count) {
#pragma unroll
      for (int k = 0; k < 8; ++k) {
        r = AMTK_FADD(r, cur[k].x); r = AMTK_FADD(r, cur[k].y); r = AMTK_FADD(r, cur[k].z); r = AMTK_FADD(r, cur[k].w);
      }
      c += 32;
    } else {
#pragma unroll
      for (int k = 0; k < 8; ++k) {
        if (c < count) r = AMTK_FADD(r, cur[k].x); ++c;
        if (c < count) r = AMTK_FADD(r, cur[k].y); ++c;
        if (c < count) r = AMTK_FADD(r, cur[k].z); ++c;
        if (c < count) r = AMTK_FADD(r, cur[k].w); ++c;
      }
    }
#pragma unroll
    for (int k = 0; k < 8; ++k) cur[k] = nxt[k];
  }
  float v = AMTK_FDIV(r, blackScore);
  if (take_abs) v = fabsf(v);
  const int f = t / nfades, fi = t - f * nfades;
  out[(size_t)f * out_frame_stride + out_off + (size_t)fi * out_fade_stride] = v;
}

__global__ void __launch_bounds__(32) logo_sum_bulk_kernel(const float* __restrict__ scores, int count, int countPad,
                                                            int nframes, int nfades, float blackScore, int take_abs,
                                                            float* __restrict__ out, int out_frame_stride, int out_off,
                                                            int out_fade_stride) {
  extern __shared__ __align__(16) float sum_rows[];
  __shared__ __align__(8) uint64_t bar;
  const int lane = threadIdx.x, total = nframes * nfades;
  const int t0 = blockIdx.x * 32, nrows = min(32, total - t0);
  const int pitch = countPad + 4;
  const uint32_t row_bytes = (uint32_t)countPad * sizeof(float);
  if (lane == 0) { mbar_init(&bar, 1); asm volatile("fence.mbarrier_init.release.cluster;" ::: "memory"); }
  __syncwarp();
  if (lane == 0) mbar_expect_tx(&bar, row_bytes * (uint32_t)nrows);
  __syncwarp();
  if (lane < nrows) bulk_load_1d(sum_rows + (size_t)lane * pitch, scores + (size_t)(t0 + lane) * countPad, row_bytes, &bar);
  mbar_wait(&bar, 0);
  if (lane >= nrows) return;
  const float4* row = reinterpret_cast<const float4*>(sum_rows + (size_t)lane * pitch);
  float r = 0.0f;
  const int n4 = count >> 2;
#pragma unroll 8
  for (int i = 0; i < n4; ++i) {
    const float4 v = row[i];
    r = AMTK_FADD(r, v.x); r = AMTK_FADD(r, v.y); r = AMTK_FADD(r, v.z); r = AMTK_FADD(r, v.w);
  }
  const float* tail = sum_rows + (size_t)lane * pitch;
  for (int c = n4 << 2; c < count; ++c) r = AMTK_FADD(r, tail[c]);
  float v = AMTK_FDIV(r, blackScore);
  if (take_abs) v = fabsf(v);
  const int t = t0 + lane;
  const int f = t / nfades, fi = t - f * nfades;
  out[(size_t)f * out_frame_stride + out_off + (size_t)fi * out_fade_stride] = v;
}

__global__ void fill_pairs_kernel(float* out, int nframes, int stride, int off, float v0, float v1) {
  const int f = blockIdx.x * blockDim.x + threadIdx.x;
  if (f < nframes) { out[(size_t)f * stride + off] = v0; out[(size_t)f * stride + off + 1] = v1; }
}

}
```

Before: 855,500.

## Fuse logo scan into the band-form comb warp-stream kernel as interleaved work items

Removes the separate lite and overlap logo-scan paths and instead folds single-logo evaluation into the persistent comb warp-stream kernel. Logo work items (tile = -1) are spread evenly among the head comb segments and use the kernel's smem ring to stage ROI bytes and the A/B tables via cp.async. Each item computes both fades in one pass and reduces per-frame sums in-block, replacing a second launch plus a separate sum kernel. The intent is to remove launch overhead and hide the small logo work inside the comb stream. The cost is extra per-item smem reuse and fence overhead, and the comb kernel becomes more complex.

```diff
diff --git a/__graft_entry__.py b/__graft_entry__.py
--- a/__graft_entry__.py
+++ b/__graft_entry__.py
@@ -58,7 +58,7 @@
     assert np.array_equal(scores[:, 0].view(np.uint32), ref_s.view(np.uint32)), "logo scores differ from the oracle"
     assert np.array_equal(counts, ref_c), "combing counters differ from the oracle"
     launches = ctx.launches
-    assert launches >= 2
+    assert launches == 1
     ctx.close()
     del logo
     print("smoke ok: %d frames bit-exact vs %s, corr0 range [%.3f, %.3f], launches=%d"
diff --git a/amatsukaze_b200/csrc/amtk_b200.cu b/amatsukaze_b200/csrc/amtk_b200.cu
--- a/amatsukaze_b200/csrc/amtk_b200.cu
+++ b/amatsukaze_b200/csrc/amtk_b200.cu
@@ -378,17 +378,26 @@
   return 1;
 }
 
-static int launch_comb_ws(amtk_ctx* ctx, const amtk_clip* clip, const Window& win, int lo, int hi,
-                          const amtk_comb_params* prm, int* dcounts, int out_row0) {
+static const WsVariant* ws_variant(const amtk_ctx* ctx, const amtk_clip* clip) {
   const int hY = clip->height, hC = clip->height >> clip->log_uvy;
-  const int wY = clip->width, wC = clip->width >> clip->log_uvx;
   const int R = ctx->knobs.comb_R ? ctx->knobs.comb_R : pick_ws_R(hY, hC);
   int nvar = 0; const WsVariant* vars = ws_variants(&nvar); const WsVariant* V = nullptr;
   const int bps = clip->bytes_per_sample;
   const bool band = bps == 1 && ctx->knobs.comb_ws_band && ctx->knobs.comb_ws_warps == kWsWarps;
   for (int i = 0; i < nvar; ++i)
     if (vars[i].R == R && vars[i].stages == ctx->knobs.comb_ws_stages && vars[i].warps == ctx->knobs.comb_ws_warps && vars[i].bps == bps && vars[i].band == band) V = &vars[i];
+  return V;
+}
+
+static int launch_comb_ws(amtk_ctx* ctx, const amtk_clip* clip, const Window& win, int lo, int hi,
+                          const amtk_comb_params* prm, int* dcounts, int out_row0, const ScanItemJob* lj = nullptr) {
+  const int hY = clip->height, hC = clip->height >> clip->log_uvy;
+  const int wY = clip->width, wC = clip->width >> clip->log_uvx;
+  const int bps = clip->bytes_per_sample;
+  const WsVariant* V = ws_variant(ctx, clip);
   if (!V) AMTK_FAIL("comb: no warp-stream kernel variant for the requested AMTK_COMB_* settings");
+  const bool band = V->band;
+  if (lj && !band) AMTK_FAIL("comb: logo items need the band form");
   const int WW = V->warps;
   if (!ws_watchdog_ok(ctx)) return 0;
   WsArgs args;
@@ -458,13 +467,15 @@
   }
   int occ = plan.occ;
   if (ctx->knobs.comb_ctas > 0) occ = std::min(occ, ctx->knobs.comb_ctas);
-  const long long total = (long long)ntiles * nf;
+  const int logoF = lj ? lj->frames : 0, nlogo = lj ? (nf + logoF - 1) / logoF : 0;
+  const long long total = (long long)ntiles * nf + nlogo;
   const int per_cta = band ? 1 : WW;
   const int nwarps = ctx->sm_count * occ * per_cta;
   const int grid = (int)std::min<long long>((long long)ctx->sm_count * occ, (total + per_cta - 1) / per_cta);
   const int f0 = lo - win.first;
   if (!(plan.valid && plan.wY == wY && plan.hY == hY && plan.wC == wC && plan.hC == hC && plan.ntiles == ntiles && plan.nf == nf && plan.f0 == f0 &&
-        plan.R == V->R + 100 * bps + 1000 * band && plan.item == ctx->knobs.comb_item + 1000 * ctx->knobs.comb_tail && plan.ctas == occ * WW)) {
+        plan.R == V->R + 100 * bps + 1000 * band && plan.item == ctx->knobs.comb_item + 1000 * ctx->knobs.comb_tail && plan.ctas == occ * WW &&
+        plan.nlogo == nlogo && plan.logoF == logoF)) {
     int big = ctx->knobs.comb_item > 0 ? ctx->knobs.comb_item : 64, small = std::max(4, big / 4);
     while (big > 8 && (long long)ntiles * (nf / big) < 6LL * nwarps) { big /= 2; small = std::max(4, big / 4); }
     const int tail_frames = std::min(nf, std::max(small, (int)(nf * 0.15)));
@@ -473,7 +484,7 @@
     const int end_frames = (tiny > 0 && tiny < small) ? std::min(tail_frames, std::max(tiny, (int)(nf * 0.04))) : 0;
     const int mid_end = nf - end_frames;
     std::vector<CombSegment> segs;
-    segs.reserve((size_t)ntiles * (head_frames / big + tail_frames / small + (tiny > 0 ? end_frames / tiny : 0) + 3));
+    segs.reserve((size_t)ntiles * (head_frames / big + tail_frames / small + (tiny > 0 ? end_frames / tiny : 0) + 3) + nlogo);
     auto tier = [&](int fa, int fz, int step) {
       if (band) {
         for (int f = fa; f < fz; f += step)
@@ -484,6 +495,17 @@
       }
     };
     tier(0, head_frames, big);
+    if (nlogo > 0) {
+      const std::vector<CombSegment> head(segs);
+      const long long nhead = (long long)head.size();
+      segs.clear();
+      int k = 0;
+      for (long long i = 0; i <= nhead; ++i) {
+        for (; k < nlogo && (2LL * k + 1) * nhead / (2LL * nlogo) <= i; ++k)
+          segs.push_back(CombSegment{ -1, f0 + k * logoF, f0 + std::min(nf, (k + 1) * logoF) });
+        if (i < nhead) segs.push_back(head[(size_t)i]);
+      }
+    }
     tier(head_frames, mid_end, small);
     if (tiny > 0) tier(mid_end, nf, tiny);
     const size_t seg_bytes = segs.size() * sizeof(CombSegment);
@@ -494,7 +516,7 @@
     AMTK_CUDA(cudaStreamSynchronize(ctx->stream));
     plan.nitems = (int)segs.size();
     plan.wY = wY; plan.hY = hY; plan.wC = wC; plan.hC = hC; plan.ntiles = ntiles; plan.nf = nf; plan.f0 = f0; plan.R = V->R + 100 * bps + 1000 * band;
-    plan.item = ctx->knobs.comb_item + 1000 * ctx->knobs.comb_tail; plan.ctas = occ * WW; plan.valid = true;
+    plan.item = ctx->knobs.comb_item + 1000 * ctx->knobs.comb_tail; plan.ctas = occ * WW; plan.nlogo = nlogo; plan.logoF = logoF; plan.valid = true;
   }
   AMTK_CUDA(cudaMemsetAsync(reinterpret_cast<uint8_t*>(plan.dev) + plan.q_off, 0, 256, ctx->stream));
   args.segs = reinterpret_cast<const CombSegment*>(plan.dev);
@@ -510,10 +532,7 @@
     AMTK_CUDA(cudaEventRecord(ev.first, ctx->stream));
   }
   args.prefetch = ctx->knobs.comb_ws_prefetch;
-  if (ctx->want_side_mark) {
-    AMTK_CUDA(cudaEventRecord(ctx->ev_side, ctx->stream));
-    ctx->want_side_mark = false;
-  }
+  if (lj) args.logo = *lj;
   V->kernel<<<grid, 32 * WW, V->smem, ctx->stream>>>(args);
   AMTK_CUDA(cudaGetLastError());
   if (ctx->timing) { AMTK_CUDA(cudaEventRecord(ev.second, ctx->stream)); ctx->timing_events.push_back(ev); }
@@ -637,11 +656,18 @@
   return 1;
 }
 
+static bool comb_tma_layout(const amtk_ctx* ctx, const amtk_clip* clip, const Window& win) {
+  return ctx->encode_tiled && !((clip->frame_stride & 15) || (clip->pitch_y & 15) || (clip->pitch_uv & 15) || (clip->off_u & 15) ||
+                                (clip->off_v & 15) || (reinterpret_cast<uintptr_t>(win.dev_base) & 15));
+}
+static bool comb_runs_band(const amtk_ctx* ctx, const amtk_clip* clip, const Window& win) {
+  return comb_tma_layout(ctx, clip, win) && !ctx->knobs.comb_generic && !ctx->knobs.comb_mma && ctx->knobs.comb_ws &&
+         clip->bytes_per_sample == 1 && ctx->knobs.comb_ws_band && ctx->knobs.comb_ws_warps == kWsWarps;
+}
+
 static int launch_comb(amtk_ctx* ctx, const amtk_clip* clip, const Window& win, int lo, int hi,
                        const amtk_comb_params* prm, int* dcounts, int out_row0) {
-  const bool tma_layout = !((clip->frame_stride & 15) || (clip->pitch_y & 15) || (clip->pitch_uv & 15) || (clip->off_u & 15) ||
-                            (clip->off_v & 15) || (reinterpret_cast<uintptr_t>(win.dev_base) & 15));
-  if (!tma_layout || !ctx->encode_tiled || ctx->knobs.comb_generic) {
+  if (!comb_tma_layout(ctx, clip, win) || ctx->knobs.comb_generic) {
     CombGenericArgs g;
     g.base = win.dev_base; g.frame_stride = clip->frame_stride;
     g.off[0] = 0; g.off[1] = clip->off_u; g.off[2] = clip->off_v;
@@ -878,8 +904,6 @@
   c->stream = reinterpret_cast<cudaStream_t>(cuda_stream); c->own_stream = false;
   bool ok = cuda_ok(cudaStreamCreateWithFlags(&c->copy_stream, cudaStreamNonBlocking), "cudaStreamCreate(copy)") &&
             cuda_ok(cudaStreamCreateWithFlags(&c->side_stream, cudaStreamNonBlocking), "cudaStreamCreate(side)") &&
-            cuda_ok(cudaEventCreateWithFlags(&c->ev_side, cudaEventDisableTiming), "cudaEventCreate") &&
-            cuda_ok(cudaEventCreateWithFlags(&c->ev_side_done, cudaEventDisableTiming), "cudaEventCreate") &&
             cuda_ok(cudaStreamCreateWithFlags(&c->side_stream2, cudaStreamNonBlocking), "cudaStreamCreate(side2)") &&
             cuda_ok(cudaEventCreateWithFlags(&c->ev_fork, cudaEventDisableTiming), "cudaEventCreate") &&
             cuda_ok(cudaEventCreateWithFlags(&c->ev_join1, cudaEventDisableTiming), "cudaEventCreate") &&
@@ -906,8 +930,6 @@
   if (const char* e = getenv("AMTK_EVAL_WAVES")) c->knobs.eval_waves = std::max(1, atoi(e));
   if (const char* e = getenv("AMTK_COMB_L2")) c->knobs.comb_l2 = atoi(e);
   if (const char* e = getenv("AMTK_COMB_WS")) c->knobs.comb_ws = atoi(e);
-  if (const char* e = getenv("AMTK_SCAN_LITE")) c->knobs.scan_lite = atoi(e);
-  if (const char* e = getenv("AMTK_LITE_CTAS")) c->knobs.lite_ctas = std::max(1, atoi(e));
   if (const char* e = getenv("AMTK_COMB_WS_STAGES")) c->knobs.comb_ws_stages = atoi(e);
   if (const char* e = getenv("AMTK_COMB_ITEM")) c->knobs.comb_item = atoi(e);
   if (const char* e = getenv("AMTK_COMB_TAIL")) c->knobs.comb_tail = atoi(e);
@@ -915,7 +937,6 @@
   if (const char* e = getenv("AMTK_COMB_WS10")) c->knobs.comb_ws10 = atoi(e);
   if (const char* e = getenv("AMTK_EVAL_CW")) c->knobs.eval_cw = atoi(e);
   if (const char* e = getenv("AMTK_EVAL_PAR")) c->knobs.eval_par = atoi(e);
-  if (const char* e = getenv("AMTK_SCAN_OVERLAP")) c->knobs.scan_overlap = atoi(e);
   if (const char* e = getenv("AMTK_COMB_WS_WARPS")) c->knobs.comb_ws_warps = atoi(e);
   if (const char* e = getenv("AMTK_COMB_WS_PF")) c->knobs.comb_ws_prefetch = atoi(e);
   if (const char* e = getenv("AMTK_COMB_WS_BAND")) c->knobs.comb_ws_band = atoi(e);
@@ -931,8 +952,6 @@
   if (c->stream) cudaStreamSynchronize(c->stream);
   if (c->copy_stream) { cudaStreamSynchronize(c->copy_stream); cudaStreamDestroy(c->copy_stream); }
   if (c->side_stream) { cudaStreamSynchronize(c->side_stream); cudaStreamDestroy(c->side_stream); }
-  if (c->ev_side) cudaEventDestroy(c->ev_side);
-  if (c->ev_side_done) cudaEventDestroy(c->ev_side_done);
   if (c->side_stream2) { cudaStreamSynchronize(c->side_stream2); cudaStreamDestroy(c->side_stream2); }
   for (cudaEvent_t e : { c->ev_fork, c->ev_join1, c->ev_join2 }) if (e) cudaEventDestroy(e);
   for (int b = 0; b < 2; ++b) { if (c->ev_copy[b]) cudaEventDestroy(c->ev_copy[b]); if (c->ev_done[b]) cudaEventDestroy(c->ev_done[b]); if (c->stage[b]) cudaFree(c->stage[b]); }
@@ -1358,45 +1377,11 @@
   return finish_output(ctx, counts, d, bytes, out_on_device);
 }
 
-static int launch_scan_lite(amtk_ctx* ctx, const amtk_clip* clip, const Window& win, int lo, int hi, const amtk_logo* lg,
-                            float* dscores, int nlogos, int logo_index, int row0, bool side) {
-  cudaStream_t st = side ? ctx->side_stream : ctx->stream;
-  if (!logo_ensure_device(lg, ctx, true)) return 0;
-  const amtk::HostLogo& hl = lg->host;
-  const int count = hl.count(), countPad = lg->countPad, n = hi - lo;
-  if (!ensure(&ctx->scratch, &ctx->scratch_bytes, (size_t)n * 2 * countPad * sizeof(float))) return 0;
-  LiteJob job;
-  job.ybase = win.dev_base; job.frame_stride = clip->frame_stride; job.pitch = clip->pitch_y / clip->bytes_per_sample;
-  job.frame0 = lo - win.first; job.nframes = n; job.imgx = hl.imgx; job.imgy = hl.imgy;
-  job.logo = logo_dev(lg); job.maxv = (float)((1 << clip->bits_per_sample) - 1);
-  job.nfades = 2; job.fades[0] = 0.0f; job.fades[1] = 1.0f;
-  job.scores = reinterpret_cast<float*>(ctx->scratch);
-  const size_t smem = logo_lite_smem_bytes(hl.w, hl.h, clip->bytes_per_sample);
-  if (side) AMTK_CUDA(cudaStreamWaitEvent(ctx->side_stream, ctx->ev_side, 0));
-  const int grid = side ? std::min(n, ctx->sm_count) : std::min(n, ctx->sm_count * ctx->knobs.lite_ctas);
-  static bool carveout_set = false;
-  if (!carveout_set) {
-    AMTK_CUDA(cudaFuncSetAttribute(logo_lite_kernel<uint8_t>, cudaFuncAttributePreferredSharedMemoryCarveout, cudaSharedmemCarveoutMaxShared));
-    AMTK_CUDA(cudaFuncSetAttribute(logo_lite_kernel<uint16_t>, cudaFuncAttributePreferredSharedMemoryCarveout, cudaSharedmemCarveoutMaxShared));
-    AMTK_CUDA(cudaFuncSetAttribute(logo_sum_bulk_kernel, cudaFuncAttributePreferredSharedMemoryCarveout, cudaSharedmemCarveoutMaxShared));
-    carveout_set = true;
-  }
-  if (clip->bytes_per_sample == 1) logo_lite_kernel<uint8_t><<<grid, kLiteThreads, smem, st>>>(job);
-  else logo_lite_kernel<uint16_t><<<grid, kLiteThreads, smem, st>>>(job);
-  AMTK_CUDA(cudaGetLastError());
-  const int total = n * 2;
-  float* sum_out = dscores + (size_t)(lo - row0) * nlogos * 2;
-  const size_t sum_smem = (size_t)32 * (countPad + 4) * sizeof(float);
-  if (sum_smem <= 200 * 1024) {
-    if (!want_smem(ctx, (const void*)logo_sum_bulk_kernel, (int)sum_smem)) return 0;
-    logo_sum_bulk_kernel<<<(total + 31) / 32, 32, sum_smem, st>>>(job.scores, count, countPad, n, 2, hl.blackScore, 0, sum_out, nlogos * 2, logo_index * 2, 1);
-  } else {
-    logo_sum_kernel<<<(total + kSumThreads - 1) / kSumThreads, kSumThreads, 0, st>>>(job.scores, count, countPad, n, 2, hl.blackScore, 0, sum_out, nlogos * 2, logo_index * 2, 1);
-  }
-  AMTK_CUDA(cudaGetLastError());
-  if (side) AMTK_CUDA(cudaEventRecord(ctx->ev_side_done, ctx->side_stream));
-  ctx->launches += 2;
-  return 1;
+static int scan_item_frames(const amtk_logo* lg, const WsVariant* V) {
+  const size_t ring = (size_t)V->smem - 128;
+  int F = 0;
+  while (F < kScanItemMaxFrames && scan_item_smem_bytes(lg->host.w, lg->host.h, lg->countPad, F + 1) <= ring) ++F;
+  return F;
 }
 
 int amtk_scan_comb_frames(amtk_ctx* ctx, const amtk_clip* clip, amtk_logo* const* logos, int nlogos,
@@ -1412,36 +1397,20 @@
     ds_ = reinterpret_cast<float*>(ctx->dout); dc = reinterpret_cast<int*>(ctx->dout2);
   }
   const amtk_logo* lg0 = logos[0];
-  const bool lite = ctx->knobs.scan_lite && nlogos == 1 && lg0 && lg0->has_mask && lg0->host.count() > 0 &&
-                    lg0->host.imgw == clip->width && lg0->host.imgh == clip->height &&
-                    roi_inside(lg0->host, clip, clip->pitch_y / clip->bytes_per_sample) &&
-                    logo_lite_smem_bytes(lg0->host.w, lg0->host.h, clip->bytes_per_sample) <= 29 * 1024;
+  const bool one_logo = nlogos == 1 && lg0 && lg0->has_mask && lg0->host.count() > 0 &&
+                        lg0->host.imgw == clip->width && lg0->host.imgh == clip->height && lg0->host.imgx >= 0 && lg0->host.imgy >= 0 &&
+                        lg0->host.imgx + lg0->host.w <= clip->width && lg0->host.imgy + lg0->host.h <= clip->height;
   if (!for_each_window(ctx, clip, frame0, nframes, true, [&](const Window& w, int lo, int hi) -> int {
-        if (lite && ctx->knobs.scan_lite == 2) {
-          return launch_comb(ctx, clip, w, lo, hi, prm, dc, frame0) && launch_scan_lite(ctx, clip, w, lo, hi, lg0, ds_, nlogos, 0, frame0, false);
-        }
-        if (lite) {
-          AMTK_CUDA(cudaEventRecord(ctx->ev_side, ctx->stream));
-          if (!launch_comb(ctx, clip, w, lo, hi, prm, dc, frame0)) return 0;
-          if (!launch_scan_lite(ctx, clip, w, lo, hi, lg0, ds_, nlogos, 0, frame0, true)) return 0;
-          return cuda_ok(cudaStreamWaitEvent(ctx->stream, ctx->ev_side_done, 0), "cudaStreamWaitEvent") ? 1 : 0;
-        }
-        if (ctx->knobs.scan_overlap && clip->on_device) {
-          ctx->want_side_mark = true;
-          if (!launch_comb(ctx, clip, w, lo, hi, prm, dc, frame0)) { ctx->want_side_mark = false; return 0; }
-          const bool marked = !ctx->want_side_mark;
-          ctx->want_side_mark = false;
-          if (marked) {
-            AMTK_CUDA(cudaStreamWaitEvent(ctx->side_stream, ctx->ev_side, 0));
-            cudaStream_t main_stream = ctx->stream;
-            ctx->stream = ctx->side_stream;
-            const int ok = scan_frames_impl(ctx, clip, clip, 0, 0, logos, nlogos, w, lo, hi, 0, ds_, frame0);
-            ctx->stream = main_stream;
-            if (!ok) return 0;
-            AMTK_CUDA(cudaEventRecord(ctx->ev_side_done, ctx->side_stream));
-            return cuda_ok(cudaStreamWaitEvent(ctx->stream, ctx->ev_side_done, 0), "cudaStreamWaitEvent") ? 1 : 0;
-          }
-          return scan_frames_impl(ctx, clip, clip, 0, 0, logos, nlogos, w, lo, hi, 0, ds_, frame0);
+        const WsVariant* V = one_logo && comb_runs_band(ctx, clip, w) ? ws_variant(ctx, clip) : nullptr;
+        const int F = V ? scan_item_frames(lg0, V) : 0;
+        if (F > 0) {
+          if (!logo_ensure_device(lg0, ctx, true)) return 0;
+          ScanItemJob lj;
+          lj.ybase = w.dev_base; lj.frame_stride = clip->frame_stride; lj.pitch = clip->pitch_y;
+          lj.imgx = lg0->host.imgx; lj.imgy = lg0->host.imgy;
+          lj.logo = logo_dev(lg0); lj.maxv = (float)((1 << clip->bits_per_sample) - 1);
+          lj.frames = F; lj.scores = ds_;
+          return launch_comb_ws(ctx, clip, w, lo, hi, prm, dc, frame0, &lj);
         }
         return launch_comb(ctx, clip, w, lo, hi, prm, dc, frame0) &&
                scan_frames_impl(ctx, clip, clip, 0, 0, logos, nlogos, w, lo, hi, 0, ds_, frame0); }))
diff --git a/amatsukaze_b200/csrc/amtk_internal.h b/amatsukaze_b200/csrc/amtk_internal.h
--- a/amatsukaze_b200/csrc/amtk_internal.h
+++ b/amatsukaze_b200/csrc/amtk_internal.h
@@ -46,9 +46,7 @@
   cudaStream_t stream = nullptr;
   bool own_stream = false;
   cudaStream_t copy_stream = nullptr;
-  cudaStream_t side_stream = nullptr;
-  cudaEvent_t ev_side = nullptr, ev_side_done = nullptr;
-  cudaStream_t side_stream2 = nullptr;
+  cudaStream_t side_stream = nullptr, side_stream2 = nullptr;
   cudaEvent_t ev_fork = nullptr, ev_join1 = nullptr, ev_join2 = nullptr;
   size_t scratch_off = 0;
   cudaEvent_t ev_copy[2] = { nullptr, nullptr };
@@ -63,12 +61,10 @@
   void* dout2 = nullptr; size_t dout2_bytes = 0;
   void* hout = nullptr; void* hout_dev = nullptr;
   amtk_encode_tiled_fn encode_tiled = nullptr;
-  bool want_side_mark = false;
   struct Knobs {
     int eval_waves = 1;
     int eval_cw = 1;
     int eval_par = 1;
-    int scan_overlap = 0;
     int comb_generic = 0;
     int comb_merge_uv = 1;
     int comb_part = -1;
@@ -81,13 +77,12 @@
     int comb_ws_warps = 4;
     int comb_ws_prefetch = 0;
     int comb_ws_band = 1;
-    int lite_ctas = 5;
-    int scan_lite = 0;
     int comb_ws = 1;
   } knobs;
   struct CombPlan {
     bool valid = false;
     int wY = 0, hY = 0, wC = 0, hC = 0, ntiles = 0, nf = 0, f0 = 0, R = 0, item = 0, ctas = 0;
+    int nlogo = 0, logoF = 0;
     void* dev = nullptr; size_t cap = 0;
     int nitems = 0; size_t q_off = 0;
     int occ = 0; const void* occ_kernel = nullptr;
diff --git a/amatsukaze_b200/csrc/comb_stream.cuh b/amatsukaze_b200/csrc/comb_stream.cuh
--- a/amatsukaze_b200/csrc/comb_stream.cuh
+++ b/amatsukaze_b200/csrc/comb_stream.cuh
@@ -3,6 +3,7 @@
 #include "amtk_internal.h"
 #include "tma_utils.cuh"
 #include "comb_kernels.cuh"
+#include "logo_kernels.cuh"
 
 namespace amtk {
 
@@ -62,6 +63,7 @@
   int* counts;
   int out_frame0;
   int prefetch;
+  ScanItemJob logo;
 };
 
 __device__ __forceinline__ void tma_load_4d(void* smem_dst, const CUtensorMap* map, uint64_t* bar, int c0, int c1, int c2, int c3) {
@@ -436,6 +438,11 @@
     const int item = item_s[it];
     if (item >= a.nitems) break;
     const CombSegment seg = a.segs[item];
+    if (seg.tile < 0) {
+      scan_item<32 * NW>(a.logo, seg.fbegin, seg.fend, a.out_frame0, slots);
+      asm volatile("fence.proxy.async.shared::cta;" ::: "memory");
+      continue;
+    }
     int ci = 0;
 #pragma unroll
     for (int k = 1; k < kWsMaxClasses; ++k) if (k < a.nclasses && seg.tile >= a.cl[k].tile0) ci = k;
diff --git a/amatsukaze_b200/csrc/logo_kernels.cuh b/amatsukaze_b200/csrc/logo_kernels.cuh
--- a/amatsukaze_b200/csrc/logo_kernels.cuh
+++ b/amatsukaze_b200/csrc/logo_kernels.cuh
@@ -176,56 +176,97 @@
   }
 }
 
-constexpr int kLiteThreads = 128;
-struct LiteJob {
-  const void* ybase; long long frame_stride; int pitch;
-  int frame0, nframes;
+struct ScanItemJob {
+  const uint8_t* ybase;
+  long long frame_stride;
+  int pitch;
   int imgx, imgy;
   LogoDev logo;
   float maxv;
-  int nfades; float fades[4];
+  int frames;
   float* scores;
 };
-__host__ __device__ inline size_t logo_lite_smem_bytes(int w, int h, int bps) {
-  return (((size_t)w * h + 8 + 3) & ~(size_t)3) * sizeof(float) + (((size_t)w * h * bps + 15) & ~(size_t)15) + 16;
-}
-
-template <typename pixel_t>
-__global__ void __launch_bounds__(kLiteThreads, 4) logo_lite_kernel(const LiteJob job) {
-  extern __shared__ __align__(16) float lite_smem[];
-  const LogoDev& lg = job.logo;
-  const int w = lg.w, h = lg.h, npx = w * h, tid = threadIdx.x;
-  float* work = lite_smem;
-  pixel_t* raw = reinterpret_cast<pixel_t*>(lite_smem + ((npx + 8 + 3) & ~3));
-  for (int f = blockIdx.x; f < job.nframes; f += gridDim.x) {
-    const pixel_t* roi = reinterpret_cast<const pixel_t*>(reinterpret_cast<const uint8_t*>(job.ybase) + (long long)(job.frame0 + f) * job.frame_stride) +
-                         job.imgx + (long long)job.imgy * job.pitch;
-    for (int i = tid; i < npx; i += kLiteThreads) { const int y = i / w, x = i - y * w; raw[i] = roi[x + (long long)y * job.pitch]; }
+constexpr int kScanItemMaxFrames = 8;
+__host__ __device__ inline size_t scan_item_smem_bytes(int w, int h, int countPad, int frames) {
+  return (2 * (((size_t)w * h + 8 + 3) & ~(size_t)3) + (size_t)frames * 2 * (countPad + 4)) * sizeof(float) + (size_t)((w + 30) & ~15) * h;
+}
+
+__device__ __forceinline__ void cp_async16(void* smem_dst, const void* src) {
+  asm volatile("cp.async.cg.shared.global [%0], [%1], 16;" ::"r"(smem_u32(smem_dst)), "l"(src) : "memory");
+}
+__device__ __forceinline__ void cp_async4(void* smem_dst, const void* src) {
+  asm volatile("cp.async.ca.shared.global [%0], [%1], 4;" ::"r"(smem_u32(smem_dst)), "l"(src) : "memory");
+}
+
+template <int NT>
+__device__ __forceinline__ void scan_item(const ScanItemJob& j, int fbegin, int fend, int out_frame0, uint8_t* smem) {
+  const LogoDev& lg = j.logo;
+  const int tid = threadIdx.x, w = lg.w, h = lg.h, npx = w * h, count = lg.count, spitch = lg.countPad + 4;
+  float* work0 = reinterpret_cast<float*>(smem);
+  float* work1 = work0 + ((npx + 8 + 3) & ~3);
+  float* sc = work1 + ((npx + 8 + 3) & ~3);
+  uint8_t* raw = reinterpret_cast<uint8_t*>(sc + (size_t)j.frames * 2 * spitch);
+  const int xa = j.imgx & ~15, xo = j.imgx - xa;
+  const int rpitch = (xo + w + 15) & ~15, cpr = rpitch >> 4, nchunks = cpr * h;
+  const float omf0 = AMTK_FSUB(1.0f, 0.0f), omf1 = AMTK_FSUB(1.0f, 1.0f);
+  const int dx = NT % w, dy = NT / w, y0 = tid / w, x0 = tid - y0 * w;
+  for (int f = fbegin; f < fend; ++f) {
     __syncthreads();
-    for (int fi = 0; fi < job.nfades; ++fi) {
-      const float fade = job.fades[fi], omf = AMTK_FSUB(1.0f, fade);
-      for (int i = tid; i < npx; i += kLiteThreads) {
-        const int y = i / w;
+    const uint8_t* roi = j.ybase + (long long)f * j.frame_stride + xa + (long long)j.imgy * j.pitch;
+    for (int k = tid; k < nchunks; k += NT) {
+      const int y = k / cpr;
+      cp_async16(raw + 16 * k, roi + (long long)y * j.pitch + 16 * (k - y * cpr));
+    }
+    for (int q = tid; q < (npx >> 2); q += NT) { cp_async16(work0 + 4 * q, lg.A + 4 * q); cp_async16(work1 + 4 * q, lg.B + 4 * q); }
+    for (int i = (npx & ~3) + tid; i < npx; i += NT) { cp_async4(work0 + i, lg.A + i); cp_async4(work1 + i, lg.B + i); }
+    asm volatile("cp.async.wait_all;" ::: "memory");
+    __syncthreads();
+    {
+      int x = x0, y = y0;
+      for (int i = tid; i < npx; i += NT) {
+        const uint8_t* rp = raw + y * rpitch + xo + x;
         float v;
-        if (y > 0 && y < h - 1) { const int a = raw[i - w], b = raw[i], c = raw[i + w]; v = (float)(a + 2 * b + c + 2) / 4.0f; }
-        else v = (float)raw[i];
-        work[i] = remove_logo(v, __ldg(lg.A + i), __ldg(lg.B + i), job.maxv, fade, omf);
-      }
-      __syncthreads();
-      float* out = job.scores + ((size_t)f * job.nfades + fi) * lg.countPad;
-      for (int c = tid; c < lg.count; c += kLiteThreads) {
-        const uint32_t pv = __ldg(lg.pix + c);
-        const float* wp = work + (int)((pv & 0xFFFFu) - 2) + (int)((pv >> 16) - 2) * w;
-        float taps[25];
-#pragma unroll
-        for (int t = 0; t < 25; ++t) taps[t] = __ldg(lg.tapsT + (size_t)t * lg.countPad + c);
-        float avg;
-        const float sum = corr5x5_tree(taps, [&](int dy, int dx) { return wp[dy * w + dx]; }, &avg);
-        const float2 sc = __ldg(lg.scales + (size_t)c * 32 + scale_bin(avg));
-        out[c] = pixel_score(sum, sc.x, sc.y);
-      }
-      __syncthreads();
-    }
+        if (y > 0 && y < h - 1) { const int a = rp[-rpitch], b = rp[0], c = rp[rpitch]; v = (float)(a + 2 * b + c + 2) / 4.0f; }
+        else v = (float)rp[0];
+        const float av = work0[i], bv = work1[i];
+        work0[i] = remove_logo(v, av, bv, j.maxv, 0.0f, omf0);
+        work1[i] = remove_logo(v, av, bv, j.maxv, 1.0f, omf1);
+        x += dx; y += dy; if (x >= w) { x -= w; ++y; }
+      }
+    }
+    __syncthreads();
+    float* s0 = sc + (size_t)(f - fbegin) * 2 * spitch;
+    float2 kp0 = make_float2(0.0f, 0.0f), kp1 = kp0;
+    int cp = -1;
+#pragma unroll 1
+    for (int c = tid; c < count; c += NT) {
+      const uint32_t pv = __ldg(lg.pix + c);
+      float taps[25];
+#pragma unroll
+      for (int t = 0; t < 25; ++t) taps[t] = __ldg(lg.tapsT + (size_t)t * lg.countPad + c);
+      const int o = (int)((pv & 0xFFFFu) - 2) + (int)((pv >> 16) - 2) * w;
+      float avg0, avg1;
+      s0[c] = corr5x5_tree(taps, [&](int ry, int rx) { return work0[o + ry * w + rx]; }, &avg0);
+      s0[spitch + c] = corr5x5_tree(taps, [&](int ry, int rx) { return work1[o + ry * w + rx]; }, &avg1);
+      const float2 kn0 = __ldg(lg.scales + (size_t)c * 32 + scale_bin(avg0)), kn1 = __ldg(lg.scales + (size_t)c * 32 + scale_bin(avg1));
+      if (cp >= 0) { s0[cp] = pixel_score(s0[cp], kp0.x, kp0.y); s0[spitch + cp] = pixel_score(s0[spitch + cp], kp1.x, kp1.y); }
+      kp0 = kn0; kp1 = kn1; cp = c;
+    }
+    if (cp >= 0) { s0[cp] = pixel_score(s0[cp], kp0.x, kp0.y); s0[spitch + cp] = pixel_score(s0[spitch + cp], kp1.x, kp1.y); }
+  }
+  __syncthreads();
+  if (tid < 2 * (fend - fbegin)) {
+    const float* row = sc + (size_t)tid * spitch;
+    const float4* row4 = reinterpret_cast<const float4*>(row);
+    const int n4 = count >> 2;
+    float r = 0.0f;
+#pragma unroll 1
+    for (int i = 0; i < n4; ++i) {
+      const float4 v = row4[i];
+      r = AMTK_FADD(r, v.x); r = AMTK_FADD(r, v.y); r = AMTK_FADD(r, v.z); r = AMTK_FADD(r, v.w);
+    }
+    for (int c = n4 << 2; c < count; ++c) r = AMTK_FADD(r, row[c]);
+    j.scores[(size_t)(fbegin + (tid >> 1) - out_frame0) * 2 + (tid & 1)] = AMTK_FDIV(r, lg.blackScore);
   }
 }
 
```

After: 898,200, median of 6. 1.05x the previous value.
